# daijifeng001/MNC

Measured on AMD Instinct MI355X. Metric: images/sec (600x1000, 300 RoIs) VGG16 MNC-5stage, higher is better.
Workload: dtype f32; 1 GPU; VGG16 MNC 5-stage inference + gpu_mask_voting; one 600x1000 uint8 image per GPU per step (8 seeded images rotating), 300 RoIs per stage, H2D + device prep + forward + tail + gpu_mask_voting + D2H of the voted instances all inside the timed region; synthetic weights; math=fp32, images_in_flight_per_gpu=12, engine=native, parallelism=single GPU

## Files before the change

include/mnc_hip.h:

```cpp
#ifndef MNC_HIP_H_
#define MNC_HIP_H_

#include <stddef.h>

#ifdef __cplusplus
extern "C" {
#endif

#define MNC_API __attribute__((visibility("default")))

enum {
  MNC_OK = 0,
  MNC_ERR_INVALID = 1,
  MNC_ERR_HIP = 2,
  MNC_ERR_NOMEM = 3,
  MNC_ERR_STATE = 4,
  MNC_ERR_UNSUPPORTED = 5
};

MNC_API const char* mnc_last_error(void);
MNC_API int mnc_device_count(int* count);
MNC_API int mnc_device_mem_info(int device_id, size_t* free_bytes, size_t* total_bytes);
MNC_API const char* mnc_version(void);

// ... 61 lines not shown
  long long work;
  long long reserved1;
} mnc_mask_info;
typedef struct mnc_mask_head {
  int kept;
  int reserved0;
  long long bits_bytes;
  long long items;
  long long reserved1[29];
} mnc_mask_head;
MNC_API int mnc_instance_masks(const double* boxes, const float* masks, int n, int mask_size, double binarize_thresh,
                               int image_height, int image_width, int clip, int* bounds, long long* offsets, long long* areas,
                               void* bits, size_t bits_cap, size_t* bits_bytes, int device_id);

MNC_API int mnc_mask_overlaps(const int* a_bounds, const long long* a_offsets, const long long* a_areas, const void* a_bits,
                              size_t a_bytes, int na, const int* b_bounds, const long long* b_offsets, const long long* b_areas,
                              const void* b_bits, size_t b_bytes, int nb, long long* inter, double* iou, int device_id);
MNC_API int mnc_mask_nms(const int* bounds, const long long* offsets, const long long* areas, const void* bits, size_t bytes,
                         int n, const int* classes, const float* scores, double thresh, int class_aware, int* keep_out,
                         int* num_out, int device_id);

MNC_API int mnc_mask_rle(const int* bounds, const long long* offsets, const void* bits, size_t bytes, int n, int H, int W,
                         long long* run_ptr, unsigned* runs, size_t runs_cap, size_t* runs_total, int device_id);
MNC_API int mnc_mask_from_rle(const long long* run_ptr, const unsigned* runs, int n, int H, int W, int* bounds, long long* offsets,
                              long long* areas, void* bits, size_t bits_cap, size_t* bits_bytes, int device_id);

MNC_API int mnc_mask_match(const int* dt_bounds, const long long* dt_offsets, const long long* dt_areas, const void* dt_bits,
                           size_t dt_bytes, int nd, const int* dt_classes, const float* dt_scores, const int* gt_bounds,
                           const long long* gt_offsets, const long long* gt_areas, const void* gt_bits, size_t gt_bytes, int ng,
                           const int* gt_classes, const unsigned char* gt_crowd, const unsigned char* gt_ignore_in,
                           const double* gt_eval_area, const double* iou_thrs, int T, const double* area_rngs, int A, int max_det,
                           int* rank, int* dt_match, unsigned char* dt_ignore, int* gt_match, unsigned char* gt_ignore,
                           double* iou, int device_id);

MNC_API int mnc_mask_from_polygons(const double* xy, const long long* vert_ptr, const long long* poly_ptr, int n, int H, int W,
                                   int* bounds, long long* offsets, long long* areas, void* bits, size_t bits_cap,
                                   size_t* bits_bytes, int device_id);
MNC_API int mnc_mask_poly_timing(int on, double* last_ms);

MNC_API int mnc_coco_accumulate(const int* dt_class_idx, const float* dt_score, const int* dt_rank, const unsigned char* dt_flags,
                                int N, const int* gt_class_idx, const unsigned char* gt_ignore, int Gn, int K, int T, int A,
                                const int* max_dets, int M, const double* rec_thrs, int R, double* precision, double* recall,
                                long long* npig, int device_id);
MNC_API int mnc_coco_accum_timing(int on, double* last_ms);

MNC_API int mnc_mask_boundary(const int* bounds, const long long* offsets, const void* bits, size_t bytes, int n, int H, int W,
                              int d, int* out_bounds, long long* out_offsets, long long* out_areas, void* out_bits,
                              size_t bits_cap, size_t* bits_bytes, int device_id);
MNC_API int mnc_mask_match_boundary(const int* dt_bounds, const long long* dt_offsets, const long long* dt_areas, const void* dt_bits,
                                    size_t dt_bytes, int nd, const int* dt_classes, const float* dt_scores, const int* gt_bounds,
                                    const long long* gt_offsets, const long long* gt_areas, const void* gt_bits, size_t gt_bytes,
                                    int ng, const int* gt_classes, const unsigned char* gt_crowd, const unsigned char* gt_ignore_in,
                                    const double* gt_eval_area, const double* iou_thrs, int T, const double* area_rngs, int A,
                                    int max_det, int H, int W, int d, int* rank, int* dt_match, unsigned char* dt_ignore,
                                    int* gt_match, unsigned char* gt_ignore, double* iou, double* biou, int device_id);
MNC_API int mnc_mask_boundary_timing(int on, double* last_ms);

MNC_API int mnc_mask_components(const int* bounds, const long long* offsets, const void* bits, size_t bytes, int n, int connectivity,
                                long long* comp_ptr, long long* area, int* bbox, int* anchor, size_t comp_cap, size_t* n_comp,
                                int device_id);
MNC_API int mnc_mask_select(const int* bounds, const long long* offsets, const void* bits, size_t bytes, int n, int connectivity,
                            int min_area, int keep, long long* out_areas, void* out_bits, size_t bits_cap, int device_id);
MNC_API int mnc_mask_fill_holes(const int* bounds, const long long* offsets, const void* bits, size_t bytes, int n, int connectivity,
                                long long* out_areas, void* out_bits, size_t bits_cap, int device_id);
MNC_API int mnc_mask_split(const int* bounds, const long long* offsets, const void* bits, size_t bytes, int n, int connectivity,
                           int* out_bounds, long long* out_offsets, long long* out_areas, int* out_source, size_t comp_cap,
                           size_t* n_comp, void* out_bits, size_t bits_cap, size_t* bits_bytes, int device_id);
MNC_API int mnc_mask_components_timing(int on, double* last_ms);

MNC_API int mnc_mask_contours(const int* bounds, const long long* offsets, const void* bits, size_t bytes, int n, int connectivity,
                              long long* loop_ptr, long long* vert_ptr, long long* area, int* xy, size_t loop_cap, size_t vert_cap,
                              size_t* n_loops, size_t* n_verts, int device_id);
MNC_API int mnc_mask_contours_timing(int on, double* last_ms);

MNC_API int mnc_contours_simplify(const long long* vert_ptr, const int* xy, size_t n_loops, size_t n_verts, int q,
                                  long long* out_vert_ptr, int* out_xy, long long* out_index, size_t* out_verts, int device_id);
MNC_API int mnc_contours_simplify_timing(int on, double* last_ms);

MNC_API int mnc_mcg_maskdb(const int* superpixels, int H, int W, const int* label_ptr, const int* label_ids, int n,
                           int mask_size, double* boxes, unsigned char* masks, int device_id);

MNC_API int mnc_bbox_overlaps(const double* boxes, int n, const double* query_boxes, int k, double* overlaps);

typedef struct mnc_ctx mnc_ctx;

MNC_API int mnc_ctx_create(mnc_ctx** out, int device_id);
MNC_API int mnc_ctx_destroy(mnc_ctx* ctx);
MNC_API int mnc_ctx_sync(mnc_ctx* ctx);
MNC_API int mnc_ctx_device(const mnc_ctx* ctx, int* device_id);
MNC_API int mnc_ctx_arena_generation(const mnc_ctx* ctx, unsigned long* generation);

typedef struct mnc_layer_conventions {
  int warp_sample;
  int warp_round_edges;
  int warp_no_plus_one;
  int warp_oob;
  int resize_mode;
  int maskpool_binary;
  float maskpool_thresh;
  int inherit;
} mnc_layer_conventions;
MNC_API int mnc_ctx_set_layer_conventions(mnc_ctx* ctx, const mnc_layer_conventions* conv);
MNC_API int mnc_ctx_set_tuning(mnc_ctx* ctx, const char* name, const char* value);
MNC_API int mnc_ctx_get_layer_conventions(const mnc_ctx* ctx, mnc_layer_conventions* conv);

typedef struct mnc_graph mnc_graph;
MNC_API int mnc_ctx_capture_begin(mnc_ctx* ctx);
MNC_API int mnc_ctx_capture_end(mnc_ctx* ctx, mnc_graph** out);
MNC_API int mnc_graph_launch(mnc_ctx* ctx, mnc_graph* graph);
MNC_API int mnc_graph_destroy(mnc_graph* graph);
MNC_API int mnc_proposal_count_ptr(mnc_ctx* ctx, void** d_count);

MNC_API int mnc_dev_alloc(mnc_ctx* ctx, size_t bytes, void** d_ptr);
MNC_API int mnc_dev_free(mnc_ctx* ctx, void* d_ptr);
MNC_API int mnc_h2d(mnc_ctx* ctx, void* d_dst, const void* src_host, size_t bytes);
MNC_API int mnc_d2h(mnc_ctx* ctx, void* dst_host, const void* d_src, size_t bytes);
MNC_API int mnc_d2d(mnc_ctx* ctx, void* d_dst, const void* d_src, size_t bytes);
MNC_API int mnc_dev_zero(mnc_ctx* ctx, void* d_ptr, size_t bytes);
MNC_API int mnc_host_alloc(mnc_ctx* ctx, size_t bytes, void** host_ptr);
MNC_API int mnc_host_free(mnc_ctx* ctx, void* host_ptr);
MNC_API int mnc_h2d_async(mnc_ctx* ctx, void* d_dst, const void* src_host, size_t bytes);
MNC_API int mnc_d2h_async(mnc_ctx* ctx, void* dst_host, const void* d_src, size_t bytes);

MNC_API int mnc_prof_enable(mnc_ctx* ctx, int enable);
MNC_API int mnc_prof_reset(mnc_ctx* ctx);
MNC_API int mnc_prof_count(mnc_ctx* ctx, int* n_records);
MNC_API int mnc_prof_get(mnc_ctx* ctx, int index, char* name_buf, int name_cap, float* ms, double* flops,
                         double* bytes);

MNC_API int mnc_nchw_to_c8(mnc_ctx* ctx, const float* d_nchw, float* d_c8, int C, int H, int W);
MNC_API int mnc_c8_to_nchw(mnc_ctx* ctx, const float* d_c8, float* d_nchw, int C, int H, int W);
MNC_API int mnc_rchw_to_rhwc(mnc_ctx* ctx, const float* d_in, float* d_out, int R, int C, int PH, int PW);
MNC_API int mnc_rhwc_to_rchw(mnc_ctx* ctx, const float* d_in, float* d_out, int R, int C, int PH, int PW);
MNC_API int mnc_pack_conv3x3_weights(mnc_ctx* ctx, const float* d_oihw, float* d_packed, int Cout, int Cin);
MNC_API int mnc_pack_fc_weights(mnc_ctx* ctx, const float* d_nchw_cols, float* d_hwc_cols, int N, int C, int PH, int PW);

MNC_API int mnc_conv3x3_c3(mnc_ctx* ctx, const float* d_in_nchw, const float* d_w_oihw, const float* d_bias,
                           float* d_out_c8, int H, int W, int Cout, int relu);
MNC_API int mnc_conv3x3(mnc_ctx* ctx, const float* d_in_c8, const float* d_w_packed, const float* d_bias,
                        float* d_out_c8, int H, int W, int Cin, int Cout, int relu);
MNC_API int mnc_pack_conv3x3_bf16x3(mnc_ctx* ctx, const float* d_oihw, void* d_packed, int Cout, int Cin);
MNC_API int mnc_conv3x3_bf16x3(mnc_ctx* ctx, const float* d_in_c8, const void* d_w_packed, const float* d_bias,
                               float* d_out_c8, int H, int W, int Cin, int Cout, int relu);
MNC_API int mnc_pack_conv3x3_wino(mnc_ctx* ctx, const float* d_oihw, float* d_packed, int Cout, int Cin);
MNC_API int mnc_conv3x3_wino(mnc_ctx* ctx, const float* d_in_c8, const float* d_w_packed, const float* d_bias, float* d_out_c8,
                             int H, int W, int Cin, int Cout, int relu);
MNC_API int mnc_conv3x3_wino_pool(mnc_ctx* ctx, const float* d_in_c8, const float* d_w_packed, const float* d_bias,
                                  float* d_out_pooled_c8, int H, int W, int Cin, int Cout, int relu);
MNC_API int mnc_pack_conv3x3_wino4(mnc_ctx* ctx, const float* d_oihw, float* d_packed, int Cout, int Cin);
MNC_API int mnc_conv3x3_wino4(mnc_ctx* ctx, const float* d_in_c8, const float* d_w_packed, const float* d_bias, float* d_out_c8,
                              int H, int W, int Cin, int Cout, int relu);
MNC_API int mnc_conv3x3_wino4_pool(mnc_ctx* ctx, const float* d_in_c8, const float* d_w_packed, const float* d_bias,
                                   float* d_out_pooled_c8, int H, int W, int Cin, int Cout, int relu);
MNC_API int mnc_maxpool2_c8(mnc_ctx* ctx, const float* d_in, float* d_out, int C, int H, int W);
MNC_API int mnc_conv1x1_to_nchw(mnc_ctx* ctx, const float* d_in_c8, const float* d_w, const float* d_bias,
                                float* d_out_nchw, int H, int W, int Cin, int Cout);
MNC_API int mnc_rpn_softmax(mnc_ctx* ctx, const float* d_score_nchw, float* d_prob_nchw, int A, int H, int W);
MNC_API int mnc_rpn_heads(mnc_ctx* ctx, const float* d_in_c8, const float* d_w, const float* d_bias, float* d_score_nchw,
                          float* d_prob_nchw, int H, int W, int Cin, int A);
MNC_API int mnc_roi_warp(mnc_ctx* ctx, const float* d_feat_c8, int C, int H, int W, const float* d_rois, int R,
                         int PH, int PW, float spatial_scale, int pool2, float* d_out_rhwc);
MNC_API int mnc_pack_conv_weights(mnc_ctx* ctx, const float* d_oihw, float* d_packed, int Cout, int Cin, int KH, int KW);
MNC_API int mnc_conv2d(mnc_ctx* ctx, const float* d_in_c8, const float* d_w_packed, const float* d_bias,
                       const float* d_residual_c8, float* d_out_c8, int H, int W, int Cin, int Cout, int KH, int KW, int stride,
                       int pad, int relu);
MNC_API int mnc_pack_conv_weights_f16(mnc_ctx* ctx, const float* d_oihw, void* d_packed, int Cout, int Cin, int KH, int KW);
MNC_API int mnc_conv2d_f16(mnc_ctx* ctx, const float* d_in_c8, const void* d_w_packed, const float* d_bias,
                           const float* d_residual_c8, float* d_out_c8, int H, int W, int Cin, int Cout, int KH, int KW,
                           int stride, int pad, int relu);
MNC_API int mnc_pack_conv1x1(mnc_ctx* ctx, const float* d_w, void* d_packed, int Cout, int Cin, int f16);
MNC_API int mnc_conv1x1(mnc_ctx* ctx, const float* d_in_c8, const void* d_w_packed, const float* d_bias,
                        const float* d_residual_c8, float* d_out_c8, int H, int W, int Cin, int Cout, int stride, int relu);
MNC_API int mnc_conv1x1_f16_pk(mnc_ctx* ctx, const void* d_in_pk, const void* d_w_packed, const float* d_bias,
                               const void* d_residual, void* d_out, int H, int W, int Cin, int Cout, int stride, int relu,
                               int res_packed, int out_packed);
MNC_API int mnc_conv_stem_c3(mnc_ctx* ctx, const float* d_in_nchw, const float* d_w_oihw, const float* d_bias, float* d_out_c8,
                             int H, int W, int Cout, int K, int stride, int pad, int relu);
MNC_API int mnc_conv_stem_c3_fmt(mnc_ctx* ctx, const float* d_in_nchw, const float* d_w_oihw, const float* d_bias, void* d_out,
                                 int H, int W, int Cout, int K, int stride, int pad, int relu, int out_packed);
MNC_API int mnc_pack_conv_stem_f16(mnc_ctx* ctx, const float* d_w_oihw, void* d_packed, int Cout, int K);
MNC_API int mnc_conv_stem_f16(mnc_ctx* ctx, const float* d_in_nchw, const void* d_w_packed, const float* d_bias, void* d_out, int H,
                              int W, int Cout, int K, int stride, int pad, int relu, int out_packed);
MNC_API int mnc_maxpool_c8(mnc_ctx* ctx, const float* d_in, float* d_out, int C, int H, int W, int K, int stride, int pad);
MNC_API int mnc_maxpool_c8_f16(mnc_ctx* ctx, const void* d_in, void* d_out, int C, int H, int W, int K, int stride, int pad);
MNC_API int mnc_add(mnc_ctx* ctx, const float* d_a, const float* d_b, float* d_out, size_t n, int relu);
MNC_API int mnc_prep_image(mnc_ctx* ctx, const unsigned char* d_bgr_hwc, int H, int W, const double* means_host,
                           const int* d_x0, const float* d_ax, int OW, const int* d_y0, const float* d_ay, int OH,
                           float* d_out_chw, int PH, int PW);
MNC_API int mnc_roi_pool(mnc_ctx* ctx, const float* d_feat_c8, int N, int C, int H, int W, const float* d_rois, int R,
                         int PH, int PW, float spatial_scale, float* d_out_rhwc);
MNC_API int mnc_maxpool2_rhwc(mnc_ctx* ctx, const float* d_in, float* d_out, int R, int PH, int PW, int C);
MNC_API int mnc_mask_resize(mnc_ctx* ctx, const float* d_in, float* d_out, int R, int IH, int IW, int OH, int OW);
MNC_API int mnc_mask_pool(mnc_ctx* ctx, const float* d_feat, const float* d_mask, float* d_out, int R, int PH,
                          int PW, int C, int pool2);
MNC_API int mnc_fc(mnc_ctx* ctx, const float* d_a, const float* d_w, const float* d_bias, float* d_out, int M,
                   int N, int K, int ldc, int act);
MNC_API int mnc_fc_pair(mnc_ctx* ctx, const float* d_a0, const float* d_w0, const float* d_bias0, float* d_out0, const float* d_a1,
                        const float* d_w1, const float* d_bias1, float* d_out1, int M, int N, int K, int ldc, int act);
MNC_API int mnc_pack_fc_bf16x3(mnc_ctx* ctx, const float* d_w, void* d_packed, int N, int K);
MNC_API int mnc_fc_bf16x3(mnc_ctx* ctx, const float* d_a, const void* d_w_packed, const float* d_bias, float* d_out, int M,
                          int N, int K, int ldc, int act);
MNC_API size_t mnc_conv3x3_lowp_weight_bytes(int mode, int Cout, int Cin);
MNC_API int mnc_pack_conv3x3_lowp(mnc_ctx* ctx, int mode, const float* d_oihw, void* d_packed, int Cout, int Cin);
MNC_API int mnc_conv3x3_lowp(mnc_ctx* ctx, int mode, const void* d_in_packed, const void* d_w_packed, const float* d_bias,
                             void* d_out_packed, float* d_out_c8, int H, int W, int Cin, int Cout, int relu);
MNC_API int mnc_conv3x3_lowp_pool(mnc_ctx* ctx, int mode, const void* d_in_packed, const void* d_w_packed, const float* d_bias,
                                  void* d_out_pooled_packed, int H, int W, int Cin, int Cout, int relu);
MNC_API int mnc_pack_conv3x3_f16(mnc_ctx* ctx, const float* d_oihw, void* d_packed, int Cout, int Cin);
MNC_API int mnc_pack_conv3x3_bf16(mnc_ctx* ctx, const float* d_oihw, void* d_packed, int Cout, int Cin);
MNC_API int mnc_conv3x3_bf16(mnc_ctx* ctx, const float* d_in_c8, const void* d_w_packed, const float* d_bias, float* d_out_c8,
                             int H, int W, int Cin, int Cout, int relu);
MNC_API int mnc_conv3x3_f16(mnc_ctx* ctx, const float* d_in_c8, const void* d_w_packed, const float* d_bias, float* d_out_c8,
                            int H, int W, int Cin, int Cout, int relu);
MNC_API int mnc_conv3x3_bf16x3_pk(mnc_ctx* ctx, const void* d_in, const void* d_w_packed, const float* d_bias, void* d_out,
                                  int H, int W, int Cin, int Cout, int relu, int in_packed, int out_packed);
MNC_API int mnc_conv3x3_f16_pk(mnc_ctx* ctx, const void* d_in, const void* d_w_packed, const float* d_bias, void* d_out,
                               int H, int W, int Cin, int Cout, int relu, int in_packed, int out_packed);
MNC_API int mnc_conv3x3_bf16_pk(mnc_ctx* ctx, const void* d_in, const void* d_w_packed, const float* d_bias, void* d_out,
                                int H, int W, int Cin, int Cout, int relu, int in_packed, int out_packed);
MNC_API int mnc_conv3x3_c3_fmt(mnc_ctx* ctx, const float* d_in_nchw, const float* d_w_oihw, const float* d_bias, void* d_out,
                               int H, int W, int Cout, int relu, int out_fmt);
MNC_API int mnc_maxpool2_c8_bf16x3(mnc_ctx* ctx, const void* d_in, void* d_out, int C, int H, int W);
MNC_API int mnc_maxpool2_c8_f16(mnc_ctx* ctx, const void* d_in, void* d_out, int C, int H, int W);
MNC_API int mnc_maxpool2_c8_bf16(mnc_ctx* ctx, const void* d_in, void* d_out, int C, int H, int W);
MNC_API int mnc_act_pack(mnc_ctx* ctx, const float* d_c8, void* d_packed, size_t n, int f16);
MNC_API int mnc_act_unpack(mnc_ctx* ctx, const void* d_packed, float* d_c8, size_t n, int f16);
MNC_API int mnc_pack_fc_f16(mnc_ctx* ctx, const float* d_w, void* d_packed, int N, int K);
MNC_API int mnc_pack_fc_bf16(mnc_ctx* ctx, const float* d_w, void* d_packed, int N, int K);
MNC_API int mnc_fc_bf16(mnc_ctx* ctx, const float* d_a, const void* d_w_packed, const float* d_bias, float* d_out, int M, int N,
                        int K, int ldc, int act);
MNC_API int mnc_fc_f16(mnc_ctx* ctx, const float* d_a, const void* d_w_packed, const float* d_bias, float* d_out, int M, int N,
                       int K, int ldc, int act);
MNC_API int mnc_fc_lowp_pair(mnc_ctx* ctx, int mode, const float* d_a0, const void* d_a_sm0, const float* d_a1, const void* d_a_sm1,
                             int m_stride, const void* d_w0, const void* d_w1, const float* d_bias0, const float* d_bias1,
                             float* d_out0, float* d_out1, int M, int N, int K, int ldc, int act, void* d_out_sm0, void* d_out_sm1,
                             int out_sm_fmt);
MNC_API int mnc_fc_pack_act(mnc_ctx* ctx, const float* d_a, void* d_a_sm, int M, int K, int f16);
MNC_API int mnc_fc_unpack_act(mnc_ctx* ctx, const void* d_a_sm, float* d_a, int M, int K, int fmt);
MNC_API int mnc_roi_warp_sm_only_ok(mnc_ctx* ctx, int C, int pool2, int* ok);
MNC_API int mnc_fc_f16_pre(mnc_ctx* ctx, const void* d_a_sm, int m_stride, const void* d_w_packed, const float* d_bias,
                           float* d_out, int M, int N, int K, int ldc, int act);
MNC_API int mnc_fc_bf16x3_pre(mnc_ctx* ctx, const void* d_a_sm, int m_stride, const void* d_w_packed, const float* d_bias,
                              float* d_out, int M, int N, int K, int ldc, int act);
MNC_API int mnc_fc_f16_ex(mnc_ctx* ctx, const float* d_a, const void* d_a_sm, int m_stride, const void* d_w_packed,
                          const float* d_bias, float* d_out, int M, int N, int K, int ldc, int act, void* d_out_sm, int out_sm_fmt);
MNC_API int mnc_fc_bf16x3_ex(mnc_ctx* ctx, const float* d_a, const void* d_a_sm, int m_stride, const void* d_w_packed,
                             const float* d_bias, float* d_out, int M, int N, int K, int ldc, int act, void* d_out_sm,
                             int out_sm_fmt);
MNC_API int mnc_fc_bf16_ex(mnc_ctx* ctx, const float* d_a, const void* d_a_sm, int m_stride, const void* d_w_packed,
                           const float* d_bias, float* d_out, int M, int N, int K, int ldc, int act, void* d_out_sm, int out_sm_fmt);
MNC_API int mnc_roi_warp_sm(mnc_ctx* ctx, const float* d_feat_c8, int C, int H, int W, const float* d_rois, int R, int PH, int PW,
                            float spatial_scale, int pool2, float* d_out_rhwc, void* d_sm, int sm_fmt);
MNC_API int mnc_maxpool2_rhwc_sm(mnc_ctx* ctx, const float* d_in, float* d_out, int R, int PH, int PW, int C, void* d_sm,
                                 int sm_fmt);
MNC_API int mnc_mask_pool_sm(mnc_ctx* ctx, const float* d_feat, const float* d_mask, float* d_out, int R, int PH, int PW, int C,
                             int pool2, void* d_sm, int sm_fmt);
MNC_API int mnc_box_mask_pool(mnc_ctx* ctx, const float* d_feat, const float* d_mask, float* d_box_out, float* d_mask_out, int R,
                              int PH, int PW, int C, void* d_box_sm, void* d_mask_sm, int sm_fmt);
MNC_API int mnc_box_mask_pool_ex(mnc_ctx* ctx, const float* d_feat, const void* d_feat_sm, int feat_sm_fmt, const float* d_mask,
                                 float* d_box_out, float* d_mask_out, int R, int PH, int PW, int C, void* d_box_sm, void* d_mask_sm,
                                 int sm_fmt);
MNC_API int mnc_softmax_rows(mnc_ctx* ctx, const float* d_in, float* d_out, int M, int N);
MNC_API int mnc_softmax_rows_ld(mnc_ctx* ctx, const float* d_in, int ld_in, float* d_out, int M, int N);
MNC_API int mnc_eltwise(mnc_ctx* ctx, const float* d_in, float* d_out, size_t count, int op);
MNC_API int mnc_copy2d(mnc_ctx* ctx, float* d_dst, int dst_ld, const float* d_src, int src_ld, int rows, int cols);

MNC_API int mnc_proposal(mnc_ctx* ctx, const float* d_cls_prob, const float* d_bbox_pred, int A, int H, int W,
                         const float* anchors_host, int feat_stride, float im_h, float im_w, float im_scale,
                         int pre_nms_topn, int post_nms_topn, float nms_thresh, float min_size, float* d_rois,
                         int* num_rois_host);
MNC_API int mnc_mask_voting_dev(mnc_ctx* ctx, const float* d_boxes, const float* d_masks, const float* d_scores, int n,
                                int num_classes, int mask_size, int max_per_image, float nms_thresh, float iou_thresh,
                                int image_height, int image_width, float* out_mask, int* out_box, float* out_score,
                                int* class_count, int* result_num);
MNC_API int mnc_vote_instances(mnc_ctx* ctx, const float* d_boxes, const float* d_masks, const float* d_scores, int n,
                               int num_classes, int mask_size, int max_per_image, float nms_thresh, float iou_thresh,
                               int image_height, int image_width, float* d_records, int record_cap, int* d_counts);
#define MNC_VOTE_MV 0
#define MNC_VOTE_IMAGE 1
MNC_API int mnc_vote_instances_ex(mnc_ctx* ctx, int mode, const float* d_boxes, const float* d_masks, const float* d_scores,
                                  int n, int num_classes, int mask_size, int max_per_image, float nms_thresh, float iou_thresh,
                                  double binarize_thresh, int image_height, int image_width, float* d_records, int record_cap,
                                  int* d_counts);
MNC_API int mnc_render_records(mnc_ctx* ctx, const float* d_records, const int* d_counts, int record_cap, int num_classes,
                               int mask_size, double vis_thresh, double binarize_thresh, int H, int W,
                               const unsigned char* d_bgr_hwc, float alpha, int* d_inst, int* d_cls, unsigned char* d_inst_rgb,
                               unsigned char* d_cls_rgb, unsigned char* d_overlay_rgb, int* d_kept);
MNC_API int mnc_mask_records(mnc_ctx* ctx, const float* d_records, const int* d_counts, int record_cap, int num_classes,
                             int mask_size, double score_thresh, double binarize_thresh, int H, int W, void** d_info,
                             void** d_bits);
MNC_API int mnc_mask_overlaps_dev(mnc_ctx* ctx, const void* d_info, const void* d_bits, int rows_cap, const int* b_bounds,
                                  const long long* b_offsets, const long long* b_areas, const void* b_bits, size_t b_bytes, int nb,
                                  void** d_inter, void** d_iou);
MNC_API int mnc_mask_nms_dev(mnc_ctx* ctx, const void* d_info, const void* d_bits, int rows_cap, double thresh, int class_aware,
                             void** d_keep);
MNC_API int mnc_mask_rle_dev(mnc_ctx* ctx, const void* d_info, const void* d_bits, int rows_cap, int H, int W, size_t runs_cap,
                             void** d_rle);
MNC_API int mnc_mask_match_dev(mnc_ctx* ctx, const void* d_info, const void* d_bits, int rows_cap, const int* gt_bounds,
                               const long long* gt_offsets, const long long* gt_areas, const void* gt_bits, size_t gt_bytes, int ng,
                               const int* gt_classes, const unsigned char* gt_crowd, const unsigned char* gt_ignore_in,
                               const double* gt_eval_area, const double* iou_thrs, int T, const double* area_rngs, int A,
                               int max_det, int want_iou, void** d_rank, void** d_dt_match, void** d_dt_ignore, void** d_gt_match,
                               void** d_gt_ignore, void** d_iou);
MNC_API int mnc_detect_tail(mnc_ctx* ctx, const float* d_rois1, int R1, const float* d_rois2, int R2, float scale,
                            int image_height, int image_width, float* d_boxes);

MNC_API int mnc_proposal_count(mnc_ctx* ctx, int* num_rois_host);
MNC_API int mnc_proposal_candidates(mnc_ctx* ctx, float* boxes_host, float* scores_host, int capacity, int* n_host);
MNC_API int mnc_stage_bridge(mnc_ctx* ctx, const float* d_rois, const float* d_bbox_pred, int ld_bbox, const float* d_probs,
                             int ld_probs, int R, int K, float im_h, float im_w, float* d_rois_ext);

typedef struct mnc_net mnc_net;
typedef struct mnc_net_config {
  int trunk_channels[5];
  int rpn_channels;
  int num_anchors;
  float anchors[64];
  int feat_stride;
  int pre_nms_topn, post_nms_topn;
  float rpn_nms_thresh, rpn_min_size;
  int mask_fc, mask_size;
  int fc_dim;
  int num_classes;
  int roi_size;
  float spatial_scale;
  int target_size, max_size;
  double pixel_means[3];
  int max_per_image;
  float vote_nms_thresh, vote_iou_thresh;
  int math;
  int use_graph;
  int winograd;
  mnc_layer_conventions conventions;
} mnc_net_config;

MNC_API int mnc_net_default_config(mnc_net_config* cfg);
MNC_API int mnc_net_create(mnc_ctx* ctx, const mnc_net_config* cfg, mnc_net** out);
MNC_API int mnc_net_create_shared(mnc_ctx* ctx, mnc_net* parent, mnc_net** out);
MNC_API int mnc_net_set_param(mnc_net* net, const char* layer, int index, const float* data_host, size_t count);
MNC_API int mnc_net_load_file(mnc_net* net, const char* path);
MNC_API int mnc_net_set_voting(mnc_net* net, int mode, double binarize_thresh);
MNC_API int mnc_forward_image(mnc_net* net, const unsigned char* bgr_host, int H, int W, float* records_host, int record_cap,
                              int* counts_host);
MNC_API int mnc_forward_image_async(mnc_net* net, const unsigned char* bgr_host, int H, int W, float** d_records, int** d_counts);
MNC_API int mnc_net_fetch(mnc_net* net, float* records_host, int record_cap, int* counts_host);
MNC_API int mnc_net_render(mnc_net* net, double vis_thresh, double binarize_thresh, float alpha, int* inst_host, int* cls_host,
                           unsigned char* inst_rgb_host, unsigned char* cls_rgb_host, unsigned char* overlay_rgb_host,
                           int* kept_host);
MNC_API int mnc_net_masks(mnc_net* net, double score_thresh, double binarize_thresh, void* info_host, int info_cap,
                          void* bits_host, size_t bits_cap, size_t* bits_bytes);
MNC_API int mnc_net_blob(mnc_net* net, const char* name, void** d_ptr, int* dims, int* ndim);
// ... 13 lines not shown
```

mnc_amd/_lib.py:

```python
import ctypes
import os
import re

import numpy as np

HERE = os.path.dirname(os.path.abspath(__file__))
HEADER = os.path.join(HERE, "..", "include", "mnc_hip.h")
LIB_PATH = os.environ.get("MNC_LIB_PATH") or os.path.join(HERE, "libmnc_hip.so")

MNC_OK = 0


class MncError(RuntimeError):
    def __init__(self, code, func, msg):
        RuntimeError.__init__(self, "%s failed (status %d): %s" % (func, code, msg))
        self.code = code


_CTYPES = {
    "int": ctypes.c_int, "float": ctypes.c_float, "size_t": ctypes.c_size_t, "double": ctypes.c_double,
    "void": None,
}


def _map_type(t):
    t = t.replace("const ", "").strip()
    if t.endswith("*"):
        return ctypes.c_void_p
    return _CTYPES[t]


def parse_header(path=HEADER):
    with open(path) as f:
        src = f.read()
    src = re.sub(r"/\*.*?\*/", "", src, flags=re.S)
    decls = {}
    for m in re.finditer(r"MNC_API\s+([\w\s\*]+?)\s*\b(\w+)\s*\(([^)]*)\)\s*;", src):
        ret, name, args = m.group(1).strip(), m.group(2), m.group(3).strip()
        argtypes, argnames = [], []
        if args and args != "void":
            for a in args.split(","):
                a = " ".join(a.split())
                mm = re.match(r"(.+?)(\w+)$", a)
                argtypes.append(_map_type(mm.group(1)))
                argnames.append(mm.group(2))
        restype = ctypes.c_char_p if "char" in ret else _map_type(ret)
        decls[name] = (restype, argtypes, argnames)
    return decls


_lib = None
_decls = None


def load():
    global _lib, _decls
    if _lib is not None:
        return _lib
    if not os.path.isfile(LIB_PATH):
        from . import _build
        _build.build()
    lib = ctypes.CDLL(LIB_PATH)
    _decls = parse_header()
    for name, (restype, argtypes, _) in _decls.items():
        fn = getattr(lib, name)
        fn.restype = restype
        fn.argtypes = argtypes
    _lib = lib
    return lib


def call(name, *args):
    lib = load()
    rc = getattr(lib, name)(*args)
    if rc != MNC_OK:
        raise MncError(rc, name, lib.mnc_last_error().decode("utf-8", "replace"))
    return rc


def ptr(a):
    if a is None:
        return None
    if isinstance(a, np.ndarray):
        assert a.flags["C_CONTIGUOUS"], "array must be C-contiguous"
        return a.ctypes.data
    return a


def device_count():
    n = ctypes.c_int(0)
    call("mnc_device_count", ctypes.addressof(n))
    return n.value


def device_mem_info(device_id=0):
    fr, tot = ctypes.c_size_t(0), ctypes.c_size_t(0)
    call("mnc_device_mem_info", int(device_id), ctypes.addressof(fr), ctypes.addressof(tot))
    return fr.value, tot.value


def timing(entry_name, on):
    last = ctypes.c_double(-1.0)
    call(entry_name, int(bool(on)), ctypes.addressof(last))
    return float(last.value)
```

mnc_amd/csrc/gemm.hip:

```cpp
#include <atomic>
#include <type_traits>
#include <cstdlib>

#include "fc_plan.h"
#include "mnc_internal.h"
#include "x3_split.h"

namespace mnc {

typedef float f32x16 __attribute__((ext_vector_type(16)));

constexpr int kBN = 128, kBK = 32;

__device__ __forceinline__ float apply_act(float v, int act) {
  if (act == 1) return fmaxf(v, 0.f);
  if (act == 2) return 1.0f / (1.0f + expf(-v));
  return v;
}

template <int kMT, int kSK = 32, int ABL = 0>
__global__ __launch_bounds__(256) void fc_mfma_kernel(const float* __restrict__ A, const float* __restrict__ Wt,
                                                      const float* __restrict__ bias, float* __restrict__ out,
                                                      float* __restrict__ part, int M, int N, int K, int ldc, int kper,
                                                      int act, int fused, int tn_, int splits_, int tm_) {
// ... 231 lines not shown
  typedef float f32x4v __attribute__((ext_vector_type(4)));
  f32x4v hacc[2] = {{0.f, 0.f, 0.f, 0.f}, {0.f, 0.f, 0.f, 0.f}};
  const int r16 = lane & 15, g4 = lane >> 4;
  int h_off[8];
#pragma unroll
  for (int c = 0; c < 8; ++c)
    h_off[c] = ((2 * (c >> 1) + (g4 & 1)) ^ ((r16 >> 1) & 7)) * 16 + (2 * (c & 1) + (g4 >> 1)) * 4;
  const int ha_base = ((kMT - 1) * 32 + r16) * 128, hb_base = (kBM + wn * 32 + r16) * 128;
  int hflip = 0;

  int a_off[4], b_off[4];
#pragma unroll
  for (int kc = 0; kc < 4; ++kc) {
    const int c = (2 * kc + kk) ^ ((j >> 1) & 7);
    a_off[kc] = ((wm * TR * 32 + j) * 32 + c * 4) * 4;
    b_off[kc] = ((kBM + wn * 32 + j) * 32 + c * 4) * 4;
  }
  struct Frags { float4 a[TR]; float4 b; float ha[2]; float hb[2][2]; };
  auto read_frags = [&](int kc, int flip, Frags& f, auto last_tag) {
    constexpr bool LAST = decltype(last_tag)::value;
    f.b = *reinterpret_cast<const float4*>(s_fc_dma + (b_off[kc] ^ flip));
#pragma unroll
    for (int t = 0; t < (LAST ? TR - 1 : TR); ++t) f.a[t] = *reinterpret_cast<const float4*>(s_fc_dma + (a_off[kc] ^ flip) + t * 4096);
    if (LAST) {
      const int hf = hflip ^ flip;
#pragma unroll
      for (int h = 0; h < 2; ++h) {
        f.ha[h] = *reinterpret_cast<const float*>(s_fc_dma + ((ha_base + h_off[2 * kc + h]) ^ hf));
        f.hb[h][0] = *reinterpret_cast<const float*>(s_fc_dma + ((hb_base + h_off[2 * kc + h]) ^ hf));
        f.hb[h][1] = *reinterpret_cast<const float*>(s_fc_dma + ((hb_base + 2048 + h_off[2 * kc + h]) ^ hf));
      }
    }
  };
  auto half_mfmas = [&](const Frags& f) {
    hacc[0] = __builtin_amdgcn_mfma_f32_16x16x4f32(f.ha[0], f.hb[0][0], hacc[0], 0, 0, 0);
    hacc[1] = __builtin_amdgcn_mfma_f32_16x16x4f32(f.ha[0], f.hb[0][1], hacc[1], 0, 0, 0);
    hacc[0] = __builtin_amdgcn_mfma_f32_16x16x4f32(f.ha[1], f.hb[1][0], hacc[0], 0, 0, 0);
    hacc[1] = __builtin_amdgcn_mfma_f32_16x16x4f32(f.ha[1], f.hb[1][1], hacc[1], 0, 0, 0);
  };
  auto mfmas = [&](const Frags& f, auto last_tag) {
    constexpr bool LAST = decltype(last_tag)::value;
    constexpr int NT = LAST ? TR - 1 : TR;
#pragma unroll
    for (int t = 0; t < NT; ++t) acc[t] = __builtin_amdgcn_mfma_f32_32x32x2f32(f.a[t].x, f.b.x, acc[t], 0, 0, 0);
#pragma unroll
    for (int t = 0; t < NT; ++t) acc[t] = __builtin_amdgcn_mfma_f32_32x32x2f32(f.a[t].y, f.b.y, acc[t], 0, 0, 0);
    if (LAST) half_mfmas(f);
#pragma unroll
    for (int t = 0; t < NT; ++t) acc[t] = __builtin_amdgcn_mfma_f32_32x32x2f32(f.a[t].z, f.b.z, acc[t], 0, 0, 0);
#pragma unroll
    for (int t = 0; t < NT; ++t) acc[t] = __builtin_amdgcn_mfma_f32_32x32x2f32(f.a[t].w, f.b.w, acc[t], 0, 0, 0);
  };
  auto pin_acc = [&]() {
#pragma unroll
    for (int t = 0; t < TR; ++t) asm volatile("" : "+a"(acc[t]));
  };

  auto run = [&](auto last_tag) {
    constexpr bool LAST = decltype(last_tag)::value;
    constexpr int NT = LAST ? TR - 1 : TR;
    constexpr int kNM = 4 * NT + (LAST ? 4 : 0), kNR = NT + 1 + (LAST ? 6 : 0);
    Frags f0, f1;
    dma_stage(0, 0);
    dma_stage(1, kBufXor);
    dma_wait();
    __syncthreads();
    read_frags(0, 0, f0, last_tag);
    int cur = 0;
    for (int s = 0; s < nstages; ++s) {
      read_frags(1, 0, f1, last_tag);
      mfmas(f0, last_tag);
      read_frags(2, 0, f0, last_tag);
      mfmas(f1, last_tag);
      read_frags(3, 0, f1, last_tag);
      mfmas(f0, last_tag);
#pragma unroll
      for (int i = 0; i < 3 * kNM; ++i) {
        __builtin_amdgcn_sched_group_barrier(0x008, 1, 0);
        if ((i + 1) * 3 * kNR / (3 * kNM) > i * 3 * kNR / (3 * kNM)) __builtin_amdgcn_sched_group_barrier(0x100, 1, 0);
      }
      pin_acc();
      dma_wait();
      __syncthreads();
      read_frags(0, kBufXor, f0, last_tag);
      {
        const long off = ABL == 1 ? 0 : (long)min(s + 2, nstages - 1) * 32;
#pragma unroll
        for (int q = 0; q < 4; ++q) {
#pragma unroll
          for (int t = 0; t < NT; ++t) {
            const int i = q * NT + t;
            const float av = q == 0 ? f1.a[t].x : q == 1 ? f1.a[t].y : q == 2 ? f1.a[t].z : f1.a[t].w;
            const float bv = q == 0 ? f1.b.x : q == 1 ? f1.b.y : q == 2 ? f1.b.z : f1.b.w;
            acc[t] = __builtin_amdgcn_mfma_f32_32x32x2f32(av, bv, acc[t], 0, 0, 0);
            if (i >= 4 * NT - kPer - 2 && i < 4 * NT - 2) {
              __builtin_amdgcn_sched_barrier(0);
              dma_piece(i - (4 * NT - kPer - 2), off, cur);
              __builtin_amdgcn_sched_barrier(0);
            }
          }
          if (LAST && q == 0) half_mfmas(f1);
        }
      }
      pin_acc();
#pragma unroll
      for (int kc = 0; kc < 4; ++kc) { a_off[kc] ^= kBufXor; b_off[kc] ^= kBufXor; }
      hflip ^= kBufXor;
      cur ^= kBufXor;
    }
    dma_wait();
    __syncthreads();
  };
  if (nstages > 0) {
    if (last_wave) run(std::true_type{});
    else run(std::false_type{});
  }

  const int n = n0 + wn * 32 + j;
  if (n < N) {
    const float bv = fused ? bias[n] : 0.f;
#pragma unroll
    for (int t = 0; t < TR; ++t) {
      if (last_wave && t == TR - 1) continue;
      if (wm * TR + t < mtiles) {
#pragma unroll
        for (int e = 0; e < 16; ++e) {
          const int m = m0 + (wm * TR + t) * 32 + (e & 3) + 8 * (e >> 2) + 4 * kk;
          if (m < M) {
            if (fused) out[(long)m * ldc + n] = apply_act(acc[t][e] + bv, act);
            else part[((long)split * M + m) * N + n] = acc[t][e];
          }
        }
      }
    }
  }
  if (last_wave) {
#pragma unroll
    for (int ch = 0; ch < 2; ++ch) {
      const int nh = n0 + wn * 32 + ch * 16 + r16;
      if (nh >= N) continue;
      const float bh = fused ? bias[nh] : 0.f;
#pragma unroll
      for (int e = 0; e < 4; ++e) {
        const int m = m0 + (kMT - 1) * 32 + 4 * g4 + e;
        if (m < M) {
          if (fused) out[(long)m * ldc + nh] = apply_act(hacc[ch][e] + bh, act);
          else part[((long)split * M + m) * N + nh] = hacc[ch][e];
        }
      }
    }
  }
}

template <int kMT, int ABL = 0, int BUF = 0>
__global__ __launch_bounds__(512) void fc_mfma_dma16_kernel(const float* __restrict__ A_0, const float* __restrict__ Wt_0,
                                                            const float* __restrict__ bias_0, float* __restrict__ out_0,
                                                            float* __restrict__ part_0, int M, int N, int K, int ldc, int kper,
                                                            int act, int fused, int tn_, int splits_, int tm_, int drop_last,
                                                            const float* __restrict__ A_1,
                                                            const float* __restrict__ Wt_1, const float* __restrict__ bias_1,
                                                            float* __restrict__ out_1, int pair_tn) {
  constexpr int kBM = 32 * kMT;
  constexpr int kRows = kBM + kBN;
  constexpr int kNW = 8;
  constexpr int TS = kMT;
  constexpr int kPer = kRows * 128 / 1024 / kNW;
  static_assert(kRows % (8 * kNW) == 0 && kMT % 2 == 0, "whole pieces and row tiles per wave");
  extern __shared__ __attribute__((aligned(1024))) char s_fc_dma[];
  constexpr int kBufXor = 65536;
  const int tid = threadIdx.x, lane = tid & 63;
  const int wave = __builtin_amdgcn_readfirstlane(tid >> 6);
  const int wn = wave & 3, wm = wave >> 2;
  const int r16 = lane & 15, g4 = lane >> 4;
  int bn, split, bmz;
  xcd_decode(blockIdx.x, tn_, splits_, tm_, bn, split, bmz);
  const int which = (pair_tn && bn >= pair_tn) ? 1 : 0;
  bn -= which * pair_tn;
  const float* __restrict__ A = which ? A_1 : A_0;
  const float* __restrict__ Wt = which ? Wt_1 : Wt_0;
  const float* __restrict__ bias = which ? bias_1 : bias_0;
  float* __restrict__ out = which ? out_1 : out_0;
  float* __restrict__ part = part_0;
  const int n0 = bn * kBN, m0 = bmz * kBM;
  const int kbeg = split * kper, kend = min(K, kbeg + kper);
  const int nstages = (kend - kbeg) / 32;
  const int mrows = min(M - m0, kBM);

  const float* src[kPer];
#pragma unroll
  for (int i = 0; i < kPer; ++i) {
    const int slot = (wave + kNW * i) * 64 + lane, r = slot >> 3, c = (slot & 7) ^ ((r >> 1) & 7);
    src[i] = (r < kBM ? A + (long)(m0 + min(r, mrows - 1)) * K
                      : Wt + (long)min(n0 + r - kBM, N - 1) * K) + kbeg + c * 4;
  }
  const unsigned lds0 = (unsigned)(unsigned long)(__attribute__((address_space(3))) char*)s_fc_dma;
  typedef int i32x4d __attribute__((ext_vector_type(4)));
  auto make_rsrc = [](const float* base) {
    const unsigned long a = (unsigned long)base;
    i32x4d r;
    r.x = __builtin_amdgcn_readfirstlane((int)(unsigned)a);
    r.y = __builtin_amdgcn_readfirstlane((int)((unsigned)(a >> 32) & 0xFFFFu));
    r.z = 0x70000000;
    r.w = 0x00020000;
    return r;
  };
  const i32x4d rs_a = make_rsrc(A + (long)m0 * K + kbeg), rs_w = make_rsrc(Wt + (long)min(n0, N - 1) * K + kbeg);
  int voff[kPer];
#pragma unroll
  for (int i = 0; i < kPer; ++i) {
    const int slot = (wave + kNW * i) * 64 + lane, r = slot >> 3, c = (slot & 7) ^ ((r >> 1) & 7);
    voff[i] = (r < kBM ? min(r, mrows - 1) * K : (min(n0 + r - kBM, N - 1) - min(n0, N - 1)) * K) * 4 + c * 16;
  }
  auto dma_piece = [&](int i, long off, int buf_byte, bool in_loop = false) {
    const unsigned l = __builtin_amdgcn_readfirstlane(lds0 + (unsigned)buf_byte + (unsigned)(wave + kNW * i) * 1024u);
    if (BUF) {
      const bool is_a = (wave + kNW * i) * 8 < kBM;
      const i32x4d rs = is_a ? rs_a : rs_w;
      const int so = __builtin_amdgcn_readfirstlane((int)off * 4);
      const int vo = ((ABL & 4) && in_loop) ? 0x7FFFFFF0 : voff[i];
      asm volatile("s_mov_b32 m0, %3\n\ts_nop 0\n\tbuffer_load_dwordx4 %0, %1, %2 offen lds" ::"v"(vo), "s"(rs), "s"(so), "s"(l) : "memory");
    } else {
      const float* g = src[i] + off;
      asm volatile("s_mov_b32 m0, %1\n\ts_nop 0\n\tglobal_load_lds_dwordx4 %0, off" ::"v"(g), "s"(l));
    }
  };
  auto dma_stage = [&](int s, int buf_byte) {
    const long off = (long)min(s, nstages - 1) * 32;
#pragma unroll
    for (int i = 0; i < kPer; ++i) dma_piece(i, off, buf_byte);
  };
  auto dma_wait = [&]() { asm volatile("s_waitcnt vmcnt(0)" ::: "memory"); };

  typedef float f32x4v __attribute__((ext_vector_type(4)));
  f32x4v acc[TS][2];
#pragma unroll
  for (int i = 0; i < TS; ++i)
#pragma unroll
    for (int c = 0; c < 2; ++c) acc[i][c] = f32x4v{0.f, 0.f, 0.f, 0.f};

  int a_off[2], b_off[2];
#pragma unroll
  for (int G = 0; G < 2; ++G) {
    const int sl = ((4 * G + g4) ^ ((r16 >> 1) & 7)) * 16;
    a_off[G] = (wm * TS * 16 + r16) * 128 + sl;
    b_off[G] = (kBM + wn * 32 + r16) * 128 + sl;
  }
  const bool last_wave = drop_last && wm == 1;

  auto run = [&](auto last_tag) {
    constexpr int NS = decltype(last_tag)::value ? TS - 1 : TS;
    constexpr int kNM = 8 * NS, kNR = NS + 2;
    struct Frags { f32x4v a[NS]; f32x4v b[2]; };
    auto read_frags = [&](int G, int flip, Frags& f) {
      f.b[0] = *reinterpret_cast<const f32x4v*>(s_fc_dma + (b_off[G] ^ flip));
      f.b[1] = *reinterpret_cast<const f32x4v*>(s_fc_dma + (b_off[G] ^ flip) + 2048);
#pragma unroll
      for (int i = 0; i < NS; ++i) f.a[i] = *reinterpret_cast<const f32x4v*>(s_fc_dma + (a_off[G] ^ flip) + i * 2048);
    };
    Frags f0, f1;
    dma_stage(0, 0);
    dma_stage(1, kBufXor);
    static_assert(kPer == 7, "the literal in the wait below");
    asm volatile("s_waitcnt vmcnt(7)" ::: "memory");
    __syncthreads();
    read_frags(0, 0, f0);
    int cur = 0;
    for (int s = 0; s < nstages; ++s) {
      read_frags(1, 0, f1);
#pragma unroll
      for (int q = 0; q < 4; ++q)
#pragma unroll
        for (int i = 0; i < NS; ++i) {
          acc[i][0] = __builtin_amdgcn_mfma_f32_16x16x4f32(f0.a[i][q], f0.b[0][q], acc[i][0], 0, 0, 0);
          acc[i][1] = __builtin_amdgcn_mfma_f32_16x16x4f32(f0.a[i][q], f0.b[1][q], acc[i][1], 0, 0, 0);
        }
#pragma unroll
      for (int i = 0; i < kNM; ++i) {
        __builtin_amdgcn_sched_group_barrier(0x008, 1, 0);
        if ((i + 1) * 2 * kNR / kNM > i * 2 * kNR / kNM && i * 2 < kNM) __builtin_amdgcn_sched_group_barrier(0x100, 1, 0);
      }
      dma_wait();
      if (!(ABL & 2)) __syncthreads();
      read_frags(0, kBufXor, f0);
      {
        const long off = (long)min(s + 2, nstages - 1) * 32;
#pragma unroll
        for (int q = 0; q < 4; ++q)
#pragma unroll
          for (int i = 0; i < NS; ++i) {
            acc[i][0] = __builtin_amdgcn_mfma_f32_16x16x4f32(f1.a[i][q], f1.b[0][q], acc[i][0], 0, 0, 0);
            acc[i][1] = __builtin_amdgcn_mfma_f32_16x16x4f32(f1.a[i][q], f1.b[1][q], acc[i][1], 0, 0, 0);
            const int m = 2 * (q * NS + i);
            if (m >= kNM - 4 * kPer - 8 && m < kNM - 8 && (m - (kNM - 4 * kPer - 8)) % 4 == 0) {
              __builtin_amdgcn_sched_barrier(0);
              if (!(ABL & 1)) dma_piece((m - (kNM - 4 * kPer - 8)) / 4, off, cur, true);
              __builtin_amdgcn_sched_barrier(0);
            }
          }
      }
#pragma unroll
      for (int G = 0; G < 2; ++G) { a_off[G] ^= kBufXor; b_off[G] ^= kBufXor; }
      cur ^= kBufXor;
    }
    dma_wait();
    __syncthreads();
  };
  if (nstages > 0) {
    if (last_wave) run(std::true_type{});
    else run(std::false_type{});
  }

  const bool final_out = fused == 1;
  if (fused == 0) {
    constexpr int kSlabF4 = kNW * TS * 2 * 64;
    const int tile = bmz * tn_ + which * pair_tn + bn;
    f32x4v* slab = reinterpret_cast<f32x4v*>(part) + ((size_t)tile * splits_ + split) * kSlabF4 + wave * TS * 2 * 64 + lane;
#pragma unroll
    for (int i = 0; i < TS; ++i)
#pragma unroll
      for (int c = 0; c < 2; ++c) slab[(i * 2 + c) * 64] = acc[i][c];
    return;
  }
#pragma unroll
  for (int c = 0; c < 2; ++c) {
    const int n = n0 + wn * 32 + c * 16 + r16;
    if (n >= N) continue;
    const float bv = final_out ? bias[n] : 0.f;
#pragma unroll
    for (int i = 0; i < TS; ++i)
#pragma unroll
      for (int e = 0; e < 4; ++e) {
        const int m = m0 + wm * TS * 16 + i * 16 + 4 * g4 + e;
        if (m < M) {
          out[(long)m * ldc + n] = apply_act(acc[i][c][e] + bv, act);
        }
      }
  }
}

__global__ __launch_bounds__(256) void fc_reduce_slab_kernel(const float* __restrict__ part, const float* __restrict__ bias0,
                                                             const float* __restrict__ bias1, float* __restrict__ out0,
                                                             float* __restrict__ out1, int M, int N, int ldc, int splits, int act,
                                                             int tn_all, int pair_tn, int ntiles) {
  constexpr int kSlabF4 = 8 * 10 * 2 * 64;
  typedef float f32x4v __attribute__((ext_vector_type(4)));
  const f32x4v* p4 = reinterpret_cast<const f32x4v*>(part);
  const long total = (long)ntiles * kSlabF4;
  for (long idx = (long)blockIdx.x * blockDim.x + threadIdx.x; idx < total; idx += (long)gridDim.x * blockDim.x) {
    const int tile = (int)(idx / kSlabF4), piece = (int)(idx - (long)tile * kSlabF4);
    const int lane = piece & 63, ic = (piece >> 6) % 20, wave = piece / (64 * 20);
    const int i = ic >> 1, c = ic & 1, wn = wave & 3, wm = wave >> 2, r16 = lane & 15, g4 = lane >> 4;
    const int bmz = tile / tn_all;
    int bn = tile - bmz * tn_all;
    const int which = (pair_tn && bn >= pair_tn) ? 1 : 0;
    bn -= which * pair_tn;
    const int n = bn * kBN + wn * 32 + c * 16 + r16;
    const int m0 = bmz * 320 + wm * 160 + i * 16 + 4 * g4;
    if (n >= N || m0 >= M) continue;
    const f32x4v* src = p4 + (long)tile * splits * kSlabF4 + piece;
    f32x4v v = {0.f, 0.f, 0.f, 0.f};
    int sp = 0;
    for (; sp + 4 <= splits; sp += 4) {
      const f32x4v a = src[(long)sp * kSlabF4], b = src[(long)(sp + 1) * kSlabF4], cc = src[(long)(sp + 2) * kSlabF4],
                   d = src[(long)(sp + 3) * kSlabF4];
      v = (((v + a) + b) + cc) + d;
    }
    for (; sp < splits; ++sp) v += src[(long)sp * kSlabF4];
    const float bv = (which ? bias1 : bias0)[n];
    float* o = (which ? out1 : out0) + (long)m0 * ldc + n;
#pragma unroll
    for (int e = 0; e < 4; ++e)
      if (m0 + e < M) o[(long)e * ldc] = apply_act(v[e] + bv, act);
  }
}

template <int VEC, int SM = 0>
__global__ __launch_bounds__(256) void fc_reduce_kernel(const float* __restrict__ part, const float* __restrict__ bias,
                                                        float* __restrict__ out, int M, int N, int ldc, int splits,
                                                        int act, void* __restrict__ sm = nullptr, long sm_rows = 0,
                                                        long sm_row0 = 0, const float* __restrict__ part1 = nullptr,
                                                        const float* __restrict__ bias1 = nullptr, float* __restrict__ out1 = nullptr,
                                                        void* __restrict__ sm1 = nullptr) {
  if (blockIdx.y) { part = part1; bias = bias1; out = out1; sm = sm1; }
  const long total = (long)M * N;
  if (VEC == 4) {
    const int n4 = N >> 2;
    const long total4 = total >> 2;
    const float4* p4 = reinterpret_cast<const float4*>(part);
    for (long i = (long)blockIdx.x * blockDim.x + threadIdx.x; i < total4; i += (long)gridDim.x * blockDim.x) {
      const int n = (int)(i % n4) * 4;
      const long m = i / n4;
      float4 v = make_float4(0.f, 0.f, 0.f, 0.f);
      int s = 0;
      for (; s + 4 <= splits; s += 4) {
        const float4 a = p4[(long)s * total4 + i], b = p4[(long)(s + 1) * total4 + i], c = p4[(long)(s + 2) * total4 + i],
                     d = p4[(long)(s + 3) * total4 + i];
        v.x = (((v.x + a.x) + b.x) + c.x) + d.x;
        v.y = (((v.y + a.y) + b.y) + c.y) + d.y;
        v.z = (((v.z + a.z) + b.z) + c.z) + d.z;
        v.w = (((v.w + a.w) + b.w) + c.w) + d.w;
      }
      for (; s < splits; ++s) {
        const float4 a = p4[(long)s * total4 + i];
        v.x += a.x; v.y += a.y; v.z += a.z; v.w += a.w;
      }
      const float4 b = *reinterpret_cast<const float4*>(bias + n);
      const float4 y =
          make_float4(apply_act(v.x + b.x, act), apply_act(v.y + b.y, act), apply_act(v.z + b.z, act), apply_act(v.w + b.w, act));
      *reinterpret_cast<float4*>(out + m * ldc + n) = y;
      if (SM) sm_store4<SM>(sm, sm_rows, sm_row0 + m, n, y);
    }
    return;
  }
  for (long idx = (long)blockIdx.x * blockDim.x + threadIdx.x; idx < total; idx += (long)gridDim.x * blockDim.x) {
    const int n = (int)(idx % N);
    const long m = idx / N;
    float v = 0.f;
    for (int s = 0; s < splits; ++s) v += part[(long)s * total + idx];
    out[m * ldc + n] = apply_act(v + bias[n], act);
  }
}

void fc_reduce_launch(hipStream_t stream, const float* part, const float* bias, float* out, int M, int N, int ldc, int splits,
                      int act) {
  fc_reduce_launch_sm(stream, part, bias, out, M, N, ldc, splits, act, nullptr, 0, 0, 0);
}

bool fc_reduce_launch_sm(hipStream_t stream, const float* part, const float* bias, float* out, int M, int N, int ldc, int splits,
                         int act, void* sm, int sm_fmt, long sm_rows, long sm_row0) {
  const bool vec = N % 4 == 0 && ldc % 4 == 0 && (reinterpret_cast<uintptr_t>(out) & 15) == 0 &&
                   (reinterpret_cast<uintptr_t>(bias) & 15) == 0;
  const long items = vec ? (long)M * N / 4 : (long)M * N;
  int g = (int)((items + 255) / 256);
  if (g > 4096) g = 4096;
  const bool sm_ok = sm && vec && (((sm_fmt == 1 || sm_fmt == 3) && N % 64 == 0) || (sm_fmt == 2 && N % 32 == 0));
  if (sm_ok && sm_fmt == 1)
    hipLaunchKernelGGL((fc_reduce_kernel<4, 1>), dim3(g), dim3(256), 0, stream, part, bias, out, M, N, ldc, splits, act, sm, sm_rows, sm_row0);
  else if (sm_ok && sm_fmt == 3)
    hipLaunchKernelGGL((fc_reduce_kernel<4, 3>), dim3(g), dim3(256), 0, stream, part, bias, out, M, N, ldc, splits, act, sm, sm_rows, sm_row0);
  else if (sm_ok)
    hipLaunchKernelGGL((fc_reduce_kernel<4, 2>), dim3(g), dim3(256), 0, stream, part, bias, out, M, N, ldc, splits, act, sm, sm_rows, sm_row0);
  else if (vec) hipLaunchKernelGGL((fc_reduce_kernel<4, 0>), dim3(g), dim3(256), 0, stream, part, bias, out, M, N, ldc, splits, act, nullptr, 0L, 0L);
  else hipLaunchKernelGGL((fc_reduce_kernel<1, 0>), dim3(g), dim3(256), 0, stream, part, bias, out, M, N, ldc, splits, act, nullptr, 0L, 0L);
  return sm_ok;
}

bool fc_reduce_pair_launch_sm(hipStream_t stream, const float* part0, const float* part1, const float* bias0, const float* bias1,
                              float* out0, float* out1, int M, int N, int ldc, int splits, int act, void* sm0, void* sm1, int sm_fmt,
                              long sm_rows, bool* sm_done) {
  const bool vec = N % 4 == 0 && ldc % 4 == 0 && ((reinterpret_cast<uintptr_t>(out0) | reinterpret_cast<uintptr_t>(out1) |
                                                   reinterpret_cast<uintptr_t>(bias0) | reinterpret_cast<uintptr_t>(bias1)) & 15) == 0;
  if (!vec || (sm0 != nullptr) != (sm1 != nullptr)) return false;
  const long items = (long)M * N / 4;
  int g = (int)((items + 255) / 256);
  if (g > 4096) g = 4096;
  const bool sm_ok = sm0 && (((sm_fmt == 1 || sm_fmt == 3) && N % 64 == 0) || (sm_fmt == 2 && N % 32 == 0));
  if (sm_ok && sm_fmt == 1)
    hipLaunchKernelGGL((fc_reduce_kernel<4, 1>), dim3(g, 2), dim3(256), 0, stream, part0, bias0, out0, M, N, ldc, splits, act, sm0, sm_rows, 0L,
                       part1, bias1, out1, sm1);
  else if (sm_ok && sm_fmt == 3)
    hipLaunchKernelGGL((fc_reduce_kernel<4, 3>), dim3(g, 2), dim3(256), 0, stream, part0, bias0, out0, M, N, ldc, splits, act, sm0, sm_rows, 0L,
                       part1, bias1, out1, sm1);
  else if (sm_ok)
    hipLaunchKernelGGL((fc_reduce_kernel<4, 2>), dim3(g, 2), dim3(256), 0, stream, part0, bias0, out0, M, N, ldc, splits, act, sm0, sm_rows, 0L,
                       part1, bias1, out1, sm1);
  else
    hipLaunchKernelGGL((fc_reduce_kernel<4, 0>), dim3(g, 2), dim3(256), 0, stream, part0, bias0, out0, M, N, ldc, splits, act, (void*)nullptr, 0L,
                       0L, part1, bias1, out1, (void*)nullptr);
  *sm_done = sm_ok;
  return true;
}

__global__ void softmax_rows_kernel(const float* __restrict__ in, int ld_in, float* __restrict__ out, int M, int N) {
  const int m = blockIdx.x * blockDim.x + threadIdx.x;
  if (m >= M) return;
  const float* r = in + (long)m * ld_in;
  float mx = r[0];
  for (int i = 1; i < N; ++i) mx = fmaxf(mx, r[i]);
  float sum = 0.f;
  for (int i = 0; i < N; ++i) sum += expf(r[i] - mx);
  for (int i = 0; i < N; ++i) out[(long)m * N + i] = expf(r[i] - mx) / sum;
}

__global__ __launch_bounds__(256) void softmax_rows_wave_kernel(const float* __restrict__ in, int ld_in,
                                                                float* __restrict__ out, int M, int N) {
  const int lane = threadIdx.x & 63;
  const int m = blockIdx.x * (blockDim.x >> 6) + (threadIdx.x >> 6);
  if (m >= M) return;
  const bool live = lane < N;
  const float v = live ? in[(long)m * ld_in + lane] : -INFINITY;
  float mx = v;
  for (int o = 32; o > 0; o >>= 1) mx = fmaxf(mx, __shfl_xor(mx, o));
  const float e = live ? expf(v - mx) : 0.f;
  float sum = 0.f;
  for (int i = 0; i < N; ++i) sum += __shfl(e, i);
  if (live) out[(long)m * N + lane] = e / sum;
}

__global__ void eltwise_kernel(const float* __restrict__ in, float* __restrict__ out, size_t n, int op) {
  for (size_t i = (size_t)blockIdx.x * blockDim.x + threadIdx.x; i < n; i += (size_t)gridDim.x * blockDim.x)
    out[i] = apply_act(in[i], op);
}

__global__ void pack_fc_kernel(const float* __restrict__ in, float* __restrict__ out, long N, int C, int P) {
  const long total = N * C * P;
  for (long idx = (long)blockIdx.x * blockDim.x + threadIdx.x; idx < total; idx += (long)gridDim.x * blockDim.x) {
    const int c = (int)(idx % C);
    const long r = idx / C;
    const int p = (int)(r % P);
    const long n = r / P;
    out[idx] = in[(n * C + c) * P + p];
  }
}

}

using namespace mnc;

extern "C" {

int mnc_fc(mnc_ctx* ctx, const float* d_a, const float* d_w, const float* d_bias, float* d_out, int M, int N, int K,
           int ldc, int act) {
  MNC_REQUIRE(ctx && d_a && d_w && d_bias && d_out, "mnc_fc: null pointer");
  MNC_REQUIRE(M >= 0 && N > 0 && K > 0 && K % kBK == 0 && ldc >= N && act >= 0 && act <= 2,
              "mnc_fc: unsupported shape M=%d N=%d K=%d ldc=%d act=%d (need K%%32==0)", M, N, K, ldc, act);
  if (M == 0) return MNC_OK;
  const FcPlan p = fc_plan(FcCall(M, N, K, ldc), ctx->tune, kTuningBuild);
  if (p.head) {
    const int head = p.head;
    const bool defer = ctx->defer_reduce;
    ctx->defer_reduce = false;
    int rc = mnc_fc(ctx, d_a, d_w, d_bias, d_out, head, N, K, ldc, act);
    if (!rc) rc = mnc_fc(ctx, d_a + (size_t)head * K, d_w, d_bias, d_out + (size_t)head * ldc, M - head, N, K, ldc, act);
    ctx->defer_reduce = defer;
    ctx->deferred_part = nullptr;
    ctx->deferred_splits = 1;
    return rc;
  }
  const int mt = p.mt, tn = p.tn, tm = p.tm, splits = p.splits, kper = p.kper;
  const bool small = p.small, dma = p.kernel == kFcDma16, slab = p.slab;
  float* part = nullptr;
  if (splits > 1) {
    int rc = ensure_scratch(ctx, p.part_bytes);
    if (rc) return rc;
    part = (float*)ctx->scratch.p;
  }
  const double flops = 2.0 * M * (double)N * K, bytes = 4.0 * ((double)N * K + (double)M * K + (double)M * N);
  {
    LaunchScope ls(ctx, small ? "fc_mfma_small" : "fc_mfma", flops, bytes);
#define MNC_FC_LAUNCH(MT, SK, A) hipLaunchKernelGGL((fc_mfma_kernel<MT, SK, A>), dim3(tn * splits * tm), dim3(256), 0, ctx->stream, \
                         d_a, d_w, d_bias, d_out, part, M, N, K, ldc, kper, act, splits == 1 ? 1 : 0, tn, splits, tm)
#define MNC_FC_DMA_LAUNCH(A, WM) MNC_FC_DMA_LAUNCH_H(A, WM, 0)
#define MNC_FC_DMA_LAUNCH_H(A, WM, H)                                                                                               \
  do {                                                                                                                              \
    MNC_HIP_TRY((lds_limit_once<fc_mfma_dma_kernel<10, A, WM, H>>(ctx->device, lds)));                                              \
    hipLaunchKernelGGL((fc_mfma_dma_kernel<10, A, WM, H>), dim3(tn * splits * tm), dim3(256 * WM), lds, ctx->stream, d_a, d_w, d_bias, \
                       d_out, part, M, N, K, ldc, kper, act, splits == 1 ? 1 : 0, tn, splits, tm);                                  \
  } while (0)
    if (dma) {
      constexpr int lds = 65536 + (320 + kBN) * 32 * 4;
      bool launched = false;
#ifdef MNC_TUNING
      const int waves = tune(ctx, T_FC_DMA_WAVES, 8), dabl = tune(ctx, T_FC_DMA_ABL, 0);
      if (dabl >= 16) {
        launched = true;
        auto kern = dabl == 17 ? fc_mfma_dma16_kernel<10, 1> : dabl == 18 ? fc_mfma_dma16_kernel<10, 2> : dabl == 19 ? fc_mfma_dma16_kernel<10, 3>
                    : dabl == 20 ? fc_mfma_dma16_kernel<10, 0, 1> : dabl == 21 ? fc_mfma_dma16_kernel<10, 4, 1> : fc_mfma_dma16_kernel<10, 0>;
        MNC_HIP_TRY(hipFuncSetAttribute(reinterpret_cast<const void*>(kern), hipFuncAttributeMaxDynamicSharedMemorySize, lds));
        hipLaunchKernelGGL(kern, dim3(tn * splits * tm), dim3(512), lds, ctx->stream, d_a, d_w, d_bias, d_out, part, M, N, K, ldc, kper,
                           act, splits == 1 ? 1 : 0, tn, splits, tm, p.drop, (const float*)nullptr, (const float*)nullptr,
                           (const float*)nullptr, (float*)nullptr, 0);
      } else if (tune(ctx, T_FC_MFMA16, 1) == 0 || waves == 4 || dabl) {
        launched = true;
        if (dabl == 1) MNC_FC_DMA_LAUNCH(1, 1);
        else if (dabl == 3) MNC_FC_DMA_LAUNCH(3, 1);
        else if (waves == 4) MNC_FC_DMA_LAUNCH(0, 1);
        else if (tm == 1 && M > 288 && M <= 304 && tune(ctx, T_FC_HALF, 1) != 0) MNC_FC_DMA_LAUNCH_H(0, 2, 1);
        else MNC_FC_DMA_LAUNCH(0, 2);
      }
#endif
      if (!launched) {
        if (p.buf) MNC_HIP_TRY((lds_limit_once<fc_mfma_dma16_kernel<10, 0, 1>>(ctx->device, lds)));
        else MNC_HIP_TRY((lds_limit_once<fc_mfma_dma16_kernel<10, 0, 0>>(ctx->device, lds)));
        hipLaunchKernelGGL((p.buf ? fc_mfma_dma16_kernel<10, 0, 1> : fc_mfma_dma16_kernel<10, 0, 0>), dim3(tn * splits * tm), dim3(512), lds,
                           ctx->stream, d_a, d_w, d_bias, d_out, part, M, N, K, ldc, kper, act, splits == 1 ? 1 : 0, tn, splits,
                           tm, p.drop, (const float*)nullptr, (const float*)nullptr, (const float*)nullptr, (float*)nullptr, 0);
      }
    }
    else if (mt == 2) MNC_FC_LAUNCH(2, 32, 0);
    else if (mt == 5) {
#ifdef MNC_TUNING
      const int abl = tune(ctx, T_FC_ABL, 0);
      if (abl == 1) MNC_FC_LAUNCH(5, 16, 1);
      else if (abl == 3) MNC_FC_LAUNCH(5, 16, 3);
      else
#endif
      MNC_FC_LAUNCH(5, 16, 0);
    } else {
#ifdef MNC_TUNING
      const int abl = tune(ctx, T_FC_ABL, 0);
      if (abl == 1) MNC_FC_LAUNCH(10, 32, 1);
      else if (abl == 2) MNC_FC_LAUNCH(10, 32, 2);
      else if (abl == 3) MNC_FC_LAUNCH(10, 32, 3);
      else if (abl == 4) MNC_FC_LAUNCH(10, 32, 4);
      else
#endif
      MNC_FC_LAUNCH(10, 32, 0);
    }
#undef MNC_FC_LAUNCH
#undef MNC_FC_DMA_LAUNCH
#undef MNC_FC_DMA_LAUNCH_H
    int rc = ls.finish("fc_mfma_kernel");
    if (rc) return rc;
  }
  if (ctx->defer_reduce && !slab) {
    ctx->deferred_part = splits > 1 ? part : nullptr;
    ctx->deferred_splits = splits > 1 ? splits : 1;
    return MNC_OK;
  }
  ctx->deferred_part = nullptr;
  ctx->deferred_splits = 1;
  if (splits > 1 && slab) {
    LaunchScope ls(ctx, "fc_reduce", 0.0, 4.0 * ((double)splits + 1.0) * M * N);
    long g = ((long)tn * tm * 10240 + 255) / 256;
    if (g > 8192) g = 8192;
    hipLaunchKernelGGL(fc_reduce_slab_kernel, dim3((int)g), dim3(256), 0, ctx->stream, part, d_bias, (const float*)nullptr, d_out,
                       (float*)nullptr, M, N, ldc, splits, act, tn, 0, tn * tm);
    return ls.finish("fc_reduce_slab_kernel");
  }
  if (splits > 1) {
    LaunchScope ls(ctx, "fc_reduce", 0.0, 4.0 * ((double)splits + 1.0) * M * N);
    fc_reduce_launch(ctx->stream, part, d_bias, d_out, M, N, ldc, splits, act);
    return ls.finish("fc_reduce_kernel");
  }
  return MNC_OK;
}

int mnc_fc_pair(mnc_ctx* ctx, const float* d_a0, const float* d_w0, const float* d_bias0, float* d_out0, const float* d_a1,
                const float* d_w1, const float* d_bias1, float* d_out1, int M, int N, int K, int ldc, int act) {
  MNC_REQUIRE(ctx && d_a0 && d_w0 && d_bias0 && d_out0 && d_a1 && d_w1 && d_bias1 && d_out1, "mnc_fc_pair: null pointer");
  MNC_REQUIRE(M >= 0 && N > 0 && K > 0 && K % kBK == 0 && ldc >= N && act >= 0 && act <= 2,
              "mnc_fc_pair: unsupported shape M=%d N=%d K=%d ldc=%d act=%d (need K%%32==0)", M, N, K, ldc, act);
  if (M == 0) return MNC_OK;
  FcCall call(M, N, K, ldc);
  call.defer_reduce = ctx->defer_reduce;
  call.aligned16 = ((reinterpret_cast<uintptr_t>(d_out0) | reinterpret_cast<uintptr_t>(d_out1) | reinterpret_cast<uintptr_t>(d_bias0) |
                     reinterpret_cast<uintptr_t>(d_bias1)) & 15) == 0;
  const FcPlan p = fc_pair_plan(call, ctx->tune, kTuningBuild);
  if (p.two_singles) {
    int rc = mnc_fc(ctx, d_a0, d_w0, d_bias0, d_out0, M, N, K, ldc, act);
    if (rc) return rc;
    return mnc_fc(ctx, d_a1, d_w1, d_bias1, d_out1, M, N, K, ldc, act);
  }
  const int tn = p.tn / 2, tm = p.tm, splits = p.splits, kper = p.kper;
  float* part = nullptr;
  if (splits > 1) {
    int rc = ensure_scratch(ctx, p.part_bytes);
    if (rc) return rc;
    part = (float*)ctx->scratch.p;
  }
  constexpr int lds = 65536 + (320 + kBN) * 32 * 4;
  {
    const double flops = 4.0 * M * (double)N * K, bytes = 8.0 * ((double)N * K + (double)M * K + (double)M * N);
    LaunchScope ls(ctx, "fc_mfma", flops, bytes);
    MNC_HIP_TRY((lds_limit_once<fc_mfma_dma16_kernel<10, 0, 1>>(ctx->device, lds)));
    hipLaunchKernelGGL((fc_mfma_dma16_kernel<10, 0, 1>), dim3(2 * tn * splits * tm), dim3(512), lds, ctx->stream, d_a0, d_w0, d_bias0,
                       d_out0, part, M, N, K, ldc, kper, act, splits == 1 ? 1 : 0, 2 * tn, splits, tm, p.drop, d_a1, d_w1,
                       d_bias1, d_out1, tn);
    int rc = ls.finish("fc_mfma_dma16_kernel");
    if (rc) return rc;
  }
  if (splits > 1) {
    LaunchScope ls(ctx, "fc_reduce", 0.0, 8.0 * ((double)splits + 1.0) * M * N);
    long g = ((long)2 * tn * tm * 10240 + 255) / 256;
    if (g > 8192) g = 8192;
    hipLaunchKernelGGL(fc_reduce_slab_kernel, dim3((int)g), dim3(256), 0, ctx->stream, part, d_bias0, d_bias1, d_out0, d_out1, M, N,
                       ldc, splits, act, 2 * tn, tn, 2 * tn * tm);
    return ls.finish("fc_reduce_slab_kernel");
  }
  return MNC_OK;
}

int mnc_softmax_rows_ld(mnc_ctx* ctx, const float* d_in, int ld_in, float* d_out, int M, int N) {
  MNC_REQUIRE(ctx && d_in && d_out && M >= 0 && N > 0 && ld_in >= N, "mnc_softmax_rows: bad argument");
  if (M == 0) return MNC_OK;
  LaunchScope ls(ctx, "softmax_rows");
  if (N <= 64)
    hipLaunchKernelGGL(softmax_rows_wave_kernel, dim3(cdiv(M, 4)), dim3(256), 0, ctx->stream, d_in, ld_in, d_out, M, N);
  else
    hipLaunchKernelGGL(softmax_rows_kernel, dim3(cdiv(M, 64)), dim3(64), 0, ctx->stream, d_in, ld_in, d_out, M, N);
  return ls.finish("softmax_rows_kernel");
}

int mnc_softmax_rows(mnc_ctx* ctx, const float* d_in, float* d_out, int M, int N) {
  return mnc_softmax_rows_ld(ctx, d_in, N, d_out, M, N);
}

int mnc_eltwise(mnc_ctx* ctx, const float* d_in, float* d_out, size_t count, int op) {
  MNC_REQUIRE(ctx && (count == 0 || (d_in && d_out)) && (op == 1 || op == 2), "mnc_eltwise: bad argument");
  if (count == 0) return MNC_OK;
  LaunchScope ls(ctx, "eltwise");
  size_t g = (count + 255) / 256;
  if (g > 8192) g = 8192;
  hipLaunchKernelGGL(eltwise_kernel, dim3((int)g), dim3(256), 0, ctx->stream, d_in, d_out, count, op);
  return ls.finish("eltwise_kernel");
}

int mnc_copy2d(mnc_ctx* ctx, float* d_dst, int dst_ld, const float* d_src, int src_ld, int rows, int cols) {
  MNC_REQUIRE(ctx && rows >= 0 && cols >= 0 && dst_ld >= cols && src_ld >= cols, "mnc_copy2d: bad argument");
  if (rows == 0 || cols == 0) return MNC_OK;
  MNC_REQUIRE(d_dst && d_src, "mnc_copy2d: null pointer");
  MNC_HIP_TRY(hipMemcpy2DAsync(d_dst, (size_t)dst_ld * 4, d_src, (size_t)src_ld * 4, (size_t)cols * 4, rows,
                               hipMemcpyDeviceToDevice, ctx->stream));
  return MNC_OK;
}

int mnc_pack_fc_weights(mnc_ctx* ctx, const float* d_in, float* d_out, int N, int C, int PH, int PW) {
  MNC_REQUIRE(ctx && d_in && d_out && N > 0 && C > 0 && PH > 0 && PW > 0, "mnc_pack_fc_weights: bad argument");
  LaunchScope ls(ctx, "pack_fc");
  long total = (long)N * C * PH * PW;
  long g = (total + 255) / 256;
  if (g > 65536) g = 65536;
  hipLaunchKernelGGL(pack_fc_kernel, dim3((int)g), dim3(256), 0, ctx->stream, d_in, d_out, (long)N, C, PH * PW);
  return ls.finish("pack_fc_kernel");
}

}
```

mnc_amd/csrc/mnc_internal.h:

```cpp
#pragma once
#include <hip/hip_runtime.h>

#include <atomic>
#include <cstdarg>
#include <cstdio>
#include <cstring>
#include <mutex>
#include <string>
#include <vector>

#include "../../include/mnc_hip.h"
#include "tune.h"
#include "ws_layout.h"

namespace mnc {

struct DevArena {
  void* p = nullptr;
  size_t cap = 0;
};

void set_error(const char* fmt, ...);
void clear_error();

// ... 74 lines not shown
  do {                                                                                                   \
    if ((ctx)->capturing) {                                                                              \
      mnc::set_error("%s: synchronises or re-allocates; not allowed while a launch sequence is captured", what); \
      return MNC_ERR_STATE;                                                                              \
    }                                                                                                    \
  } while (0)

#define MNC_REQUIRE(cond, ...)       \
  do {                               \
    if (!(cond)) {                   \
      mnc::set_error(__VA_ARGS__);   \
      return MNC_ERR_INVALID;        \
    }                                \
  } while (0)

template <auto kKernel>
inline hipError_t lds_limit_once(int device, int bytes) {
  static std::atomic<unsigned long long> done{0};
  const unsigned long long bit = 1ull << (device & 63);
  if (done.load(std::memory_order_relaxed) & bit) return hipSuccess;
  const hipError_t e = hipFuncSetAttribute(reinterpret_cast<const void*>(kKernel), hipFuncAttributeMaxDynamicSharedMemorySize, bytes);
  if (e == hipSuccess) done.fetch_or(bit, std::memory_order_relaxed);
  return e;
}

struct LaunchScope {
  mnc_ctx* ctx;
  bool on;
  LaunchScope(mnc_ctx* c, const char* name, double flops = 0.0, double bytes = 0.0) : ctx(c) {
    (void)hipSetDevice(ctx->device);
    on = ctx->profiling == 1 || (ctx->profiling == 2 && flops >= 1.0e9);
    if (on) prof_begin(ctx, name, flops, bytes);
  }
  int finish(const char* name) {
    if (on) prof_end(ctx);
    hipError_t e = hipGetLastError();
    if (e != hipSuccess) {
      set_error("kernel launch %s failed: %s", name, hipGetErrorString(e));
      return MNC_ERR_HIP;
    }
    return MNC_OK;
  }
};

__device__ __forceinline__ void xcd_decode(int bid, int tn, int splits, int tm, int& bn, int& split, int& bm) {
  const int total = tn * splits * tm;
  const int q = total >> 3, r = total & 7;
  const int xcd = bid & 7, idx = bid >> 3;
  const int logical = (xcd < r ? xcd * (q + 1) : r * (q + 1) + (xcd - r) * q) + idx;
  bn = logical % tn;
  const int rest = logical / tn;
  split = rest % splits;
  bm = rest / splits;
}

typedef unsigned mnc_u32x4 __attribute__((ext_vector_type(4)));
typedef float mnc_f32x4 __attribute__((ext_vector_type(4)));
__device__ __forceinline__ __amdgpu_buffer_rsrc_t slab_rsrc(float* base) {
  return __builtin_amdgcn_make_buffer_rsrc(base, 0, 0x7FFFFFF0, 0x00020000);
}
__device__ __forceinline__ void slab_store(__amdgpu_buffer_rsrc_t rs, int voff, int soff, mnc_f32x4 v) {
  __builtin_amdgcn_raw_buffer_store_b128(__builtin_bit_cast(mnc_u32x4, v), rs, voff, soff,  16);
}
__device__ __forceinline__ mnc_f32x4 slab_load(__amdgpu_buffer_rsrc_t rs, int voff, int soff) {
  return __builtin_bit_cast(mnc_f32x4, __builtin_amdgcn_raw_buffer_load_b128(rs, voff, soff,  16));
}
__device__ __forceinline__ bool slab_last_arriver(unsigned* ticket, int arrivals, volatile unsigned* flag) {
  asm volatile("s_waitcnt vmcnt(0)" ::: "memory");
  __syncthreads();
  if (threadIdx.x == 0) *flag = __hip_atomic_fetch_add(ticket, 1u, __ATOMIC_RELAXED, __HIP_MEMORY_SCOPE_AGENT);
  __syncthreads();
  const bool last = __builtin_amdgcn_readfirstlane(*flag) == (unsigned)(arrivals - 1);
  if (last) {
    if (threadIdx.x == 0) {
      __hip_atomic_store(ticket, 0u, __ATOMIC_RELAXED, __HIP_MEMORY_SCOPE_AGENT);
      __builtin_amdgcn_fence(__ATOMIC_ACQUIRE, "agent");
    }
    __syncthreads();
  }
  return last;
}

struct CallBuf {
  void* p = nullptr;
  ~CallBuf() { if (p) (void)hipFree(p); }
  int alloc(const char* who, size_t bytes);
};

struct HostScope {
  std::unique_lock<std::mutex> lock;
  hipStream_t stream = nullptr;
  void* buf = nullptr;
  int open(int device_id, size_t bytes);
  hipError_t up(void* d_dst, const void* src, size_t bytes) const {
    return bytes ? hipMemcpyAsync(d_dst, src, bytes, hipMemcpyHostToDevice, stream) : hipSuccess;
  }
  hipError_t down(void* dst, const void* d_src, size_t bytes) const {
    return bytes ? hipMemcpyAsync(dst, d_src, bytes, hipMemcpyDeviceToHost, stream) : hipSuccess;
  }
  hipError_t sync() const { return hipStreamSynchronize(stream); }
};

struct CallTimer {
  std::atomic<int> on{0};
  std::atomic<double> last_ms{-1.0};
  int set(int enable, double* out_last_ms);
};

struct TimedSpan {
  CallTimer& timer;
  hipEvent_t a = nullptr, b = nullptr;
  bool on = false;
  explicit TimedSpan(CallTimer& t) : timer(t) {}
  TimedSpan(const TimedSpan&) = delete;
  ~TimedSpan() {
    if (a) (void)hipEventDestroy(a);
    if (b) (void)hipEventDestroy(b);
  }
  void begin(hipStream_t s) {
    if (!timer.on.load(std::memory_order_relaxed)) return;
    on = hipEventCreate(&a) == hipSuccess && hipEventCreate(&b) == hipSuccess && hipEventRecord(a, s) == hipSuccess;
  }
  void end(hipStream_t s) { if (on) on = hipEventRecord(b, s) == hipSuccess; }
  double ms() {
    float t = 0.f;
    if (on) on = hipEventElapsedTime(&t, a, b) == hipSuccess;
    return on ? (double)t : 0.0;
  }
  void keep() {
    const double t = ms();
    if (on) timer.last_ms.store(t);
  }
  void keep_sum(TimedSpan& earlier) {
    const double t = earlier.ms() + ms();
    if (on && earlier.on) timer.last_ms.store(t);
  }
};

int nms_mask_launch(hipStream_t stream, const float* d_boxes, const int* d_order, int n, int dim, float thr,
                    unsigned long long* d_mask, int batch);
int nms_scan_launch(hipStream_t stream, const unsigned long long* d_mask, int n, int max_keep, int* d_keep, int* d_num,
                    int batch);
int nms_mask_launch_indirect(hipStream_t stream, const float* d_boxes, const int* d_order, const int* d_n, int n_cap,
                             int dim, float thr, unsigned long long* d_mask);
int nms_scan_launch_indirect(hipStream_t stream, const unsigned long long* d_mask, const int* d_n, int n_cap, int max_keep,
                             int* d_keep, int* d_num, const float* d_gather_boxes = nullptr, const int* d_gather_order = nullptr,
                             float* d_rois = nullptr, int rois_cap = 0);
void proposal_state_free(void* state);
void comm_free(mnc_ctx* ctx);
void fc_reduce_launch(hipStream_t stream, const float* part, const float* bias, float* out, int M, int N, int ldc, int splits,
                      int act);
bool fc_reduce_launch_sm(hipStream_t stream, const float* part, const float* bias, float* out, int M, int N, int ldc, int splits,
                         int act, void* sm, int sm_fmt, long sm_rows, long sm_row0);
bool fc_reduce_pair_launch_sm(hipStream_t stream, const float* part0, const float* part1, const float* bias0, const float* bias1,
                              float* out0, float* out1, int M, int N, int ldc, int splits, int act, void* sm0, void* sm1, int sm_fmt,
                              long sm_rows, bool* sm_done);
void conv_splitk_reduce_launch(hipStream_t stream, const float* d_part, const float* d_bias, float* d_out, int H, int W,
                               int Cout, int ksplit, int relu);
int heads_finish_launch(mnc_ctx* ctx, const float* part, int splits, const float* bias, float* heads, int ld, int M, int K,
                        float* scores, const float* rois, float im_h, float im_w, float* rois_ext, const float* rois1,
                        const float* rois2, float scale, int image_height, int image_width, float* boxes, const int* copy_src,
                        int* copy_dst);
int c8_to_hwc_launch(mnc_ctx* ctx, const float* d_feat, float* d_hwc, int C, int H, int W);
int roi_warp_from_hwc(mnc_ctx* ctx, const float* d_hwc, int C, int H, int W, const float* d_rois, int R, int PH, int PW, float scale,
                      int pool2, float* d_out, void* d_sm, int sm_fmt);
bool roi_warp_sm_only_ok(const mnc_ctx* ctx, int C, int pool2);
int detect_tail_launch(mnc_ctx* ctx, const float* d_rois1, int R1, const float* d_rois2, int R2, float scale, int image_height,
                       int image_width, float* d_boxes, const int* d_copy_src, int* d_copy_dst);
int mv_launch(hipStream_t stream, const float* d_boxes, int box_dim, const float* d_masks, int S, const int* d_inds,
              const int* d_begins, const int* d_ends, const float* d_wts, int H, int W, int R, int* d_bounds,
              float* d_out_mask, int* d_out_box);
int mv_image_launch(hipStream_t stream, const float* d_boxes, const float* d_masks, int S, const int* d_inds, const int* d_begins,
                    const int* d_ends, const float* d_wts, int H, int W, double thresh, int R, const int* d_rcount, int grid_rows,
                    int* d_bounds, float* d_records, const float* d_rscore, const int* d_rows, int record_cap);

}
```

mnc_amd/csrc/pipeline.hip:

```cpp
#include <atomic>
#include <cmath>
#include <map>
#include <string>

#include "mnc_internal.h"

namespace mnc {
int* proposal_count_ptr(mnc_ctx* ctx);
}

using namespace mnc;

namespace {

struct HostBlob {
  std::vector<float> v;
};

struct DevBuf {
  void* p = nullptr;
  size_t cap = 0;
};

const char* kTrunk[13] = {"conv1_1", "conv1_2", "conv2_1", "conv2_2", "conv3_1", "conv3_2", "conv3_3",
                          "conv4_1", "conv4_2", "conv4_3", "conv5_1", "conv5_2", "conv5_3"};
const int kTrunkStage[13] = {0, 0, 1, 1, 2, 2, 2, 3, 3, 3, 4, 4, 4};
const bool kPoolAfter[13] = {false, true, false, true, false, false, true, false, false, true, false, false, false};

inline int pool_out(int n) { return (n - 2 + 1) / 2 + 1; }

void linear_taps(int n_dst, int n_src, double scale, int* lo, float* frac) {
  const double inv = 1.0 / scale;
  for (int i = 0; i < n_dst; ++i) {
    const float src = (float)(((double)i + 0.5) * inv - 0.5);
    long l = (long)std::floor((double)src);
    float f = (float)((double)src - (double)l);
    if (l < 0) { l = 0; f = 0.0f; }
    if (l >= n_src - 1) { l = n_src - 1; f = 0.0f; }
    lo[i] = (int)l;
    frac[i] = f;
  }
}

}

struct mnc_net {
  mnc_ctx* ctx = nullptr;
  mnc_ctx* ctx_b = nullptr;
  hipEvent_t ev_fork[2] = {nullptr, nullptr}, ev_join[2] = {nullptr, nullptr};
  mnc_net_config cfg;
  std::map<std::string, HostBlob> params;
  bool finalized = false;
  mnc_net* owner = nullptr;
  std::atomic<int> sharers{0};
  float* w_c3 = nullptr;
  void* w_conv[14] = {nullptr};
  bool packed_trunk = false;
  bool conv_fast[14] = {false};
  float* b_conv[14] = {nullptr};
  float *w_rpn = nullptr, *b_rpn = nullptr;
  struct Fc { void* w = nullptr; float* b = nullptr; int N = 0, K = 0, kind = 0; };
  Fc fc_maskest, fc_maskpred, fc6, fc7, fc6m, fc7m, fc_heads;
  int cap_ph = 0, cap_pw = 0, cap_src = 0;
  DevBuf img, taps, data, act[13], pooled[4], act12_pk, rpn_out, rpn_score, rpn_prob;
  float* rpn_bbox_p = nullptr;
  DevBuf rois, rois_ext, feat14, h_mask, m14, box7, mask7, f6, f6m, join, heads, boxes, masks, scores;
  DevBuf outblk;
  DevBuf hwc5;
  float* records() const { return (float*)((char*)outblk.p + 512); }
  int* counts() const { return (int*)outblk.p; }
  int* prop_count() const { return (int*)((char*)outblk.p + 256); }
  DevBuf feat14_sm, box7_sm, mask7_sm, f6_sm, f6m_sm;
  unsigned char* pin_img = nullptr; size_t pin_img_cap = 0;
  float* pin_out = nullptr; size_t pin_out_cap = 0;
  int H = 0, W = 0, OH = 0, OW = 0, fh = 0, fw = 0;
  float im_scale = 1.0f;
  int tap_key_h = -1, tap_key_w = -1;
  int last_r1 = 0, last_r2 = 0;
  bool fc_sm = true, fuse_pools = true;
  bool fuse_small = true;
  bool tail_done = false;
  bool in_flight = false;
  hipGraphExec_t gexec = nullptr;
  int graph_h = -1, graph_w = -1, seen_h = -1, seen_w = -1;
  unsigned long graph_gen = 0;
  void* render_dev = nullptr; void* render_pin = nullptr; size_t render_cap = 0;
  int vote_mode = MNC_VOTE_MV;
  double vote_binarize = 0.4;
};

namespace {

int dev_ensure(mnc_net* n, DevBuf* b, size_t bytes) {
  if (bytes <= b->cap) return MNC_OK;
  if (b->p) {
    int rc = mnc_dev_free(n->ctx, b->p);
    if (rc) return rc;
    b->p = nullptr; b->cap = 0;
  }
  const size_t want = bytes + (bytes >> 3) + 256;
  int rc = mnc_dev_alloc(n->ctx, want, &b->p);
  if (rc) return rc;
  b->cap = want;
  if (n->gexec) { (void)hipGraphExecDestroy(n->gexec); n->gexec = nullptr; n->graph_h = n->graph_w = -1; }
  return MNC_OK;
}

const HostBlob* find(mnc_net* n, const std::string& layer, int index) {
  auto it = n->params.find(layer + "/" + std::to_string(index));
  return it == n->params.end() ? nullptr : &it->second;
}

int upload(mnc_net* n, const std::vector<float>& v, float** out) {
  void* p = nullptr;
  int rc = mnc_dev_alloc(n->ctx, v.size() * 4, &p);
  if (rc) return rc;
  rc = mnc_h2d(n->ctx, p, v.data(), v.size() * 4);
  if (rc) return rc;
  *out = (float*)p;
  return MNC_OK;
}

#define NET_TRY(expr)        \
  do {                       \
    int rc__ = (expr);       \
    if (rc__) return rc__;   \
  } while (0)

int need(mnc_net* n, const char* layer, int index, size_t count, const HostBlob** out) {
  const HostBlob* b = find(n, layer, index);
  if (!b) {
    set_error("mnc_net: parameter %s/%d has not been set", layer, index);
    return MNC_ERR_STATE;
  }
  if (b->v.size() != count) {
    set_error("mnc_net: parameter %s/%d holds %zu values, the configured graph needs %zu", layer, index, b->v.size(), count);
    return MNC_ERR_INVALID;
  }
  *out = b;
  return MNC_OK;
}

static inline int conv_math(const mnc_net_config& c) { return c.math == 3 ? 1 : c.math; }
static inline int lowp_mode(int cm) { return cm == 1 ? 0 : cm == 2 ? 1 : 2; }
static inline int fc_math(const mnc_net_config& c) { return c.math == 3 ? 2 : c.math; }

int prepare_fc(mnc_net* n, const char* layer, int N, int K, int C, int PH, int PW, mnc_net::Fc* fc) {
  const HostBlob *w, *b;
  NET_TRY(need(n, layer, 0, (size_t)N * K, &w));
  NET_TRY(need(n, layer, 1, (size_t)N, &b));
  fc->N = N; fc->K = K;
  NET_TRY(upload(n, b->v, &fc->b));
  float* raw = nullptr;
  NET_TRY(upload(n, w->v, &raw));
  if (PH * PW > 1) {
    void* perm = nullptr;
    NET_TRY(mnc_dev_alloc(n->ctx, (size_t)N * K * 4, &perm));
    NET_TRY(mnc_pack_fc_weights(n->ctx, raw, (float*)perm, N, C, PH, PW));
    NET_TRY(mnc_dev_free(n->ctx, raw));
    raw = (float*)perm;
  }
  const bool big = 2.0 * n->cfg.post_nms_topn * (double)N * (double)K >= 2.0e9;
  const int fm = (n->cfg.math == 3 && K > 50000) ? 1 : fc_math(n->cfg);
  const bool bf = fm == 4 && K % 64 == 0 && big;
  const bool f16 = (fm == 2 && K % 64 == 0 && big) || bf;
  const bool x3 = !f16 && (fm == 1 || fm == 2) && K % 32 == 0 && big;
  fc->kind = bf ? 3 : f16 ? 2 : x3 ? 1 : 0;
  if (fc->kind == 0) { fc->w = raw; return MNC_OK; }
  void* packed = nullptr;
  NET_TRY(mnc_dev_alloc(n->ctx, (size_t)((N + 127) / 128) * 128 * K * (f16 ? 2 : 4), &packed));
  NET_TRY(bf ? mnc_pack_fc_bf16(n->ctx, raw, packed, N, K)
             : f16 ? mnc_pack_fc_f16(n->ctx, raw, packed, N, K) : mnc_pack_fc_bf16x3(n->ctx, raw, packed, N, K));
  NET_TRY(mnc_dev_free(n->ctx, raw));
  fc->w = packed;
  return MNC_OK;
}

int run_fc(mnc_ctx* ctx, const mnc_net::Fc& fc, const float* a, float* out, int M, int ldc, int act) {
  if (M == 0) return MNC_OK;
  if (fc.kind == 3) return mnc_fc_bf16(ctx, a, fc.w, fc.b, out, M, fc.N, fc.K, ldc, act);
  if (fc.kind == 2) return mnc_fc_f16(ctx, a, fc.w, fc.b, out, M, fc.N, fc.K, ldc, act);
  if (fc.kind == 1) return mnc_fc_bf16x3(ctx, a, fc.w, fc.b, out, M, fc.N, fc.K, ldc, act);
  return mnc_fc(ctx, a, (const float*)fc.w, fc.b, out, M, fc.N, fc.K, ldc, act);
}
int run_fc(mnc_net* n, const mnc_net::Fc& fc, const float* a, float* out, int M, int ldc, int act) {
  return run_fc(n->ctx, fc, a, out, M, ldc, act);
}
int sm_format(const mnc_net* n, const mnc_net::Fc& fc, int C) {
  if (!n->fc_sm) return 0;
  if (fc.kind == 2) return C % 64 == 0 ? 1 : 0;
  if (fc.kind == 1) return C % 32 == 0 ? 2 : 0;
  if (fc.kind == 3) return C % 64 == 0 ? 3 : 0;
  return 0;
}
int run_fc_sm(mnc_ctx* ctx, const mnc_net::Fc& fc, const float* a, const void* a_sm, int fmt, float* out, int M, int ldc, int act,
              void* out_sm = nullptr, int out_fmt = 0) {
  if (M == 0) return MNC_OK;
  if (!out_sm) out_fmt = 0;
  if (fc.kind == 2) return mnc_fc_f16_ex(ctx, fmt == 1 ? nullptr : a, fmt == 1 ? a_sm : nullptr, M, fc.w, fc.b, out, M, fc.N, fc.K, ldc,
                                         act, out_fmt ? out_sm : nullptr, out_fmt);
  if (fc.kind == 1) return mnc_fc_bf16x3_ex(ctx, fmt == 2 ? nullptr : a, fmt == 2 ? a_sm : nullptr, M, fc.w, fc.b, out, M, fc.N, fc.K,
                                            ldc, act, out_fmt ? out_sm : nullptr, out_fmt);
  if (fc.kind == 3) return mnc_fc_bf16_ex(ctx, fmt == 3 ? nullptr : a, fmt == 3 ? a_sm : nullptr, M, fc.w, fc.b, out, M, fc.N, fc.K, ldc,
                                          act, out_fmt ? out_sm : nullptr, out_fmt);
  return run_fc(ctx, fc, a, out, M, ldc, act);
}

int finalize(mnc_net* n) {
  if (n->finalized) return MNC_OK;
  const mnc_net_config& c = n->cfg;
  const HostBlob *w, *b;
  int cin = 3;
  for (int i = 0; i < 14; ++i) {
    const char* name = i < 13 ? kTrunk[i] : "rpn_conv_3x3";
    const int cout = i < 13 ? c.trunk_channels[kTrunkStage[i]] : c.rpn_channels;
    NET_TRY(need(n, name, 0, (size_t)cout * cin * 9, &w));
    NET_TRY(need(n, name, 1, (size_t)cout, &b));
    NET_TRY(upload(n, b->v, &n->b_conv[i]));
    if (i == 0) {
      NET_TRY(upload(n, w->v, &n->w_c3));
    } else {
      float* raw = nullptr;
      NET_TRY(upload(n, w->v, &raw));
      n->conv_fast[i] = cout % 32 == 0;
      if (n->conv_fast[i]) {
        const int cm = conv_math(c);
        const int pitch = c.winograd == 4 ? 288 : c.winograd ? 136 : 76;
        const size_t wbytes = cm == 0 ? (size_t)(cin / 8) * cout * pitch * 4 : mnc_conv3x3_lowp_weight_bytes(lowp_mode(cm), cout, cin);
        NET_TRY(mnc_dev_alloc(n->ctx, wbytes, &n->w_conv[i]));
        NET_TRY(cm == 0 ? (c.winograd == 4 ? mnc_pack_conv3x3_wino4(n->ctx, raw, (float*)n->w_conv[i], cout, cin)
                               : c.winograd ? mnc_pack_conv3x3_wino(n->ctx, raw, (float*)n->w_conv[i], cout, cin)
                                            : mnc_pack_conv3x3_weights(n->ctx, raw, (float*)n->w_conv[i], cout, cin))
                : cm == 1 ? mnc_pack_conv3x3_bf16x3(n->ctx, raw, n->w_conv[i], cout, cin)
                : cm == 4 ? mnc_pack_conv3x3_bf16(n->ctx, raw, n->w_conv[i], cout, cin)
                              : mnc_pack_conv3x3_f16(n->ctx, raw, n->w_conv[i], cout, cin));
      } else if (conv_math(c) == 2) {
        NET_TRY(mnc_dev_alloc(n->ctx, (size_t)9 * ((cin + 31) / 32) * 32 * cout * 2, &n->w_conv[i]));
        NET_TRY(mnc_pack_conv_weights_f16(n->ctx, raw, n->w_conv[i], cout, cin, 3, 3));
      } else {
        NET_TRY(mnc_dev_alloc(n->ctx, (size_t)cout * cin * 9 * 4, &n->w_conv[i]));
        NET_TRY(mnc_pack_conv_weights(n->ctx, raw, (float*)n->w_conv[i], cout, cin, 3, 3));
      }
      NET_TRY(mnc_dev_free(n->ctx, raw));
    }
    cin = cout;
  }
  n->packed_trunk = conv_math(c) != 0 && tune(n->ctx, T_PACKED_ACT, 1) != 0;
  for (int i = 1; i < 13; ++i) n->packed_trunk = n->packed_trunk && n->conv_fast[i];
  const int A = c.num_anchors, RC = c.rpn_channels;
  {
    const HostBlob *wc, *bc, *wb, *bb;
    NET_TRY(need(n, "rpn_cls_score", 0, (size_t)2 * A * RC, &wc));
    NET_TRY(need(n, "rpn_cls_score", 1, (size_t)2 * A, &bc));
    NET_TRY(need(n, "rpn_bbox_pred", 0, (size_t)4 * A * RC, &wb));
    NET_TRY(need(n, "rpn_bbox_pred", 1, (size_t)4 * A, &bb));
    std::vector<float> wcat(wc->v), bcat(bc->v);
    wcat.insert(wcat.end(), wb->v.begin(), wb->v.end());
    bcat.insert(bcat.end(), bb->v.begin(), bb->v.end());
    NET_TRY(upload(n, wcat, &n->w_rpn));
    NET_TRY(upload(n, bcat, &n->b_rpn));
  }
  const int C5 = c.trunk_channels[4], P = c.roi_size, S = c.mask_size, F = c.fc_dim, K = c.num_classes;
  NET_TRY(prepare_fc(n, "fc6_maskest", c.mask_fc, C5 * P * P, C5, P, P, &n->fc_maskest));
  NET_TRY(prepare_fc(n, "mask_pred", S * S, c.mask_fc, c.mask_fc, 1, 1, &n->fc_maskpred));
  NET_TRY(prepare_fc(n, "fc6", F, C5 * (P / 2) * (P / 2), C5, P / 2, P / 2, &n->fc6));
  NET_TRY(prepare_fc(n, "fc7", F, F, F, 1, 1, &n->fc7));
  NET_TRY(prepare_fc(n, "fc6_mask", F, C5 * (P / 2) * (P / 2), C5, P / 2, P / 2, &n->fc6m));
  NET_TRY(prepare_fc(n, "fc7_mask", F, F, F, 1, 1, &n->fc7m));
  {
    const char* names[3] = {"cls_score", "seg_cls_score", "bbox_pred"};
    const int widths[3] = {K, K, 4 * K};
    std::vector<float> W, B;
    for (int i = 0; i < 3; ++i) {
      NET_TRY(need(n, names[i], 0, (size_t)widths[i] * 2 * F, &w));
      NET_TRY(need(n, names[i], 1, (size_t)widths[i], &b));
      W.insert(W.end(), w->v.begin(), w->v.end());
      B.insert(B.end(), b->v.begin(), b->v.end());
    }
    n->fc_heads.N = 6 * K; n->fc_heads.K = 2 * F; n->fc_heads.kind = 0;
    float* dw = nullptr;
    NET_TRY(upload(n, W, &dw));
    n->fc_heads.w = dw;
    NET_TRY(upload(n, B, &n->fc_heads.b));
  }
  NET_TRY(mnc_ctx_sync(n->ctx));
  n->params.clear();
  n->finalized = true;
  return MNC_OK;
}

int ensure_buffers(mnc_net* n, int H, int W, int OH, int OW) {
  const mnc_net_config& c = n->cfg;
  NET_TRY(dev_ensure(n, &n->img, (size_t)H * W * 3));
  NET_TRY(dev_ensure(n, &n->taps, (size_t)(2 * OW + 2 * OH) * 4));
  NET_TRY(dev_ensure(n, &n->data, (size_t)3 * OH * OW * 4));
  int h = OH, w = OW, pi = 0;
  for (int i = 0; i < 13; ++i) {
    const int ch = c.trunk_channels[kTrunkStage[i]];
    NET_TRY(dev_ensure(n, &n->act[i], (size_t)ch * h * w * 4));
    if (kPoolAfter[i]) {
      h = pool_out(h); w = pool_out(w);
      NET_TRY(dev_ensure(n, &n->pooled[pi++], (size_t)ch * h * w * 4));
    }
  }
  const int A = c.num_anchors;
  if (n->packed_trunk) NET_TRY(dev_ensure(n, &n->act12_pk, (size_t)c.trunk_channels[4] * h * w * 4));
  NET_TRY(dev_ensure(n, &n->hwc5, (size_t)c.trunk_channels[4] * h * w * 4));
  NET_TRY(dev_ensure(n, &n->rpn_out, (size_t)c.rpn_channels * h * w * 4));
  NET_TRY(dev_ensure(n, &n->rpn_score, (size_t)6 * A * h * w * 4));
  NET_TRY(dev_ensure(n, &n->rpn_prob, (size_t)2 * A * h * w * 4));
  n->rpn_bbox_p = (float*)n->rpn_score.p + (size_t)2 * A * h * w;
  const int R = c.post_nms_topn, C5 = c.trunk_channels[4], P = c.roi_size, S = c.mask_size, F = c.fc_dim, K = c.num_classes;
  NET_TRY(dev_ensure(n, &n->rois, (size_t)R * 5 * 4));
  NET_TRY(dev_ensure(n, &n->rois_ext, (size_t)R * 5 * 4));
  NET_TRY(dev_ensure(n, &n->feat14, (size_t)R * P * P * C5 * 4));
  NET_TRY(dev_ensure(n, &n->h_mask, (size_t)R * c.mask_fc * 4));
  NET_TRY(dev_ensure(n, &n->m14, (size_t)R * P * P * 4));
  NET_TRY(dev_ensure(n, &n->box7, (size_t)R * (P / 2) * (P / 2) * C5 * 4));
  NET_TRY(dev_ensure(n, &n->mask7, (size_t)R * (P / 2) * (P / 2) * C5 * 4));
  if (sm_format(n, n->fc_maskest, C5)) NET_TRY(dev_ensure(n, &n->feat14_sm, (size_t)R * P * P * C5 * (n->fc_maskest.kind == 1 ? 4 : 2)));
  if (sm_format(n, n->fc6, C5)) NET_TRY(dev_ensure(n, &n->box7_sm, (size_t)R * (P / 2) * (P / 2) * C5 * (n->fc6.kind == 1 ? 4 : 2)));
  if (sm_format(n, n->fc6m, C5)) NET_TRY(dev_ensure(n, &n->mask7_sm, (size_t)R * (P / 2) * (P / 2) * C5 * (n->fc6m.kind == 1 ? 4 : 2)));
  NET_TRY(dev_ensure(n, &n->f6, (size_t)R * F * 4));
  NET_TRY(dev_ensure(n, &n->f6m, (size_t)R * F * 4));
  if (sm_format(n, n->fc7, F)) NET_TRY(dev_ensure(n, &n->f6_sm, (size_t)R * F * (n->fc7.kind == 1 ? 4 : 2)));
  if (sm_format(n, n->fc7m, F)) NET_TRY(dev_ensure(n, &n->f6m_sm, (size_t)R * F * (n->fc7m.kind == 1 ? 4 : 2)));
  NET_TRY(dev_ensure(n, &n->join, (size_t)R * 2 * F * 4));
  NET_TRY(dev_ensure(n, &n->heads, (size_t)2 * R * 6 * K * 4));
  NET_TRY(dev_ensure(n, &n->boxes, (size_t)2 * R * 4 * 4));
  NET_TRY(dev_ensure(n, &n->masks, (size_t)2 * R * S * S * 4));
  NET_TRY(dev_ensure(n, &n->scores, (size_t)2 * R * K * 4));
  const size_t rows = (size_t)(K - 1) * c.max_per_image;
  NET_TRY(dev_ensure(n, &n->outblk, 512 + rows * (6 + S * S) * 4));
  if ((size_t)H * W * 3 > n->pin_img_cap) {
    if (n->pin_img) NET_TRY(mnc_host_free(n->ctx, n->pin_img));
    n->pin_img = nullptr;
    NET_TRY(mnc_host_alloc(n->ctx, (size_t)H * W * 3 + 4096, (void**)&n->pin_img));
    n->pin_img_cap = (size_t)H * W * 3 + 4096;
    if (n->gexec) { (void)hipGraphExecDestroy(n->gexec); n->gexec = nullptr; n->graph_h = n->graph_w = -1; }
  }
  const size_t out_bytes = 512 + rows * (6 + S * S) * 4;
  if (out_bytes > n->pin_out_cap) {
    if (n->pin_out) NET_TRY(mnc_host_free(n->ctx, n->pin_out));
    n->pin_out = nullptr;
    NET_TRY(mnc_host_alloc(n->ctx, out_bytes, (void**)&n->pin_out));
    n->pin_out_cap = out_bytes;
    if (n->gexec) { (void)hipGraphExecDestroy(n->gexec); n->gexec = nullptr; n->graph_h = n->graph_w = -1; }
  }
  return MNC_OK;
}

int set_geometry(mnc_net* n, int H, int W) {
  const mnc_net_config& c = n->cfg;
  const int shortside = H < W ? H : W, longside = H < W ? W : H;
  double scale = (double)c.target_size / (double)shortside;
  if (std::nearbyint(scale * longside) > c.max_size) scale = (double)c.max_size / (double)longside;
  const int OH = (int)std::nearbyint(H * scale), OW = (int)std::nearbyint(W * scale);
  NET_TRY(ensure_buffers(n, H, W, OH, OW));
  n->H = H; n->W = W; n->OH = OH; n->OW = OW;
  n->im_scale = (float)scale;
  if (n->tap_key_h != H || n->tap_key_w != W) {
    std::vector<int> lo(OW > OH ? OW : OH);
    std::vector<float> fr(lo.size());
    std::vector<float> table((size_t)2 * OW + 2 * OH);
    linear_taps(OW, W, scale, lo.data(), fr.data());
    memcpy(table.data(), lo.data(), (size_t)OW * 4);
    memcpy(table.data() + OW, fr.data(), (size_t)OW * 4);
    linear_taps(OH, H, scale, lo.data(), fr.data());
    memcpy(table.data() + 2 * OW, lo.data(), (size_t)OH * 4);
    memcpy(table.data() + 2 * OW + OH, fr.data(), (size_t)OH * 4);
    NET_TRY(mnc_h2d(n->ctx, n->taps.p, table.data(), table.size() * 4));
    n->tap_key_h = H; n->tap_key_w = W;
  }
  return MNC_OK;
}

int conv3(mnc_net* n, int i, const float* in, float* out, int h, int w, int cin, int cout) {
  const mnc_net_config& c = n->cfg;
  const int cm = conv_math(c);
  if (!n->conv_fast[i]) {
    if (cm == 2) return mnc_conv2d_f16(n->ctx, in, n->w_conv[i], n->b_conv[i], nullptr, out, h, w, cin, cout, 3, 3, 1, 1, 1);
    return mnc_conv2d(n->ctx, in, (const float*)n->w_conv[i], n->b_conv[i], nullptr, out, h, w, cin, cout, 3, 3, 1, 1, 1);
  }
  if (cm == 0 && c.winograd == 4)
    return mnc_conv3x3_wino4(n->ctx, in, (const float*)n->w_conv[i], n->b_conv[i], out, h, w, cin, cout, 1);
  if (cm == 0 && c.winograd)
    return mnc_conv3x3_wino(n->ctx, in, (const float*)n->w_conv[i], n->b_conv[i], out, h, w, cin, cout, 1);
  if (cm == 0) return mnc_conv3x3(n->ctx, in, (const float*)n->w_conv[i], n->b_conv[i], out, h, w, cin, cout, 1);
  if (cm == 1) return mnc_conv3x3_bf16x3(n->ctx, in, n->w_conv[i], n->b_conv[i], out, h, w, cin, cout, 1);
  if (cm == 4) return mnc_conv3x3_bf16(n->ctx, in, n->w_conv[i], n->b_conv[i], out, h, w, cin, cout, 1);
  return mnc_conv3x3_f16(n->ctx, in, n->w_conv[i], n->b_conv[i], out, h, w, cin, cout, 1);
}

int run_trunk(mnc_net* n) {
  const mnc_net_config& c = n->cfg;
  mnc_ctx* ctx = n->ctx;
  const float* t = (const float*)n->taps.p;
  NET_TRY(mnc_prep_image(ctx, (const unsigned char*)n->img.p, n->H, n->W, c.pixel_means, (const int*)t, t + n->OW, n->OW,
                         (const int*)(t + 2 * n->OW), t + 2 * n->OW + n->OH, n->OH, (float*)n->data.p, n->OH, n->OW));
  int h = n->OH, w = n->OW, pi = 0, cin = 3;
  const float* cur = (const float*)n->data.p;
  if (n->packed_trunk) {
    const int mode = lowp_mode(conv_math(c));
    const void* pc = cur;
    for (int i = 0; i < 13; ++i) {
      const int cout = c.trunk_channels[kTrunkStage[i]];
      void* out = n->act[i].p;
      if (kPoolAfter[i] && i > 0 && n->fuse_small) {
        void* p = n->pooled[pi++].p;
        NET_TRY(mnc_conv3x3_lowp_pool(ctx, mode, pc, n->w_conv[i], n->b_conv[i], p, h, w, cin, cout, 1));
        h = pool_out(h); w = pool_out(w);
        pc = p; cin = cout;
        continue;
      }
      if (i == 0) NET_TRY(mnc_conv3x3_c3_fmt(ctx, cur, n->w_c3, n->b_conv[0], out, h, w, cout, 1, mode + 1));
      else if (i < 12) NET_TRY(mnc_conv3x3_lowp(ctx, mode, pc, n->w_conv[i], n->b_conv[i], out, nullptr, h, w, cin, cout, 1));
      else NET_TRY(mnc_conv3x3_lowp(ctx, mode, pc, n->w_conv[i], n->b_conv[i], n->act12_pk.p, (float*)out, h, w, cin, cout, 1));
      pc = out; cin = cout;
      if (kPoolAfter[i]) {
        void* p = n->pooled[pi++].p;
        NET_TRY(mode == 1 ? mnc_maxpool2_c8_f16(ctx, pc, p, cout, h, w)
                          : mode == 2 ? mnc_maxpool2_c8_bf16(ctx, pc, p, cout, h, w) : mnc_maxpool2_c8_bf16x3(ctx, pc, p, cout, h, w));
        h = pool_out(h); w = pool_out(w);
        pc = p;
      }
    }
    cur = (const float*)pc;
  } else
  for (int i = 0; i < 13; ++i) {
    const int cout = c.trunk_channels[kTrunkStage[i]];
    float* out = (float*)n->act[i].p;
    if (kPoolAfter[i] && i > 0 && conv_math(c) == 0 && c.winograd && n->conv_fast[i]) {
      float* p = (float*)n->pooled[pi++].p;
      NET_TRY(c.winograd == 4 ? mnc_conv3x3_wino4_pool(ctx, cur, (const float*)n->w_conv[i], n->b_conv[i], p, h, w, cin, cout, 1)
                              : mnc_conv3x3_wino_pool(ctx, cur, (const float*)n->w_conv[i], n->b_conv[i], p, h, w, cin, cout, 1));
      h = pool_out(h); w = pool_out(w);
      cur = p; cin = cout;
      continue;
    }
    if (i == 0) NET_TRY(mnc_conv3x3_c3(ctx, cur, n->w_c3, n->b_conv[0], out, h, w, cout, 1));
    else NET_TRY(conv3(n, i, cur, out, h, w, cin, cout));
    cur = out; cin = cout;
    if (kPoolAfter[i]) {
      float* p = (float*)n->pooled[pi++].p;
      NET_TRY(mnc_maxpool2_c8(ctx, cur, p, cout, h, w));
      h = pool_out(h); w = pool_out(w);
      cur = p;
    }
  }
  n->fh = h; n->fw = w;
  if (n->fuse_small)
    NET_TRY(c8_to_hwc_launch(ctx, (const float*)n->act[12].p, (float*)n->hwc5.p, c.trunk_channels[4], h, w));
  const int A = c.num_anchors;
  if (n->packed_trunk && n->conv_fast[13])
    NET_TRY(mnc_conv3x3_lowp(ctx, lowp_mode(conv_math(c)), n->act12_pk.p, n->w_conv[13], n->b_conv[13], nullptr, (float*)n->rpn_out.p, h, w,
                             cin, c.rpn_channels, 1));
  else NET_TRY(conv3(n, 13, cur, (float*)n->rpn_out.p, h, w, cin, c.rpn_channels));
  if (n->fuse_small) {
    NET_TRY(mnc_rpn_heads(ctx, (const float*)n->rpn_out.p, n->w_rpn, n->b_rpn, (float*)n->rpn_score.p, (float*)n->rpn_prob.p, h, w,
                          c.rpn_channels, A));
  } else {
    NET_TRY(mnc_conv1x1_to_nchw(ctx, (const float*)n->rpn_out.p, n->w_rpn, n->b_rpn, (float*)n->rpn_score.p, h, w, c.rpn_channels,
                                6 * A));
    NET_TRY(mnc_rpn_softmax(ctx, (const float*)n->rpn_score.p, (float*)n->rpn_prob.p, A, h, w));
  }
  NET_TRY(mnc_proposal(ctx, (const float*)n->rpn_prob.p, (const float*)n->rpn_bbox_p, A, h, w, c.anchors, c.feat_stride,
                       (float)n->OH, (float)n->OW, n->im_scale, c.pre_nms_topn, c.post_nms_topn, c.rpn_nms_thresh,
                       c.rpn_min_size, (float*)n->rois.p, nullptr));
  return MNC_OK;
}

int run_stage(mnc_net* n, const float* rois, int R, bool second, int row0) {
  const mnc_net_config& c = n->cfg;
  mnc_ctx* ctx = n->ctx;
  const int C5 = c.trunk_channels[4], P = c.roi_size, S = c.mask_size, F = c.fc_dim, K = c.num_classes;
  const float* conv5 = (const float*)n->act[12].p;
  float* feat14 = (float*)n->feat14.p;
  const int sm_feat = sm_format(n, n->fc_maskest, C5), sm_box = sm_format(n, n->fc6, C5), sm_mask = sm_format(n, n->fc6m, C5);
  const bool fork0 = n->ctx_b && ctx->profiling == 0 && R > 0;
  const bool lowp_pairs = n->fuse_small && n->fuse_pools && sm_box == sm_mask && !fork0 && n->fc6.kind != 0 && n->fc6m.kind == n->fc6.kind &&
                          n->fc7.kind == n->fc6.kind && n->fc7m.kind == n->fc6.kind && n->fc6.K == n->fc6m.K &&
                          sm_format(n, n->fc7, F) == sm_format(n, n->fc7m, F) && R > 0;
  const bool sm_only = lowp_pairs && sm_box != 0;
  const bool feat_sm_only = sm_only && sm_feat != 0 && (P * P * C5) % 64 == 0 && roi_warp_sm_only_ok(ctx, C5, second ? 0 : 1);
  if (feat_sm_only) feat14 = nullptr;
  if (n->fuse_small)
    NET_TRY(roi_warp_from_hwc(ctx, (const float*)n->hwc5.p, C5, n->fh, n->fw, rois, R, P, P, c.spatial_scale, second ? 0 : 1, feat14,
                              n->feat14_sm.p, sm_feat));
  else
    NET_TRY(mnc_roi_warp_sm(ctx, conv5, C5, n->fh, n->fw, rois, R, P, P, c.spatial_scale, second ? 0 : 1, feat14, n->feat14_sm.p,
                            sm_feat));
  float* masks = (float*)n->masks.p + (size_t)row0 * S * S;
  NET_TRY(run_fc_sm(ctx, n->fc_maskest, feat14, n->feat14_sm.p, sm_feat, (float*)n->h_mask.p, R, c.mask_fc, 1));
  NET_TRY(run_fc(n, n->fc_maskpred, (const float*)n->h_mask.p, masks, R, S * S, 2));
  NET_TRY(mnc_mask_resize(ctx, masks, (float*)n->m14.p, R, S, S, P, P));
  float* join = (float*)n->join.p;
  const bool one_pass = n->fuse_pools && sm_box == sm_mask;
  if (one_pass)
    NET_TRY(mnc_box_mask_pool_ex(ctx, feat14, sm_feat ? n->feat14_sm.p : nullptr, sm_feat, (const float*)n->m14.p,
                                 sm_only ? nullptr : (float*)n->box7.p, sm_only ? nullptr : (float*)n->mask7.p, R, P, P, C5, n->box7_sm.p,
                                 n->mask7_sm.p, sm_box));
  const bool fork = n->ctx_b && ctx->profiling == 0 && R > 0;
  mnc_ctx* cb = fork ? n->ctx_b : ctx;
  const int si = second ? 1 : 0;
  if (fork) {
    MNC_HIP_TRY(hipEventRecord(n->ev_fork[si], ctx->stream));
    MNC_HIP_TRY(hipStreamWaitEvent(cb->stream, n->ev_fork[si], 0));
  }
  if (!one_pass) NET_TRY(mnc_maxpool2_rhwc_sm(cb, feat14, (float*)n->box7.p, R, P, P, C5, n->box7_sm.p, sm_box));
  const int sm_f6 = sm_format(n, n->fc7, F), sm_f6m = sm_format(n, n->fc7m, F);
  if (n->fuse_small && one_pass && !fork && n->fc6.kind == 0 && n->fc6m.kind == 0 && n->fc7.kind == 0 && n->fc7m.kind == 0 &&
      n->fc6.K == n->fc6m.K) {
    NET_TRY(mnc_fc_pair(ctx, (const float*)n->box7.p, (const float*)n->fc6.w, n->fc6.b, (float*)n->f6.p, (const float*)n->mask7.p,
                        (const float*)n->fc6m.w, n->fc6m.b, (float*)n->f6m.p, R, F, n->fc6.K, F, 1));
    NET_TRY(mnc_fc_pair(ctx, (const float*)n->f6.p, (const float*)n->fc7.w, n->fc7.b, join + F, (const float*)n->f6m.p,
                        (const float*)n->fc7m.w, n->fc7m.b, join, R, F, F, 2 * F, 1));
  } else if (lowp_pairs) {
    const int mode = n->fc6.kind == 1 ? 0 : n->fc6.kind == 2 ? 1 : 2;
    const bool pre6 = sm_box != 0, pre7 = sm_f6 != 0;
    NET_TRY(mnc_fc_lowp_pair(ctx, mode, pre6 ? nullptr : (const float*)n->box7.p, pre6 ? n->box7_sm.p : nullptr,
                             pre6 ? nullptr : (const float*)n->mask7.p, pre6 ? n->mask7_sm.p : nullptr, R, n->fc6.w, n->fc6m.w, n->fc6.b,
                             n->fc6m.b, (float*)n->f6.p, (float*)n->f6m.p, R, F, n->fc6.K, F, 1, pre7 ? n->f6_sm.p : nullptr,
                             pre7 ? n->f6m_sm.p : nullptr, sm_f6));
    NET_TRY(mnc_fc_lowp_pair(ctx, mode, pre7 ? nullptr : (const float*)n->f6.p, pre7 ? n->f6_sm.p : nullptr,
                             pre7 ? nullptr : (const float*)n->f6m.p, pre7 ? n->f6m_sm.p : nullptr, R, n->fc7.w, n->fc7m.w, n->fc7.b,
                             n->fc7m.b, join + F, join, R, F, F, 2 * F, 1, nullptr, nullptr, 0));
  } else {
  NET_TRY(run_fc_sm(cb, n->fc6, (const float*)n->box7.p, n->box7_sm.p, sm_box, (float*)n->f6.p, R, F, 1, n->f6_sm.p, sm_f6));
  NET_TRY(run_fc_sm(cb, n->fc7, (const float*)n->f6.p, n->f6_sm.p, n->fc6.kind ? sm_f6 : 0, join + F, R, 2 * F, 1));
  if (fork) MNC_HIP_TRY(hipEventRecord(n->ev_join[si], cb->stream));
  if (!one_pass)
    NET_TRY(mnc_mask_pool_sm(ctx, feat14, (const float*)n->m14.p, (float*)n->mask7.p, R, P, P, C5, 1, n->mask7_sm.p, sm_mask));
  NET_TRY(run_fc_sm(ctx, n->fc6m, (const float*)n->mask7.p, n->mask7_sm.p, sm_mask, (float*)n->f6m.p, R, F, 1, n->f6m_sm.p, sm_f6m));
  NET_TRY(run_fc_sm(ctx, n->fc7m, (const float*)n->f6m.p, n->f6m_sm.p, n->fc6m.kind ? sm_f6m : 0, join, R, 2 * F, 1));
  if (fork) MNC_HIP_TRY(hipStreamWaitEvent(ctx->stream, n->ev_join[si], 0));
  }
  float* heads = (float*)n->heads.p + (size_t)row0 * 6 * K;
  float* scores = (float*)n->scores.p + (size_t)row0 * K;
  n->tail_done = false;
  if (n->fuse_small && R > 0 && K <= 64 && n->fc_heads.kind == 0 && 2.0 * R * 6.0 * K * n->fc_heads.K < 2.0e9) {
    ctx->defer_reduce = true;
    int rc = run_fc(n, n->fc_heads, join, heads, R, 6 * K, 0);
    ctx->defer_reduce = false;
    if (rc) return rc;
    NET_TRY(heads_finish_launch(ctx, ctx->deferred_part, ctx->deferred_splits, n->fc_heads.b, heads, 6 * K, R, K, scores, rois,
                                (float)n->OH, (float)n->OW, second ? nullptr : (float*)n->rois_ext.p, (const float*)n->rois.p,
                                (const float*)n->rois_ext.p, n->im_scale, n->H, n->W, second ? (float*)n->boxes.p : nullptr,
                                second ? proposal_count_ptr(ctx) : nullptr, second ? n->prop_count() : nullptr));
    n->tail_done = second;
    return MNC_OK;
  }
  NET_TRY(run_fc(n, n->fc_heads, join, heads, R, 6 * K, 0));
  if (R) NET_TRY(mnc_softmax_rows_ld(ctx, heads + K, 6 * K, scores, R, K));
  if (!second)
    NET_TRY(mnc_stage_bridge(ctx, rois, heads + 2 * K, 6 * K, scores, K, R, K, (float)n->OH, (float)n->OW,
                             (float*)n->rois_ext.p));
  return MNC_OK;
}

int run_heads_and_vote(mnc_net* n, int r1) {
  const mnc_net_config& c = n->cfg;
  mnc_ctx* ctx = n->ctx;
  const int S = c.mask_size, K = c.num_classes;
  NET_TRY(run_stage(n, (const float*)n->rois.p, r1, false, 0));
  NET_TRY(run_stage(n, (const float*)n->rois_ext.p, r1, true, r1));
  if (!n->tail_done)
    NET_TRY(detect_tail_launch(ctx, (const float*)n->rois.p, r1, (const float*)n->rois_ext.p, r1, n->im_scale, n->H, n->W,
                               (float*)n->boxes.p, proposal_count_ptr(ctx), n->prop_count()));
  const int rows = (K - 1) * c.max_per_image;
  NET_TRY(mnc_vote_instances_ex(ctx, n->vote_mode, (const float*)n->boxes.p, (const float*)n->masks.p, (const float*)n->scores.p,
                                2 * r1, K, S, c.max_per_image, c.vote_nms_thresh, c.vote_iou_thresh, n->vote_binarize, n->H, n->W,
                                n->records(), rows, n->counts()));
  n->last_r1 = r1; n->last_r2 = r1;
  return MNC_OK;
}

int enqueue_outputs(mnc_net* n) {
  const mnc_net_config& c = n->cfg;
  const size_t rec_bytes = (size_t)c.max_per_image * (6 + c.mask_size * c.mask_size) * 4;
  NET_TRY(mnc_d2h_async(n->ctx, n->pin_out, n->outblk.p, 512 + rec_bytes));
  return MNC_OK;
}

int enqueue_image(mnc_net* n) {
  NET_TRY(mnc_h2d_async(n->ctx, n->img.p, n->pin_img, (size_t)n->H * n->W * 3));
  NET_TRY(run_trunk(n));
// ... 8 lines not shown
  NET_TRY(finalize(n));
  MNC_HIP_TRY(hipSetDevice(n->ctx->device));
  if (n->in_flight) MNC_HIP_TRY(hipStreamSynchronize(n->ctx->stream));
  NET_TRY(set_geometry(n, H, W));
  memcpy(n->pin_img, bgr_host, (size_t)H * W * 3);
  n->in_flight = true;
  hipStream_t s = n->ctx->stream;
  const bool want_graph = n->cfg.use_graph && n->ctx->profiling == 0;
  if (n->gexec && n->graph_gen != arena_gen(n)) {
    (void)hipGraphExecDestroy(n->gexec);
    n->gexec = nullptr; n->graph_h = n->graph_w = -1; n->seen_h = n->seen_w = -1;
  }
  if (want_graph && n->gexec && n->graph_h == H && n->graph_w == W) {
    MNC_HIP_TRY(hipGraphLaunch(n->gexec, s));
    return MNC_OK;
  }
  if (want_graph && n->seen_h == H && n->seen_w == W) {
    if (n->gexec) { (void)hipGraphExecDestroy(n->gexec); n->gexec = nullptr; }
    hipGraph_t g = nullptr;
    MNC_HIP_TRY(hipStreamBeginCapture(s, hipStreamCaptureModeRelaxed));
    const unsigned long gen0 = arena_gen(n);
    n->ctx->capturing = true;
    if (n->ctx_b) n->ctx_b->capturing = true;
    int rc = enqueue_image(n);
    n->ctx->capturing = false;
    if (n->ctx_b) n->ctx_b->capturing = false;
    hipError_t e = hipStreamEndCapture(s, &g);
    if (rc == MNC_OK && e == hipSuccess && g && gen0 == arena_gen(n)) {
      e = hipGraphInstantiate(&n->gexec, g, nullptr, nullptr, 0);
      (void)hipGraphDestroy(g);
      if (e == hipSuccess) {
        n->graph_h = H; n->graph_w = W;
        n->graph_gen = gen0;
        MNC_HIP_TRY(hipGraphLaunch(n->gexec, s));
        return MNC_OK;
      }
      n->gexec = nullptr;
      (void)hipGetLastError();
      n->cfg.use_graph = 0;
    } else {
      if (g) (void)hipGraphDestroy(g);
      (void)hipGetLastError();
      if (e != hipSuccess) n->cfg.use_graph = 0;
    }
  }
  n->seen_h = H; n->seen_w = W;
  return enqueue_image(n);
}

}

extern "C" {

int mnc_net_default_config(mnc_net_config* cfg) {
  MNC_REQUIRE(cfg, "mnc_net_default_config: null pointer");
  memset(cfg, 0, sizeof(*cfg));
  const int tc[5] = {64, 128, 256, 512, 512};
  memcpy(cfg->trunk_channels, tc, sizeof(tc));
  cfg->rpn_channels = 512;
  cfg->num_anchors = 9;
  const float a[36] = {-84, -40, 99, 55,  -176, -88, 191, 103,  -360, -184, 375, 199,  -56, -56, 71, 71,  -120, -120, 135, 135,
                       -248, -248, 263, 263,  -36, -80, 51, 95,  -80, -168, 95, 183,  -168, -344, 183, 359};
  memcpy(cfg->anchors, a, sizeof(a));
  cfg->feat_stride = 16;
  cfg->pre_nms_topn = 6000; cfg->post_nms_topn = 300;
  cfg->rpn_nms_thresh = 0.7f; cfg->rpn_min_size = 16.0f;
  cfg->mask_fc = 256; cfg->mask_size = 21;
  cfg->fc_dim = 4096;
  cfg->num_classes = 21;
  cfg->roi_size = 14;
  cfg->spatial_scale = 0.0625f;
  cfg->target_size = 600; cfg->max_size = 1000;
  cfg->pixel_means[0] = 102.9801; cfg->pixel_means[1] = 115.9465; cfg->pixel_means[2] = 122.7717;
  cfg->max_per_image = 100;
  cfg->vote_nms_thresh = 0.3f; cfg->vote_iou_thresh = 0.5f;
  cfg->math = 0;
  cfg->use_graph = 1;
  cfg->winograd = 4;
  cfg->conventions.maskpool_thresh = 0.4f;
  cfg->conventions.inherit = 1;
  clear_error();
  return MNC_OK;
}

int mnc_net_create(mnc_ctx* ctx, const mnc_net_config* cfg, mnc_net** out) {
  MNC_REQUIRE(ctx && cfg && out, "mnc_net_create: null pointer");
  *out = nullptr;
  for (int i = 0; i < 5; ++i)
    MNC_REQUIRE(cfg->trunk_channels[i] > 0 && cfg->trunk_channels[i] % 8 == 0 && cfg->trunk_channels[i] <= 4096,
                "mnc_net_create: trunk width %d must be a positive multiple of 8", cfg->trunk_channels[i]);
  MNC_REQUIRE(cfg->trunk_channels[0] <= 512, "mnc_net_create: conv1 width %d > 512", cfg->trunk_channels[0]);
  MNC_REQUIRE(cfg->rpn_channels > 0 && cfg->rpn_channels % 8 == 0 && cfg->num_anchors > 0 && cfg->num_anchors <= 16,
              "mnc_net_create: RPN shape");
  MNC_REQUIRE(cfg->roi_size > 0 && cfg->roi_size % 2 == 0 && cfg->mask_size >= 2 && cfg->num_classes >= 2 &&
              cfg->post_nms_topn > 0 && cfg->max_per_image > 0 && cfg->fc_dim > 0 && cfg->mask_fc > 0,
              "mnc_net_create: head shape");
  MNC_REQUIRE(cfg->num_classes <= 64, "mnc_net_create: num_classes %d > 64 (the result header holds 64 counts)", cfg->num_classes);
  MNC_REQUIRE(cfg->math >= 0 && cfg->math <= 4, "mnc_net_create: math must be 0 (fp32), 1 (bf16x3), 2 (f16), 3 (mixed) or 4 (bf16)");
  MNC_REQUIRE(cfg->target_size > 0 && cfg->max_size >= cfg->target_size, "mnc_net_create: target_size / max_size");
  if (!cfg->conventions.inherit) {
    int rc = mnc_ctx_set_layer_conventions(ctx, &cfg->conventions);
    if (rc) return rc;
  }
  MNC_REQUIRE(cfg->math != 0 || cfg->winograd != 4 ||
                  (double)cfg->trunk_channels[0] * cfg->max_size * (double)cfg->max_size * 4.0 < 2147483648.0,
              "mnc_net_create: winograd = 4 with max_size %d: a %d-channel %dx%d map exceeds the F(4x4) kernel's 2 GB operand range; "
              "use winograd = 2", cfg->max_size, cfg->trunk_channels[0], cfg->max_size, cfg->max_size);
  mnc_net* n = new (std::nothrow) mnc_net();
  if (!n) { set_error("mnc_net_create: out of host memory"); return MNC_ERR_NOMEM; }
  n->ctx = ctx;
  n->cfg = *cfg;
  n->cfg.conventions = ctx->conv;
  n->fc_sm = tune(ctx, T_FC_SM, 1) != 0;
  n->fuse_pools = tune(ctx, T_FUSE_POOLS, 1) != 0;
  n->fuse_small = tune(ctx, T_FUSE_SMALL, 1) != 0;
  if (tune(ctx, T_BRANCH_STREAMS, 0) == 1) {
    if (mnc_ctx_create(&n->ctx_b, ctx->device) != MNC_OK) n->ctx_b = nullptr;
    if (n->ctx_b) (void)mnc_ctx_set_layer_conventions(n->ctx_b, &ctx->conv);
    for (int i = 0; i < 2 && n->ctx_b; ++i) {
      if (hipEventCreateWithFlags(&n->ev_fork[i], hipEventDisableTiming) != hipSuccess ||
          hipEventCreateWithFlags(&n->ev_join[i], hipEventDisableTiming) != hipSuccess) {
        (void)mnc_ctx_destroy(n->ctx_b);
        n->ctx_b = nullptr;
      }
    }
  }
  *out = n;
  clear_error();
  return MNC_OK;
}

int mnc_net_create_shared(mnc_ctx* ctx, mnc_net* parent, mnc_net** out) {
  MNC_REQUIRE(ctx && parent && out, "mnc_net_create_shared: null pointer");
  *out = nullptr;
  MNC_REQUIRE(!parent->owner, "mnc_net_create_shared: `parent` borrows its weights itself; share with the net that owns them");
  MNC_REQUIRE(ctx->device == parent->ctx->device, "mnc_net_create_shared: context on device %d, the weights live on device %d",
              ctx->device, parent->ctx->device);
  MNC_REQUIRE(ctx != parent->ctx, "mnc_net_create_shared: give the sharing net its own context (stream and scratch arenas)");
  NET_TRY(finalize(parent));
  mnc_net* n = nullptr;
  {
    mnc_net_config cfg = parent->cfg;
    int rc = mnc_net_create(ctx, &cfg, &n);
    if (rc) return rc;
    rc = mnc_ctx_set_layer_conventions(ctx, &parent->cfg.conventions);
    if (rc) { (void)mnc_net_destroy(n); return rc; }
    n->cfg.conventions = ctx->conv;
  }
  n->owner = parent;
  ++parent->sharers;
  n->w_c3 = parent->w_c3;
  for (int i = 0; i < 14; ++i) {
    n->w_conv[i] = parent->w_conv[i];
    n->b_conv[i] = parent->b_conv[i];
    n->conv_fast[i] = parent->conv_fast[i];
  }
  n->packed_trunk = parent->packed_trunk;
  n->w_rpn = parent->w_rpn; n->b_rpn = parent->b_rpn;
  n->fc_maskest = parent->fc_maskest; n->fc_maskpred = parent->fc_maskpred;
  n->fc6 = parent->fc6; n->fc7 = parent->fc7; n->fc6m = parent->fc6m; n->fc7m = parent->fc7m; n->fc_heads = parent->fc_heads;
  n->finalized = true;
  *out = n;
  clear_error();
  return MNC_OK;
}

int mnc_net_set_param(mnc_net* net, const char* layer, int index, const float* data_host, size_t count) {
  MNC_REQUIRE(net && layer && data_host && index >= 0 && index <= 1 && count > 0, "mnc_net_set_param: bad argument");
  MNC_REQUIRE(!net->owner, "mnc_net_set_param: this net shares another net's weights (mnc_net_create_shared)");
  MNC_REQUIRE(!net->finalized, "mnc_net_set_param: the weights of this net are already packed (set them before the first image)");
  try {
    HostBlob& b = net->params[std::string(layer) + "/" + std::to_string(index)];
    b.v.assign(data_host, data_host + count);
  } catch (const std::exception&) {
    set_error("mnc_net_set_param: out of host memory for %s/%d (%zu values)", layer, index, count);
    return MNC_ERR_NOMEM;
  }
  clear_error();
  return MNC_OK;
}

int mnc_net_load_file(mnc_net* net, const char* path) {
  MNC_REQUIRE(net && path, "mnc_net_load_file: null pointer");
  FILE* f = fopen(path, "rb");
  MNC_REQUIRE(f, "mnc_net_load_file: cannot open %s", path);
  long file_bytes = 0;
  if (fseek(f, 0, SEEK_END) == 0) file_bytes = ftell(f);
  rewind(f);
  char magic[8];
  unsigned n = 0;
  bool ok = file_bytes >= 12 && fread(magic, 1, 8, f) == 8 && memcmp(magic, "MNCW0001", 8) == 0 && fread(&n, 4, 1, f) == 1;
  int rc = MNC_OK;
  const char* why = "is not a complete MNCW0001 file";
  try {
    std::vector<float> v;
    for (unsigned i = 0; ok && i < n; ++i) {
      unsigned short len = 0;
      unsigned char idx = 0, nd = 0;
      char name[256];
      unsigned dims[8];
      ok = fread(&len, 2, 1, f) == 1 && len < sizeof(name) && fread(name, 1, len, f) == len && fread(&idx, 1, 1, f) == 1 &&
           fread(&nd, 1, 1, f) == 1 && nd <= 8 && fread(dims, 4, nd, f) == nd;
      if (!ok) break;
      name[len] = 0;
      const bool skip = idx > 1;
      const size_t left = (size_t)(file_bytes - ftell(f)) / 4;
      size_t count = 1;
      for (int d = 0; d < nd && ok; ++d) {
        if (dims[d] == 0 || count > left / dims[d]) ok = false;
        else count *= dims[d];
      }
      if (!ok) { why = "declares a blob larger than the file"; break; }
      v.resize(count);
      ok = fread(v.data(), 4, count, f) == count;
      if (!ok) break;
      if (!skip) rc = mnc_net_set_param(net, name, idx, v.data(), count);
      if (rc) break;
    }
  } catch (const std::exception&) {
    fclose(f);
    set_error("mnc_net_load_file: out of host memory while reading %s", path);
    return MNC_ERR_NOMEM;
  }
  fclose(f);
  if (rc) return rc;
  MNC_REQUIRE(ok, "mnc_net_load_file: %s %s", path, why);
  clear_error();
  return MNC_OK;
}

int mnc_forward_image_async(mnc_net* net, const unsigned char* bgr_host, int H, int W, float** d_records, int** d_counts) {
  int rc = launch_image(net, bgr_host, H, W);
  if (rc) return rc;
  if (d_records) *d_records = net->records();
  if (d_counts) *d_counts = net->counts();
  clear_error();
  return MNC_OK;
}

int mnc_net_set_voting(mnc_net* net, int mode, double binarize_thresh) {
  MNC_REQUIRE(net, "mnc_net_set_voting: null pointer");
  MNC_REQUIRE(mode == MNC_VOTE_MV || mode == MNC_VOTE_IMAGE, "mnc_net_set_voting: mode %d is not MNC_VOTE_MV / MNC_VOTE_IMAGE", mode);
  if (mode != net->vote_mode || binarize_thresh != net->vote_binarize) {
    if (net->gexec) {
      MNC_HIP_TRY(hipSetDevice(net->ctx->device));
      if (net->in_flight) MNC_HIP_TRY(hipStreamSynchronize(net->ctx->stream));
      (void)hipGraphExecDestroy(net->gexec);
      net->gexec = nullptr; net->graph_h = net->graph_w = -1;
    }
    net->vote_mode = mode;
    net->vote_binarize = binarize_thresh;
  }
  clear_error();
  return MNC_OK;
}

int mnc_net_fetch(mnc_net* net, float* records_host, int record_cap, int* counts_host) {
  MNC_REQUIRE(net && records_host && counts_host && record_cap >= 0, "mnc_net_fetch: null pointer");
  MNC_REQUIRE(net->H > 0, "mnc_net_fetch: no image has been launched on this net");
  const mnc_net_config& c = net->cfg;
  const int D = 6 + c.mask_size * c.mask_size;
  MNC_REQUIRE(record_cap <= (c.num_classes - 1) * c.max_per_image, "mnc_net_fetch: record_cap %d > %d", record_cap,
              (c.num_classes - 1) * c.max_per_image);
  MNC_HIP_TRY(hipSetDevice(net->ctx->device));
  MNC_HIP_TRY(hipStreamSynchronize(net->ctx->stream));
  net->in_flight = false;
  const int* head = (const int*)net->pin_out;
  const int n_prop = *(const int*)((const char*)net->pin_out + 256);
  if (n_prop < c.post_nms_topn) {
    NET_TRY(run_heads_and_vote(net, n_prop));
    NET_TRY(enqueue_outputs(net));
    MNC_HIP_TRY(hipStreamSynchronize(net->ctx->stream));
  }
  const int R = head[0];
  for (int k = 0; k < c.num_classes; ++k) counts_host[k] = head[k];
  const int first = c.max_per_image < record_cap ? c.max_per_image : record_cap;
  const int have = R < first ? R : first;
  memcpy(records_host, (const char*)net->pin_out + 512, (size_t)have * D * 4);
  if (have < record_cap) memset(records_host + (size_t)have * D, 0, (size_t)(record_cap - have) * D * 4);
  if (R > first && record_cap > first) {
    const int more = (R < record_cap ? R : record_cap) - first;
    NET_TRY(mnc_d2h(net->ctx, records_host + (size_t)first * D, (const float*)net->records() + (size_t)first * D,
                    (size_t)more * D * 4));
  }
  clear_error();
  return MNC_OK;
}

int mnc_net_render(mnc_net* net, double vis_thresh, double binarize_thresh, float alpha, int* inst_host, int* cls_host,
                   unsigned char* inst_rgb_host, unsigned char* cls_rgb_host, unsigned char* overlay_rgb_host, int* kept_host) {
  MNC_REQUIRE(net, "mnc_net_render: null pointer");
  if (net->H <= 0) {
    set_error("mnc_net_render: no image has been forwarded on this net");
    return MNC_ERR_STATE;
  }
  const mnc_net_config& c = net->cfg;
  mnc_ctx* ctx = net->ctx;
  MNC_HIP_TRY(hipSetDevice(ctx->device));
  MNC_HIP_TRY(hipStreamSynchronize(ctx->stream));
  net->in_flight = false;
  if (*(const int*)((const char*)net->pin_out + 256) < c.post_nms_topn) {
    NET_TRY(run_heads_and_vote(net, *(const int*)((const char*)net->pin_out + 256)));
    NET_TRY(enqueue_outputs(net));
  }
  const size_t px = (size_t)net->H * net->W;
  const size_t o_cls = px * 4, o_irgb = o_cls + px * 4, o_crgb = o_irgb + px * 3, o_ovl = o_crgb + px * 3,
               o_kept = (o_ovl + px * 3 + 255) & ~(size_t)255, total = o_kept + 256;
  if (total > net->render_cap) {
    if (net->render_dev) MNC_HIP_TRY(hipFree(net->render_dev));
    if (net->render_pin) MNC_HIP_TRY(hipHostFree(net->render_pin));
    net->render_dev = net->render_pin = nullptr;
    net->render_cap = 0;
    if (hipMalloc(&net->render_dev, total) != hipSuccess || hipHostMalloc(&net->render_pin, total, hipHostMallocDefault) != hipSuccess) {
      (void)hipGetLastError();
      if (net->render_dev) (void)hipFree(net->render_dev);
      net->render_dev = net->render_pin = nullptr;
      set_error("mnc_net_render: allocating %zu bytes failed", total);
      return MNC_ERR_NOMEM;
    }
    net->render_cap = total;
  }
  char* d = (char*)net->render_dev;
  char* h = (char*)net->render_pin;
  const int rows = (c.num_classes - 1) * c.max_per_image;
  NET_TRY(mnc_render_records(ctx, net->records(), net->counts(), rows, c.num_classes, c.mask_size, vis_thresh, binarize_thresh,
                             net->H, net->W, (const unsigned char*)net->img.p, alpha, inst_host ? (int*)d : nullptr,
                             cls_host ? (int*)(d + o_cls) : nullptr, inst_rgb_host ? (unsigned char*)(d + o_irgb) : nullptr,
                             cls_rgb_host ? (unsigned char*)(d + o_crgb) : nullptr,
                             overlay_rgb_host ? (unsigned char*)(d + o_ovl) : nullptr, (int*)(d + o_kept)));
  struct Out { void* host; size_t off, bytes; };
  const Out outs[] = {{inst_host, 0, px * 4}, {cls_host, o_cls, px * 4}, {inst_rgb_host, o_irgb, px * 3},
                      {cls_rgb_host, o_crgb, px * 3}, {overlay_rgb_host, o_ovl, px * 3}, {kept_host, o_kept, sizeof(int)}};
  for (const Out& o : outs)
    if (o.host) NET_TRY(mnc_d2h_async(ctx, h + o.off, d + o.off, o.bytes));
  MNC_HIP_TRY(hipStreamSynchronize(ctx->stream));
  for (const Out& o : outs)
    if (o.host) memcpy(o.host, h + o.off, o.bytes);
  clear_error();
  return MNC_OK;
}

int mnc_net_masks(mnc_net* net, double score_thresh, double binarize_thresh, void* info_host, int info_cap, void* bits_host,
                  size_t bits_cap, size_t* bits_bytes) {
  MNC_REQUIRE(net && info_host && info_cap >= 0, "mnc_net_masks: null pointer");
  if (net->H <= 0) {
    set_error("mnc_net_masks: no image has been forwarded on this net");
    return MNC_ERR_STATE;
  }
  const mnc_net_config& c = net->cfg;
  mnc_ctx* ctx = net->ctx;
  MNC_HIP_TRY(hipSetDevice(ctx->device));
  MNC_HIP_TRY(hipStreamSynchronize(ctx->stream));
  net->in_flight = false;
  if (*(const int*)((const char*)net->pin_out + 256) < c.post_nms_topn) {
    NET_TRY(run_heads_and_vote(net, *(const int*)((const char*)net->pin_out + 256)));
    NET_TRY(enqueue_outputs(net));
    MNC_HIP_TRY(hipStreamSynchronize(ctx->stream));
  }
  const int cap = (c.num_classes - 1) * c.max_per_image, R = *(const int*)net->pin_out;
  const int rows = R < 0 ? 0 : R < cap ? R : cap;
  MNC_REQUIRE(info_cap >= rows, "mnc_net_masks: info_cap %d is below the image's %d instances", info_cap, rows);
  void* d_info = nullptr; void* d_bits = nullptr;
  NET_TRY(mnc_mask_records(ctx, net->records(), net->counts(), rows, c.num_classes, c.mask_size, score_thresh, binarize_thresh,
                           net->H, net->W, &d_info, bits_host ? &d_bits : nullptr));
  NET_TRY(mnc_d2h(ctx, info_host, d_info, sizeof(mnc_mask_head) + (size_t)rows * sizeof(mnc_mask_info)));
  const size_t need = (size_t)((const mnc_mask_head*)info_host)->bits_bytes;
  if (bits_bytes) *bits_bytes = need;
  if (bits_host) {
    MNC_REQUIRE(bits_cap >= need, "mnc_net_masks: bits_cap %zu is below the %zu bytes of the masks", bits_cap, need);
    if (need) NET_TRY(mnc_d2h(ctx, bits_host, d_bits, need));
  }
  clear_error();
  return MNC_OK;
}

int mnc_forward_image(mnc_net* net, const unsigned char* bgr_host, int H, int W, float* records_host, int record_cap,
                      int* counts_host) {
  MNC_REQUIRE(net && records_host && counts_host && record_cap >= 0, "mnc_forward_image: null pointer");
  int rc = launch_image(net, bgr_host, H, W);
  if (rc) return rc;
  return mnc_net_fetch(net, records_host, record_cap, counts_host);
}

int mnc_net_blob(mnc_net* net, const char* name, void** d_ptr, int* dims, int* ndim) {
  MNC_REQUIRE(net && name && d_ptr && dims && ndim, "mnc_net_blob: null pointer");
  const mnc_net_config& c = net->cfg;
  const std::string s(name);
  const int A = c.num_anchors, R1 = net->last_r1, R2 = net->last_r2;
  auto set = [&](void* p, int n, int a, int b, int cc, int d) {
    *d_ptr = p; *ndim = n; dims[0] = a; dims[1] = b; dims[2] = cc; dims[3] = d;
    return MNC_OK;
  };
  if (s == "data") return set(net->data.p, 4, 1, 3, net->OH, net->OW);
  if (s == "conv5_3") return set(net->act[12].p, 4, 1, c.trunk_channels[4], net->fh, net->fw);
  if (s == "rpn_cls_prob_reshape") return set(net->rpn_prob.p, 4, 1, 2 * A, net->fh, net->fw);
  if (s == "rpn_bbox_pred") return set(net->rpn_bbox_p, 4, 1, 4 * A, net->fh, net->fw);
  if (s == "rois") return set(net->rois.p, 2, R1, 5, 0, 0);
  if (s == "rois_ext") return set(net->rois_ext.p, 2, R2, 5, 0, 0);
  if (s == "mask_proposal") return set(net->masks.p, 4, R1 + R2, 1, c.mask_size, c.mask_size);
  if (s == "seg_cls_prob") return set(net->scores.p, 2, R1 + R2, c.num_classes, 0, 0);
  if (s == "boxes") return set(net->boxes.p, 2, R1 + R2, 4, 0, 0);
  if (s == "head_scores") return set(net->heads.p, 2, R1 + R2, 6 * c.num_classes, 0, 0);
  if (s == "records") return set(net->records(), 2, (c.num_classes - 1) * c.max_per_image, 6 + c.mask_size * c.mask_size, 0, 0);
  set_error("mnc_net_blob: unknown blob %s", name);
  return MNC_ERR_INVALID;
}

int mnc_net_destroy(mnc_net* net) {
  if (!net) return MNC_OK;
  if (net->sharers > 0) {
    set_error("mnc_net_destroy: %d net(s) created with mnc_net_create_shared still use this net's weights; destroy them first",
              net->sharers.load());
    return MNC_ERR_STATE;
  }
  mnc_ctx* ctx = net->ctx;
  (void)hipSetDevice(ctx->device);
  (void)hipStreamSynchronize(ctx->stream);
  if (net->gexec) (void)hipGraphExecDestroy(net->gexec);
  DevBuf* bufs[] = {&net->img, &net->taps, &net->data, &net->rpn_out, &net->rpn_score, &net->rpn_prob, &net->rois,
                    &net->rois_ext, &net->feat14, &net->h_mask, &net->m14, &net->box7, &net->mask7, &net->f6, &net->f6m, &net->join,
                    &net->feat14_sm, &net->box7_sm, &net->mask7_sm, &net->f6_sm, &net->f6m_sm,
                    &net->heads, &net->boxes, &net->masks, &net->scores, &net->outblk, &net->hwc5, &net->act12_pk};
  for (DevBuf* b : bufs) if (b->p) (void)hipFree(b->p);
  for (auto& b : net->act) if (b.p) (void)hipFree(b.p);
  for (auto& b : net->pooled) if (b.p) (void)hipFree(b.p);
  if (net->owner) {
    --net->owner->sharers;
  } else {
    void* singles[] = {net->w_c3, net->w_rpn, net->b_rpn};
    for (void* p : singles) if (p) (void)hipFree(p);
    for (int i = 0; i < 14; ++i) {
      if (net->w_conv[i]) (void)hipFree(net->w_conv[i]);
      if (net->b_conv[i]) (void)hipFree(net->b_conv[i]);
    }
    mnc_net::Fc* fcs[] = {&net->fc_maskest, &net->fc_maskpred, &net->fc6, &net->fc7, &net->fc6m, &net->fc7m, &net->fc_heads};
    for (mnc_net::Fc* f : fcs) {
      if (f->w) (void)hipFree(f->w);
      if (f->b) (void)hipFree(f->b);
    }
  }
  if (net->pin_img) (void)hipHostFree(net->pin_img);
  if (net->pin_out) (void)hipHostFree(net->pin_out);
  if (net->render_dev) (void)hipFree(net->render_dev);
  if (net->render_pin) (void)hipHostFree(net->render_pin);
  for (int i = 0; i < 2; ++i) {
    if (net->ev_fork[i]) (void)hipEventDestroy(net->ev_fork[i]);
    if (net->ev_join[i]) (void)hipEventDestroy(net->ev_join[i]);
  }
  if (net->ctx_b) (void)mnc_ctx_destroy(net->ctx_b);
  delete net;
  clear_error();
  return MNC_OK;
}

}
```

mnc_amd/csrc/tune.h:

```cpp
#pragma once
#include <climits>

namespace mnc {
#define MNC_TUNE_KEYS(X)                                                                                                          \
  X(CONV_COT) X(CONV_ROWS) X(CONV_KSPLIT) X(CONV_ABL) X(CONV1X1_TILE) X(CONV2D_WIDE) X(WINO_ROWS) X(WINO_TAIL) X(WINO_V) X(WINO_VAR)  \
  X(WINO_DMA) X(WINO_XCD) X(CONVX3_TILE) X(FC_NOTAIL) X(FC_TILE) X(FC_ABL) X(FC_DMA) X(PLAN) X(FC_RANGE_K) X(FC_SLOTS) X(FC_EVEN) X(FC_SPLIT_DIV) X(WINO_FILL) X(CONVX3_P0MIN) X(CONVX3_P1MIN) X(FC_DMA_ABL) X(FC_DMA_WAVES)    \
  X(FC_NO256) X(FCX3_TILE) X(FC_ORDER) X(FCX3_ABL) X(FC_SM) X(PACKED_ACT) X(FUSE_POOLS) X(BRANCH_STREAMS) X(TOPK_SINGLE_WG)           \
  X(ROI_SM_VARIANT) X(ROI_WARP_VARIANT) X(FC_REDUCE) X(WINO_F4) X(FUSE_SMALL) X(FCX3_WIDE) X(FC_HALF) X(WINO_STREAM) X(FC_MFMA16) X(WINO_MFMA16) X(ROI_ROW_SEGS)
enum TuneKey {
#define MNC_TUNE_ENUM(n) T_##n,
  MNC_TUNE_KEYS(MNC_TUNE_ENUM)
#undef MNC_TUNE_ENUM
  T_COUNT
};
constexpr int kTuneUnset = INT_MIN;

inline bool tune_set(const int* t, TuneKey k) { return t[k] != kTuneUnset; }
inline int tune(const int* t, TuneKey k, int dflt) { return t[k] != kTuneUnset ? t[k] : dflt; }
inline bool plan_latency(const int* t) { return tune(t, T_PLAN, 0) == 1; }

static inline int cdiv(long a, long b) { return (int)((a + b - 1) / b); }
}
```

mnc_amd/engine.py:

```python
import ctypes
import importlib
import os
from collections import OrderedDict
from collections.abc import Mapping

import numpy as np

from . import _lib, install_paths, prototxt
from .devarray import DeviceArray

WINOGRAD_DEFAULT = "4"


def winograd_mode(value):
    import os
    if value is None:
        value = os.environ.get("MNC_CONV_WINOGRAD", WINOGRAD_DEFAULT)
    if value is True:
        return 4
    if value is False:
        return 0
    v = int(value)
    if v not in (0, 1, 2, 4):
        raise ValueError("winograd must be 0 (direct), 2 (F(2x2,3x3)) or 4 (F(4x4,3x3)), got %r" % (value,))
# ... 617 lines not shown
    @staticmethod
    def _conv_geometry(L):
        cp = L.msg.get1("convolution_param")
        for key in ("kernel_h", "kernel_w", "pad_h", "pad_w", "stride_h", "stride_w"):
            if cp.get1(key) is not None:
                raise NotImplementedError("Convolution %s: %s is not supported (square kernel_size / pad / stride only)"
                                          % (L.name, key))
        if cp.get1("dilation", 1) != 1:
            raise NotImplementedError("Convolution %s: dilation %r is not supported" % (L.name, cp.get1("dilation")))
        if cp.get1("group", 1) != 1:
            raise NotImplementedError("Convolution %s: group %r is not supported" % (L.name, cp.get1("group")))
        if cp.get1("kernel_size") is None:
            raise NotImplementedError("Convolution %s: kernel_size is required" % L.name)
        return cp.get1("kernel_size"), cp.get1("pad", 0), cp.get1("stride", 1), cp.get1("num_output"), cp.get1("bias_term", True)

    def _conv_kind(self, L):
        k, pad, stride, cout, _ = self._conv_geometry(L)
        first = L.bottoms[0] in self.inputs
        if first:
            return "c3" if (k == 3 and pad == 1 and stride == 1) else "stem"
        if k == 3 and pad == 1 and stride == 1 and cout % 32 == 0 and L.residual is None:
            return "fast3x3"
        if k == 1 and pad == 0 and stride == 1 and not L.relu and L.bn is None and L.scale is None and L.residual is None \
                and self._rpn_head_conv(L):
            return "nchw1x1"
        return "general"

    def _conv_is_general(self, L):
        return self._conv_kind(L) == "general"

    def _rpn_head_conv(self, L):
        cons = [self._layers[i].type for i in self._consumers.get(L.tops[0], [])]
        return bool(cons) and all(t in ("Reshape", "Python", "Softmax") for t in cons)

    @staticmethod
    def _is_pool2(L):
        p = L.msg.get1("pooling_param")
        return (p.get1("pool", "MAX") == "MAX" and p.get1("kernel_size") == 2 and p.get1("stride") == 2
                and p.get1("pad", 0) == 0)

    def _bind_layers(self):
        for i, L in enumerate(self._layers):
            if L.skip:
                continue
            binder = getattr(self, "_bind_" + L.type, None)
            if binder is None:
                raise NotImplementedError("layer type %r (%s) is not supported by the MI355X engine" % (L.type, L.name))
            L.run = binder(L, i)

    def _h(self):
        return self._ctx.h

    def _folded_conv_params(self, L):
        _, _, _, cout, _ = self._conv_geometry(L)
        blobs = self._layer_weights(L)
        W = np.asarray(blobs[0], dtype=F32)
        b = np.asarray(blobs[1], dtype=F32) if len(blobs) > 1 and blobs[1] is not None else np.zeros(cout, F32)
        self.params[L.name] = [_Param(W), _Param(b)] if len(blobs) > 1 and blobs[1] is not None else [_Param(W)]
        if L.bn is None and L.scale is None:
            return W, b
        a, c = np.ones(cout, np.float64), np.zeros(cout, np.float64)
        if L.bn is not None:
            mean, var, factor = [np.asarray(x, dtype=np.float64) for x in self._layer_weights(L.bn)[:3]]
            bp = L.bn.msg.get1("batch_norm_param")
            eps = float(bp.get1("eps", 1e-5)) if bp is not None else 1e-5
            f = float(factor.reshape(-1)[0])
            inv = 0.0 if f == 0.0 else 1.0 / f
            a = 1.0 / np.sqrt(var.reshape(-1) * inv + eps)
            c = -mean.reshape(-1) * inv * a
            self.params[L.bn.name] = [_Param(np.asarray(x, dtype=F32)) for x in self._layer_weights(L.bn)[:3]]
        if L.scale is not None:
            sw = self._layer_weights(L.scale)
            gamma = np.asarray(sw[0], dtype=np.float64).reshape(-1)
            beta = np.asarray(sw[1], dtype=np.float64).reshape(-1) if len(sw) > 1 and sw[1] is not None else np.zeros(cout)
            a, c = a * gamma, c * gamma + beta
            self.params[L.scale.name] = [_Param(np.asarray(x, dtype=F32)) for x in sw if x is not None]
        Wf = (W.astype(np.float64) * a[:, None, None, None]).astype(F32)
        bf = (b.astype(np.float64) * a + c).astype(F32)
        return Wf, bf

    def _bind_Convolution(self, L, i):
        k, pad, stride, cout, _ = self._conv_geometry(L)
        kind = self._conv_kind(L)
        W, b = self._folded_conv_params(L)
        cin = W.shape[1]
        key = tuple(L.param_names) if all(L.param_names) and L.param_names else (L.name,)
        d_b = self._dev_param(key + ("b",), lambda: self._upload(b))
        bot, top = self.blobs[L.bottoms[0]], self.blobs[L.out_name or L.tops[0]]
        relu = 1 if L.relu else 0
        if kind == "c3":
            d_w = self._dev_param(key + ("w",), lambda: self._upload(W))

            def run():
                N, _, H, Wd = bot.shape
                src = bot.dev_in("plain")
                top.reshape(N, cout, H, Wd)
                pk = _PACKED_OF.get(self.conv_math, "c8h")
                dst = top.dev_out(pk if L.out_h else "c8")
                ob = _PACKED[pk][0] if L.out_h else 4
                for n in range(N):
                    if L.out_h:
                        _lib.call("mnc_conv3x3_c3_fmt", self._h(), src + n * 3 * H * Wd * 4, d_w, d_b,
                                  dst + n * cout * H * Wd * ob, H, Wd, cout, relu, _PACKED[pk][1] + 1)
                    else:
                        _lib.call("mnc_conv3x3_c3", self._h(), src + n * 3 * H * Wd * 4, d_w, d_b, dst + n * cout * H * Wd * 4,
                                  H, Wd, cout, relu)
            return run
        if kind == "stem":
            if cin != 3 or W.shape[2] != W.shape[3]:
                raise NotImplementedError("Convolution %s on the input blob: 3 channels, square kernel" % L.name)
            mfma = (self.conv_math == "f16" and k in (3, 5, 7) and cout % 32 == 0 and os.environ.get("MNC_STEM_F16", "1") != "0")
            if mfma:
                def build_stem():
                    raw = self._upload(W)
                    packed = self._ctx.alloc(((3 * k + 1) // 2) * (cout // 32) * 1024)
                    _lib.call("mnc_pack_conv_stem_f16", self._h(), raw, packed, cout, k)
                    self._ctx.free(raw)
                    return packed
                d_w = self._dev_param(key + ("w", "stem_f16"), build_stem)
            else:
                d_w = self._dev_param(key + ("w",), lambda: self._upload(W))

            def run():
                N, _, H, Wd = bot.shape
                OH, OW = (H + 2 * pad - k) // stride + 1, (Wd + 2 * pad - k) // stride + 1
                src = bot.dev_in("plain")
                top.reshape(N, cout, OH, OW)
                dst = top.dev_out("c8h" if L.out_h else "c8")
                ob = 2 if L.out_h else 4
                for n in range(N):
                    _lib.call("mnc_conv_stem_f16" if mfma else "mnc_conv_stem_c3_fmt", self._h(), src + n * 3 * H * Wd * 4, d_w, d_b,
                              dst + n * cout * OH * OW * ob, H, Wd, cout, k, stride, pad, relu, 1 if L.out_h else 0)
            return run
        if kind == "fast3x3":
            x3 = self.conv_math in ("bf16x3", "f16", "bf16")
            pitch, pack, conv = (84, "mnc_pack_conv3x3_f16", "mnc_conv3x3_f16") if self.conv_math == "f16" else \
                                (84, "mnc_pack_conv3x3_bf16", "mnc_conv3x3_bf16") if self.conv_math == "bf16" else \
                                (84, "mnc_pack_conv3x3_bf16x3", "mnc_conv3x3_bf16x3") if x3 else \
                                (288, "mnc_pack_conv3x3_wino4", "mnc_conv3x3_wino4") if self._wino == 4 else \
                                (136, "mnc_pack_conv3x3_wino", "mnc_conv3x3_wino") if self._wino == 2 else \
                                (76, "mnc_pack_conv3x3_weights", "mnc_conv3x3")

            def build():
                raw = self._upload(W)
                nbytes = (cin // 8) * cout * pitch * 4
                if x3:
                    nbytes = max(nbytes, ((cin + 15) // 16) * (cout // 32) * (4 if self.conv_math == "bf16x3" else 2) * 4608)
                packed = self._ctx.alloc(nbytes)
                _lib.call(pack, self._h(), raw, packed, cout, cin)
                self._ctx.free(raw)
                return packed
            d_w = self._dev_param(key + ("w", self.conv_math, ("wino%d" % self._wino) if (self._winograd and not x3) else "direct"), build)

            def run():
                N, _, H, Wd = bot.shape
                pk = _PACKED_OF.get(self.conv_math)
                in_h = pk is not None and bot._dev_valid and bot.layout == pk
                src = bot.dev_in(pk if in_h else "c8")
                if L.fused_pool and pk is not None:
                    if not in_h:
                        src = bot.dev_in(pk)
                    OH, OW = _pool_out(H), _pool_out(Wd)
                    top.reshape(N, cout, OH, OW)
                    dst = top.dev_out(pk)
                    eb, mode = _PACKED[pk]
                    for n in range(N):
                        _lib.call("mnc_conv3x3_lowp_pool", self._h(), mode, src + n * cin * H * Wd * eb, d_w, d_b,
                                  dst + n * cout * OH * OW * eb, H, Wd, cin, cout, relu)
                    return
                if L.fused_pool:
                    OH, OW = _pool_out(H), _pool_out(Wd)
                    top.reshape(N, cout, OH, OW)
                    dst = top.dev_out("c8")
                    for n in range(N):
                        _lib.call("mnc_conv3x3_wino4_pool" if self._wino == 4 else "mnc_conv3x3_wino_pool", self._h(), src + n * cin * H * Wd * 4, d_w, d_b,
                                  dst + n * cout * OH * OW * 4, H, Wd, cin, cout, relu)
                    return
                top.reshape(N, cout, H, Wd)
                if in_h or L.out_h:
                    dst = top.dev_out(pk if L.out_h else "c8")
                    eb = _PACKED[pk][0]
                    ib, ob = (eb if in_h else 4), (eb if L.out_h else 4)
                    for n in range(N):
                        _lib.call(conv + "_pk", self._h(), src + n * cin * H * Wd * ib, d_w, d_b,
                                  dst + n * cout * H * Wd * ob, H, Wd, cin, cout, relu, 1 if in_h else 0, 1 if L.out_h else 0)
                    return
                dst = top.dev_out("c8")
                for n in range(N):
                    _lib.call(conv, self._h(), src + n * cin * H * Wd * 4, d_w, d_b, dst + n * cout * H * Wd * 4, H, Wd, cin,
                              cout, relu)
            return run
        if kind == "nchw1x1":
            d_w = self._dev_param(key + ("w",), lambda: self._upload(W.reshape(cout, cin)))

            def run():
                N, _, H, Wd = bot.shape
                src = bot.dev_in("c8")
                top.reshape(N, cout, H, Wd)
                dst = top.dev_out("plain")
                for n in range(N):
                    _lib.call("mnc_conv1x1_to_nchw", self._h(), src + n * cin * H * Wd * 4, d_w, d_b,
                              dst + n * cout * H * Wd * 4, H, Wd, cin, cout)
            return run
        if cin % 8 or cout % 8:
            raise NotImplementedError("Convolution %s: channel counts must be multiples of 8 (got %d -> %d)" % (L.name, cin, cout))
        kh, kw = W.shape[2], W.shape[3]

        f16 = self.conv_math == "f16"
        conv2d = "mnc_conv2d_f16" if f16 else "mnc_conv2d"
        if self._conv_fast1x1(L):
            return self._bind_conv1x1(L, W, d_b, key, bot, top, stride, relu)

        def build_general():
            raw = self._upload(W)
            packed = self._ctx.alloc(kh * kw * ((cin + 31) // 32) * 32 * cout * 2 if f16 else W.nbytes)
            _lib.call("mnc_pack_conv_weights_f16" if f16 else "mnc_pack_conv_weights", self._h(), raw, packed, cout, cin, kh, kw)
            self._ctx.free(raw)
            return packed
        d_w = self._dev_param(key + ("w", "general", "f16" if f16 else "fp32"), build_general)
        res = self.blobs[L.residual] if L.residual else None

        def run():
            N, _, H, Wd = bot.shape
            OH, OW = (H + 2 * pad - kh) // stride + 1, (Wd + 2 * pad - kw) // stride + 1
            src = bot.dev_in("c8")
            rsrc = res.dev_in("c8") if res is not None else None
            if res is not None and tuple(res.shape) != (N, cout, OH, OW):
                raise ValueError("Convolution %s: residual %r has shape %r, expected %r" % (L.name, res.name, res.shape,
                                                                                            (N, cout, OH, OW)))
            top.reshape(N, cout, OH, OW)
            dst = top.dev_out("c8")
            for n in range(N):
                _lib.call(conv2d, self._h(), src + n * cin * H * Wd * 4, d_w, d_b,
                          (rsrc + n * cout * OH * OW * 4) if rsrc is not None else None, dst + n * cout * OH * OW * 4, H, Wd, cin,
                          cout, kh, kw, stride, pad, relu)
        return run

    def _bind_conv1x1(self, L, W, d_b, key, bot, top, stride, relu):
        cout, cin = int(W.shape[0]), int(W.shape[1])
        f16 = self.conv_math == "f16"

        def build():
            raw = self._upload(W.reshape(cout, cin))
            packed = self._ctx.alloc(cin * ((cout + 31) // 32) * 32 * (2 if f16 else 4))
            _lib.call("mnc_pack_conv1x1", self._h(), raw, packed, cout, cin, 1 if f16 else 0)
            self._ctx.free(raw)
            return packed
        d_w = self._dev_param(key + ("w", "1x1", "f16" if f16 else "fp32"), build)
        res = self.blobs[L.residual] if L.residual else None

        def run():
            N, _, H, Wd = bot.shape
            OH, OW = (H - 1) // stride + 1, (Wd - 1) // stride + 1
            if res is not None and tuple(res.shape) != (N, cout, OH, OW):
                raise ValueError("Convolution %s: residual %r has shape %r, expected %r" % (L.name, res.name, res.shape,
                                                                                            (N, cout, OH, OW)))
            if not f16:
                src = bot.dev_in("c8")
                rsrc = res.dev_in("c8") if res is not None else None
                top.reshape(N, cout, OH, OW)
                dst = top.dev_out("c8")
                for n in range(N):
                    _lib.call("mnc_conv1x1", self._h(), src + n * cin * H * Wd * 4, d_w, d_b,
                              (rsrc + n * cout * OH * OW * 4) if rsrc is not None else None, dst + n * cout * OH * OW * 4,
                              H, Wd, cin, cout, stride, relu)
                return
            src = bot.dev_in("c8h")
            res_h = res is not None and res._dev_valid and res.layout == "c8h"
            rsrc = res.dev_in("c8h" if res_h else "c8") if res is not None else None
            rb, ob = (2 if res_h else 4), (2 if L.out_h else 4)
            top.reshape(N, cout, OH, OW)
            dst = top.dev_out("c8h" if L.out_h else "c8")
            for n in range(N):
                _lib.call("mnc_conv1x1_f16_pk", self._h(), src + n * cin * H * Wd * 2, d_w, d_b,
                          (rsrc + n * cout * OH * OW * rb) if rsrc is not None else None, dst + n * cout * OH * OW * ob,
                          H, Wd, cin, cout, stride, relu, 1 if res_h else 0, 1 if L.out_h else 0)
        return run

    def _bind_ReLU(self, L, i):
        raise NotImplementedError("stand-alone ReLU %s (only in-place ReLU after Convolution/InnerProduct)" % L.name)

    def _bind_Dropout(self, L, i):
        if L.tops[0] == L.bottoms[0]:
            return None
        bot, top = self.blobs[L.bottoms[0]], self.blobs[L.tops[0]]

        def run():
            src = bot.dev_in("plain")
            top.reshape(*bot.shape)
            if bot.count:
                _lib.call("mnc_copy2d", self._h(), top.dev_out("plain"), bot.shape[-1], src, bot._ld() if len(bot.shape) == 2
                          else bot.shape[-1], bot.count // bot.shape[-1], bot.shape[-1])
            else:
                top.dev_out("plain")
        return run

    def _bind_Pooling(self, L, i):
        bot, top = self.blobs[L.bottoms[0]], self.blobs[L.tops[0]]
        if not self._is_pool2(L):
            p = L.msg.get1("pooling_param")
            if p.get1("pool", "MAX") != "MAX":
                raise NotImplementedError("Pooling %s: only MAX" % L.name)
            k, stride, pad = p.get1("kernel_size"), p.get1("stride", 1), p.get1("pad", 0)

            def out_size(n):
                o = -(-(n + 2 * pad - k) // stride) + 1
                return o - 1 if pad > 0 and (o - 1) * stride >= n + pad else o

            def run_general():
                N, C, H, W = bot.shape
                half = bot._dev_valid and bot.layout == "c8h"
                lay, eb = ("c8h", 2) if half else ("c8", 4)
                src = bot.dev_in(lay)
                OH, OW = out_size(H), out_size(W)
                top.reshape(N, C, OH, OW)
                dst = top.dev_out(lay)
                for n in range(N):
                    _lib.call("mnc_maxpool_c8_f16" if half else "mnc_maxpool_c8", self._h(), src + n * C * H * W * eb,
                              dst + n * C * OH * OW * eb, C, H, W, k, stride, pad)
            return run_general

        def run():
            if bot._dev_valid and (bot.layout == "c8" or bot.layout in _PACKED):
                N, C, H, W = bot.shape
                lay = bot.layout
                eb = _PACKED[lay][0] if lay in _PACKED else 4
                fn = {"c8": "mnc_maxpool2_c8", "c8h": "mnc_maxpool2_c8_f16", "c8x": "mnc_maxpool2_c8_bf16x3", "c8b": "mnc_maxpool2_c8_bf16"}[lay]
                src = bot.dev_in(lay)
                OH, OW = _pool_out(H), _pool_out(W)
                top.reshape(N, C, OH, OW)
                dst = top.dev_out(lay)
                for n in range(N):
                    _lib.call(fn, self._h(), src + n * C * H * W * eb, dst + n * C * OH * OW * eb, C, H, W)
            else:
                R, C, PH, PW = bot.shape
                if PH % 2 or PW % 2:
                    raise NotImplementedError("Pooling %s on per-RoI features: odd size %dx%d (MAX 2x2/2 needs even sizes)"
                                              % (L.name, PH, PW))
                top.reshape(R, C, PH // 2, PW // 2)
                K = C * (PH // 2) * (PW // 2)
                fmt = self._sm_format(top.name, R, K, C) if R else 0
# ... 830 lines not shown
```

Baseline: 267.5 images/s.

## Add split-phase Winograd F(4,3) conv using batched MFMA GEMM for wide layers

Adds a three-phase Winograd F(4x4,3x3) convolution: an input-transform kernel writes 36 transformed planes to a workspace, a new batched mode of the MFMA FC GEMM multiplies each plane by pre-transformed weights, and an output-transform kernel applies bias, ReLU and optional 2x2 max-pool. By default it is selected for layers with at least 512 input and output channels and enough tiles, meaning conv4/conv5 and the RPN conv. The goal is to run the channel reduction on the tuned GEMM path instead of the fused Winograd kernel. In exchange, the transformed tensors make an extra round trip through global memory and need a workspace buffer plus separately packed weights.

Result: faster. 271.5 images/s (median of 6 runs) (+1.5%).

```diff
diff --git a/include/mnc_hip.h b/include/mnc_hip.h
--- a/include/mnc_hip.h
+++ b/include/mnc_hip.h
@@ -237,6 +237,13 @@
                               int H, int W, int Cin, int Cout, int relu);
 MNC_API int mnc_conv3x3_wino4_pool(mnc_ctx* ctx, const float* d_in_c8, const float* d_w_packed, const float* d_bias,
                                    float* d_out_pooled_c8, int H, int W, int Cin, int Cout, int relu);
+MNC_API int mnc_pack_conv3x3_wino4_split(mnc_ctx* ctx, const float* d_oihw, float* d_packed, int Cout, int Cin);
+MNC_API size_t mnc_conv3x3_wino4_split_ws_bytes(int H, int W, int Cin, int Cout);
+MNC_API int mnc_conv3x3_wino4_split_selected(mnc_ctx* ctx, int H, int W, int Cin, int Cout);
+MNC_API int mnc_conv3x3_wino4_split(mnc_ctx* ctx, const float* d_in_c8, const float* d_w_split, const float* d_bias, float* d_out_c8,
+                                    void* d_ws, int H, int W, int Cin, int Cout, int relu);
+MNC_API int mnc_conv3x3_wino4_split_pool(mnc_ctx* ctx, const float* d_in_c8, const float* d_w_split, const float* d_bias,
+                                         float* d_out_pooled_c8, void* d_ws, int H, int W, int Cin, int Cout, int relu);
 MNC_API int mnc_maxpool2_c8(mnc_ctx* ctx, const float* d_in, float* d_out, int C, int H, int W);
 MNC_API int mnc_conv1x1_to_nchw(mnc_ctx* ctx, const float* d_in_c8, const float* d_w, const float* d_bias,
                                 float* d_out_nchw, int H, int W, int Cin, int Cout);
@@ -282,6 +289,8 @@
                    int N, int K, int ldc, int act);
 MNC_API int mnc_fc_pair(mnc_ctx* ctx, const float* d_a0, const float* d_w0, const float* d_bias0, float* d_out0, const float* d_a1,
                         const float* d_w1, const float* d_bias1, float* d_out1, int M, int N, int K, int ldc, int act);
+MNC_API int mnc_fc_batch(mnc_ctx* ctx, const float* d_a, long stride_a, const float* d_w, long stride_w, float* d_out,
+                         long stride_out, int B, int M, int N, int K, int ldc);
 MNC_API int mnc_pack_fc_bf16x3(mnc_ctx* ctx, const float* d_w, void* d_packed, int N, int K);
 MNC_API int mnc_fc_bf16x3(mnc_ctx* ctx, const float* d_a, const void* d_w_packed, const float* d_bias, float* d_out, int M,
                           int N, int K, int ldc, int act);
diff --git a/mnc_amd/_lib.py b/mnc_amd/_lib.py
--- a/mnc_amd/_lib.py
+++ b/mnc_amd/_lib.py
@@ -19,6 +19,7 @@
 
 _CTYPES = {
     "int": ctypes.c_int, "float": ctypes.c_float, "size_t": ctypes.c_size_t, "double": ctypes.c_double,
+    "long": ctypes.c_long,
     "void": None,
 }
 
diff --git a/mnc_amd/csrc/conv_wino4_split.hip b/mnc_amd/csrc/conv_wino4_split.hip
--- /dev/null
+++ b/mnc_amd/csrc/conv_wino4_split.hip
@@ -0,0 +1,228 @@
+#include "mnc_internal.h"
+
+namespace mnc {
+
+typedef float s4f __attribute__((ext_vector_type(4)));
+
+__device__ __forceinline__ s4f fma4(float s, s4f a, s4f b) {
+  return s4f{fmaf(s, a.x, b.x), fmaf(s, a.y, b.y), fmaf(s, a.z, b.z), fmaf(s, a.w, b.w)};
+}
+
+__device__ __forceinline__ void bt6(const s4f (&d)[6], s4f (&x)[6]) {
+  const s4f a = fma4(-4.f, d[2], d[4]), b = fma4(-4.f, d[1], d[3]), c = d[4] - d[2], e = d[3] - d[1];
+  x[0] = fma4(4.f, d[0], fma4(-5.f, d[2], d[4]));
+  x[1] = a + b;
+  x[2] = a - b;
+  x[3] = fma4(2.f, e, c);
+  x[4] = fma4(-2.f, e, c);
+  x[5] = fma4(4.f, d[1], fma4(-5.f, d[3], d[5]));
+}
+
+__device__ __forceinline__ void at6(const s4f (&m)[6], s4f (&y)[4]) {
+  const s4f s12 = m[1] + m[2], d12 = m[1] - m[2], s34 = m[3] + m[4], d34 = m[3] - m[4];
+  y[0] = (m[0] + s12) + s34;
+  y[1] = fma4(2.f, d34, d12);
+  y[2] = fma4(4.f, s34, s12);
+  y[3] = fma4(8.f, d34, d12) + m[5];
+}
+
+__global__ __launch_bounds__(256) void wino4_split_input_kernel(const float* __restrict__ in, float* __restrict__ V, int H, int W, int Cin,
+                                                                int tiles_x, int ntiles) {
+  const int c4n = Cin >> 2;
+  const long total = (long)ntiles * c4n;
+  const long idx = (long)blockIdx.x * blockDim.x + threadIdx.x;
+  if (idx >= total) return;
+  const int c4 = (int)(idx % c4n), tile = (int)(idx / c4n);
+  const int ty = tile / tiles_x, tx = tile - ty * tiles_x;
+  const int y0 = 4 * ty - 1, x0 = 4 * tx - 1;
+  const float* src = in + (long)(c4 >> 1) * H * W * 8 + (c4 & 1) * 4;
+  s4f t[6][6];
+#pragma unroll
+  for (int j = 0; j < 6; ++j) {
+    s4f d[6], x[6];
+    const int xx = x0 + j;
+#pragma unroll
+    for (int i = 0; i < 6; ++i) {
+      const int yy = y0 + i;
+      d[i] = s4f{0.f, 0.f, 0.f, 0.f};
+      if (yy >= 0 && yy < H && xx >= 0 && xx < W) d[i] = *reinterpret_cast<const s4f*>(src + ((long)yy * W + xx) * 8);
+    }
+    bt6(d, x);
+#pragma unroll
+    for (int i = 0; i < 6; ++i) t[i][j] = x[i];
+  }
+  float* dst = V + (long)tile * Cin + c4 * 4;
+  const long pstride = (long)ntiles * Cin;
+#pragma unroll
+  for (int i = 0; i < 6; ++i) {
+    s4f x[6];
+    bt6(t[i], x);
+#pragma unroll
+    for (int j = 0; j < 6; ++j) *reinterpret_cast<s4f*>(dst + (long)(6 * i + j) * pstride) = x[j];
+  }
+}
+
+template <int POOL>
+__global__ __launch_bounds__(256) void wino4_split_output_kernel(const float* __restrict__ Mt, const float* __restrict__ bias,
+                                                                 float* __restrict__ out, int H, int W, int Cout, int relu, int tiles_x,
+                                                                 int ntiles) {
+  const int c4n = Cout >> 2;
+  const long total = (long)ntiles * c4n;
+  const long idx = (long)blockIdx.x * blockDim.x + threadIdx.x;
+  if (idx >= total) return;
+  const int c4 = (int)(idx % c4n), tile = (int)(idx / c4n);
+  const int ty = tile / tiles_x, tx = tile - ty * tiles_x;
+  const int oy = 4 * ty, ox = 4 * tx;
+  const float* src = Mt + (long)tile * Cout + c4 * 4;
+  const long pstride = (long)ntiles * Cout;
+  s4f z[4][6];
+#pragma unroll
+  for (int j = 0; j < 6; ++j) {
+    s4f m[6], y[4];
+#pragma unroll
+    for (int i = 0; i < 6; ++i) m[i] = *reinterpret_cast<const s4f*>(src + (long)(6 * i + j) * pstride);
+    at6(m, y);
+#pragma unroll
+    for (int i = 0; i < 4; ++i) z[i][j] = y[i];
+  }
+  const s4f bv = *reinterpret_cast<const s4f*>(bias + c4 * 4);
+  s4f y[4][4];
+#pragma unroll
+  for (int i = 0; i < 4; ++i) {
+    at6(z[i], y[i]);
+#pragma unroll
+    for (int j = 0; j < 4; ++j) {
+      y[i][j] += bv;
+      if (relu) y[i][j] = s4f{fmaxf(y[i][j].x, 0.f), fmaxf(y[i][j].y, 0.f), fmaxf(y[i][j].z, 0.f), fmaxf(y[i][j].w, 0.f)};
+    }
+  }
+  const int cb = c4 >> 1, half = (c4 & 1) * 4;
+  if (!POOL) {
+#pragma unroll
+    for (int i = 0; i < 4; ++i)
+#pragma unroll
+      for (int j = 0; j < 4; ++j)
+        if (oy + i < H && ox + j < W) *reinterpret_cast<s4f*>(out + (((long)cb * H + oy + i) * W + ox + j) * 8 + half) = y[i][j];
+  } else {
+    const int OH = (H + 1) >> 1, OW = (W + 1) >> 1;
+#pragma unroll
+    for (int pi = 0; pi < 2; ++pi)
+#pragma unroll
+      for (int pj = 0; pj < 2; ++pj) {
+        const int py = oy + 2 * pi, px = ox + 2 * pj;
+        if (py >= H || px >= W) continue;
+        s4f best = y[2 * pi][2 * pj];
+#pragma unroll
+        for (int di = 0; di < 2; ++di)
+#pragma unroll
+          for (int dj = 0; dj < 2; ++dj)
+            if (py + di < H && px + dj < W) {
+              const s4f o = y[2 * pi + di][2 * pj + dj];
+              best = s4f{fmaxf(best.x, o.x), fmaxf(best.y, o.y), fmaxf(best.z, o.z), fmaxf(best.w, o.w)};
+            }
+        *reinterpret_cast<s4f*>(out + (((long)cb * OH + (py >> 1)) * OW + (px >> 1)) * 8 + half) = best;
+      }
+  }
+}
+
+__global__ __launch_bounds__(256) void pack_conv3x3_wino4_split_kernel(const float* __restrict__ w, float* __restrict__ U, int Cout,
+                                                                       int Cin) {
+  const double G[6][3] = {{6.0, 0.0, 0.0}, {-4.0, -4.0, -4.0}, {-4.0, 4.0, -4.0}, {1.0, 2.0, 4.0}, {1.0, -2.0, 4.0}, {0.0, 0.0, 24.0}};
+  const long total = (long)Cout * Cin;
+  for (long r = (long)blockIdx.x * blockDim.x + threadIdx.x; r < total; r += (long)gridDim.x * blockDim.x) {
+    const float* f = w + r * 9;
+    for (int a = 0; a < 6; ++a) {
+      double tmp[3];
+#pragma unroll
+      for (int b = 0; b < 3; ++b) tmp[b] = G[a][0] * (double)f[b] + G[a][1] * (double)f[3 + b] + G[a][2] * (double)f[6 + b];
+#pragma unroll
+      for (int b = 0; b < 6; ++b)
+        U[(long)(6 * a + b) * total + r] = (float)((tmp[0] * G[b][0] + tmp[1] * G[b][1] + tmp[2] * G[b][2]) / 576.0);
+    }
+  }
+}
+
+bool wino4_split_supported(int H, int W, int Cin, int Cout) {
+  return H > 0 && W > 0 && Cin > 0 && Cin % 32 == 0 && Cout > 0 && Cout % 32 == 0 &&
+         36.0 * cdiv(H, 4) * (double)cdiv(W, 4) * (Cin > Cout ? Cin : Cout) * 4.0 < 2.0e9;
+}
+
+bool wino4_split_selected(const mnc_ctx* ctx, int H, int W, int Cin, int Cout) {
+  const int v = tune(ctx, T_WINO_SPLIT, kWinoSplitDefault);
+  if (v == 0 || !wino4_split_supported(H, W, Cin, Cout)) return false;
+  if (v == 2) return true;
+  if (plan_latency(ctx)) return false;
+  return wino4_split_plan_channels(Cin, Cout) && cdiv(H, 4) * cdiv(W, 4) >= 304;
+}
+
+static size_t wino4_split_v_bytes(int H, int W, int Cin) {
+  return ((size_t)36 * cdiv(W, 4) * cdiv(H, 4) * Cin * 4 + 255) & ~(size_t)255;
+}
+
+static int wino4_split_impl(mnc_ctx* ctx, const float* d_in, const float* d_u, const float* d_bias, float* d_out, void* d_ws, int H,
+                            int W, int Cin, int Cout, int relu, int pool) {
+  MNC_REQUIRE(ctx && d_in && d_u && d_bias && d_out && d_ws, "mnc_conv3x3_wino4_split: null pointer");
+  MNC_REQUIRE((reinterpret_cast<uintptr_t>(d_ws) & 15) == 0, "mnc_conv3x3_wino4_split: workspace not 16-byte aligned");
+  MNC_REQUIRE(wino4_split_supported(H, W, Cin, Cout),
+              "mnc_conv3x3_wino4_split: unsupported shape H=%d W=%d Cin=%d Cout=%d (need Cin%%32==0, Cout%%32==0)", H, W, Cin, Cout);
+  const int tiles_x = cdiv(W, 4), ntiles = tiles_x * cdiv(H, 4);
+  float* V = (float*)d_ws;
+  float* Mt = (float*)((char*)d_ws + wino4_split_v_bytes(H, W, Cin));
+  const double flops = 2.0 * H * W * 9.0 * Cin * Cout;
+  const double out_px = pool ? (double)((H + 1) / 2) * ((W + 1) / 2) : (double)H * W;
+  const double bytes = 4.0 * ((double)H * W * Cin + out_px * Cout + 9.0 * Cin * Cout);
+  LaunchScope ls(ctx, "conv3x3_wino4_mfma", flops, bytes);
+  const long in_items = (long)ntiles * (Cin >> 2), out_items = (long)ntiles * (Cout >> 2);
+  hipLaunchKernelGGL(wino4_split_input_kernel, dim3((unsigned)((in_items + 255) / 256)), dim3(256), 0, ctx->stream, d_in, V, H, W, Cin,
+                     tiles_x, ntiles);
+  int rc = fc_batch_launch(ctx, V, (long)ntiles * Cin, d_u, (long)Cout * Cin, Mt, (long)ntiles * Cout, 36, ntiles, Cout, Cin, Cout);
+  if (rc) {
+    (void)ls.finish("conv3x3_wino4_split");
+    return rc;
+  }
+  if (pool)
+    hipLaunchKernelGGL(wino4_split_output_kernel<1>, dim3((unsigned)((out_items + 255) / 256)), dim3(256), 0, ctx->stream, Mt, d_bias,
+                       d_out, H, W, Cout, relu, tiles_x, ntiles);
+  else
+    hipLaunchKernelGGL(wino4_split_output_kernel<0>, dim3((unsigned)((out_items + 255) / 256)), dim3(256), 0, ctx->stream, Mt, d_bias,
+                       d_out, H, W, Cout, relu, tiles_x, ntiles);
+  return ls.finish("conv3x3_wino4_split");
+}
+
+}
+
+using namespace mnc;
+
+extern "C" {
+
+int mnc_pack_conv3x3_wino4_split(mnc_ctx* ctx, const float* d_oihw, float* d_packed, int Cout, int Cin) {
+  MNC_REQUIRE(ctx && d_oihw && d_packed && Cin > 0 && Cin % 32 == 0 && Cout > 0 && Cout % 32 == 0,
+              "mnc_pack_conv3x3_wino4_split: bad argument (Cin%%32==0, Cout%%32==0)");
+  LaunchScope ls(ctx, "pack_conv3x3_wino4_split");
+  long g = ((long)Cout * Cin + 255) / 256;
+  if (g > 8192) g = 8192;
+  hipLaunchKernelGGL(pack_conv3x3_wino4_split_kernel, dim3((int)g), dim3(256), 0, ctx->stream, d_oihw, d_packed, Cout, Cin);
+  return ls.finish("pack_conv3x3_wino4_split_kernel");
+}
+
+size_t mnc_conv3x3_wino4_split_ws_bytes(int H, int W, int Cin, int Cout) {
+  if (!wino4_split_supported(H, W, Cin, Cout)) return 0;
+  return wino4_split_v_bytes(H, W, Cin) + (size_t)36 * cdiv(W, 4) * cdiv(H, 4) * Cout * 4;
+}
+
+int mnc_conv3x3_wino4_split_selected(mnc_ctx* ctx, int H, int W, int Cin, int Cout) {
+  return ctx && wino4_split_selected(ctx, H, W, Cin, Cout) ? 1 : 0;
+}
+
+int mnc_conv3x3_wino4_split(mnc_ctx* ctx, const float* d_in, const float* d_u, const float* d_bias, float* d_out, void* d_ws, int H,
+                            int W, int Cin, int Cout, int relu) {
+  return wino4_split_impl(ctx, d_in, d_u, d_bias, d_out, d_ws, H, W, Cin, Cout, relu, 0);
+}
+
+int mnc_conv3x3_wino4_split_pool(mnc_ctx* ctx, const float* d_in, const float* d_u, const float* d_bias, float* d_out_pooled,
+                                 void* d_ws, int H, int W, int Cin, int Cout, int relu) {
+  MNC_REQUIRE(H >= 2 && W >= 2, "mnc_conv3x3_wino4_split_pool: map %dx%d too small for MAX 2x2/2", H, W);
+  return wino4_split_impl(ctx, d_in, d_u, d_bias, d_out_pooled, d_ws, H, W, Cin, Cout, relu, 1);
+}
+
+}
diff --git a/mnc_amd/csrc/gemm.hip b/mnc_amd/csrc/gemm.hip
--- a/mnc_amd/csrc/gemm.hip
+++ b/mnc_amd/csrc/gemm.hip
@@ -407,14 +407,15 @@
   }
 }
 
-template <int kMT, int ABL = 0, int BUF = 0>
+template <int kMT, int ABL = 0, int BUF = 0, int BATCH = 0>
 __global__ __launch_bounds__(512) void fc_mfma_dma16_kernel(const float* __restrict__ A_0, const float* __restrict__ Wt_0,
                                                             const float* __restrict__ bias_0, float* __restrict__ out_0,
                                                             float* __restrict__ part_0, int M, int N, int K, int ldc, int kper,
                                                             int act, int fused, int tn_, int splits_, int tm_, int drop_last,
                                                             const float* __restrict__ A_1,
                                                             const float* __restrict__ Wt_1, const float* __restrict__ bias_1,
-                                                            float* __restrict__ out_1, int pair_tn) {
+                                                            float* __restrict__ out_1, int pair_tn, long batch_a,
+                                                            long batch_w, long batch_o) {
   constexpr int kBM = 32 * kMT;
   constexpr int kRows = kBM + kBN;
   constexpr int kNW = 8;
@@ -429,17 +430,19 @@
   const int r16 = lane & 15, g4 = lane >> 4;
   int bn, split, bmz;
   xcd_decode(blockIdx.x, tn_, splits_, tm_, bn, split, bmz);
-  const int which = (pair_tn && bn >= pair_tn) ? 1 : 0;
+  int which = (pair_tn && bn >= pair_tn) ? 1 : 0;
   bn -= which * pair_tn;
-  const float* __restrict__ A = which ? A_1 : A_0;
-  const float* __restrict__ Wt = which ? Wt_1 : Wt_0;
+  if (BATCH) { which = bmz; bmz = split; split = 0; }
+  const float* __restrict__ A = BATCH ? A_0 + which * batch_a : which ? A_1 : A_0;
+  const float* __restrict__ Wt = BATCH ? Wt_0 + which * batch_w : which ? Wt_1 : Wt_0;
   const float* __restrict__ bias = which ? bias_1 : bias_0;
-  float* __restrict__ out = which ? out_1 : out_0;
+  float* __restrict__ out = BATCH ? out_0 + which * batch_o : which ? out_1 : out_0;
   float* __restrict__ part = part_0;
-  const int n0 = bn * kBN, m0 = bmz * kBM;
+  constexpr int kLive = kBM - 16;
+  const int n0 = bn * kBN, m0 = bmz * (BATCH && drop_last ? kLive : kBM);
   const int kbeg = split * kper, kend = min(K, kbeg + kper);
   const int nstages = (kend - kbeg) / 32;
-  const int mrows = min(M - m0, kBM);
+  const int mrows = min(M - m0, BATCH && drop_last ? kLive : kBM);
 
   const float* src[kPer];
 #pragma unroll
@@ -566,6 +569,21 @@
   }
 
   const bool final_out = fused == 1;
+  if (BATCH) {
+#pragma unroll
+    for (int c = 0; c < 2; ++c) {
+      const int n = n0 + wn * 32 + c * 16 + r16;
+      if (n >= N) continue;
+#pragma unroll
+      for (int i = 0; i < TS; ++i)
+#pragma unroll
+        for (int e = 0; e < 4; ++e) {
+          const int r = wm * TS * 16 + i * 16 + 4 * g4 + e;
+          if (r < mrows) out[(long)(m0 + r) * ldc + n] = acc[i][c][e];
+        }
+    }
+    return;
+  }
   if (fused == 0) {
     constexpr int kSlabF4 = kNW * TS * 2 * 64;
     const int tile = bmz * tn_ + which * pair_tn + bn;
@@ -768,6 +786,25 @@
   }
 }
 
+int fc_batch_launch(mnc_ctx* ctx, const float* d_a, long stride_a, const float* d_w, long stride_w, float* d_out, long stride_o, int B,
+                    int M, int N, int K, int ldc) {
+  MNC_REQUIRE(ctx && d_a && d_w && d_out, "fc_batch: null pointer");
+  MNC_REQUIRE(B > 0 && M > 0 && N > 0 && K > 0 && K % kBK == 0 && ldc >= N && stride_a >= 0 && stride_w >= 0 && stride_o >= 0,
+              "fc_batch: unsupported shape B=%d M=%d N=%d K=%d ldc=%d (need K%%32==0)", B, M, N, K, ldc);
+  MNC_REQUIRE(320.0 * (double)K * 4.0 < 1.8e9 && stride_a % 4 == 0 && stride_w % 4 == 0 &&
+                  ((reinterpret_cast<uintptr_t>(d_a) | reinterpret_cast<uintptr_t>(d_w)) & 15) == 0,
+              "fc_batch: operands must be 16-byte aligned, K=%d below the descriptor range", K);
+  const int drop = cdiv(M, 304) == cdiv(M, 320) ? 1 : 0;
+  const int tn = cdiv(N, kBN), tm = cdiv(M, drop ? 304 : 320);
+  MNC_REQUIRE((double)B * tn * tm < 2.0e9, "fc_batch: too many workgroups");
+  constexpr int lds = 65536 + (320 + kBN) * 32 * 4;
+  MNC_HIP_TRY((lds_limit_once<fc_mfma_dma16_kernel<10, 0, 1, 1>>(ctx->device, lds)));
+  hipLaunchKernelGGL((fc_mfma_dma16_kernel<10, 0, 1, 1>), dim3(B * tn * tm), dim3(512), lds, ctx->stream, d_a, d_w, (const float*)nullptr,
+                     d_out, (float*)nullptr, M, N, K, ldc, K, 0, 1, tn, tm, B, drop, (const float*)nullptr, (const float*)nullptr,
+                     (const float*)nullptr, (float*)nullptr, 0, stride_a, stride_w, stride_o);
+  return MNC_OK;
+}
+
 }
 
 using namespace mnc;
@@ -824,7 +861,7 @@
         MNC_HIP_TRY(hipFuncSetAttribute(reinterpret_cast<const void*>(kern), hipFuncAttributeMaxDynamicSharedMemorySize, lds));
         hipLaunchKernelGGL(kern, dim3(tn * splits * tm), dim3(512), lds, ctx->stream, d_a, d_w, d_bias, d_out, part, M, N, K, ldc, kper,
                            act, splits == 1 ? 1 : 0, tn, splits, tm, p.drop, (const float*)nullptr, (const float*)nullptr,
-                           (const float*)nullptr, (float*)nullptr, 0);
+                           (const float*)nullptr, (float*)nullptr, 0, 0L, 0L, 0L);
       } else if (tune(ctx, T_FC_MFMA16, 1) == 0 || waves == 4 || dabl) {
         launched = true;
         if (dabl == 1) MNC_FC_DMA_LAUNCH(1, 1);
@@ -839,7 +876,8 @@
         else MNC_HIP_TRY((lds_limit_once<fc_mfma_dma16_kernel<10, 0, 0>>(ctx->device, lds)));
         hipLaunchKernelGGL((p.buf ? fc_mfma_dma16_kernel<10, 0, 1> : fc_mfma_dma16_kernel<10, 0, 0>), dim3(tn * splits * tm), dim3(512), lds,
                            ctx->stream, d_a, d_w, d_bias, d_out, part, M, N, K, ldc, kper, act, splits == 1 ? 1 : 0, tn, splits,
-                           tm, p.drop, (const float*)nullptr, (const float*)nullptr, (const float*)nullptr, (float*)nullptr, 0);
+                           tm, p.drop, (const float*)nullptr, (const float*)nullptr, (const float*)nullptr, (float*)nullptr, 0, 0L, 0L,
+                           0L);
       }
     }
     else if (mt == 2) MNC_FC_LAUNCH(2, 32, 0);
@@ -921,7 +959,7 @@
     MNC_HIP_TRY((lds_limit_once<fc_mfma_dma16_kernel<10, 0, 1>>(ctx->device, lds)));
     hipLaunchKernelGGL((fc_mfma_dma16_kernel<10, 0, 1>), dim3(2 * tn * splits * tm), dim3(512), lds, ctx->stream, d_a0, d_w0, d_bias0,
                        d_out0, part, M, N, K, ldc, kper, act, splits == 1 ? 1 : 0, 2 * tn, splits, tm, p.drop, d_a1, d_w1,
-                       d_bias1, d_out1, tn);
+                       d_bias1, d_out1, tn, 0L, 0L, 0L);
     int rc = ls.finish("fc_mfma_dma16_kernel");
     if (rc) return rc;
   }
@@ -934,6 +972,15 @@
     return ls.finish("fc_reduce_slab_kernel");
   }
   return MNC_OK;
+}
+
+int mnc_fc_batch(mnc_ctx* ctx, const float* d_a, long stride_a, const float* d_w, long stride_w, float* d_out, long stride_out,
+                 int B, int M, int N, int K, int ldc) {
+  MNC_REQUIRE(ctx, "mnc_fc_batch: null context");
+  LaunchScope ls(ctx, "fc_batch", 2.0 * B * M * (double)N * K, 4.0 * B * ((double)N * K + (double)M * K + (double)M * N));
+  const int rc = fc_batch_launch(ctx, d_a, stride_a, d_w, stride_w, d_out, stride_out, B, M, N, K, ldc);
+  const int rf = ls.finish("fc_mfma_dma16_kernel");
+  return rc ? rc : rf;
 }
 
 int mnc_softmax_rows_ld(mnc_ctx* ctx, const float* d_in, int ld_in, float* d_out, int M, int N) {
diff --git a/mnc_amd/csrc/mnc_internal.h b/mnc_amd/csrc/mnc_internal.h
--- a/mnc_amd/csrc/mnc_internal.h
+++ b/mnc_amd/csrc/mnc_internal.h
@@ -250,6 +250,10 @@
                       int act);
 bool fc_reduce_launch_sm(hipStream_t stream, const float* part, const float* bias, float* out, int M, int N, int ldc, int splits,
                          int act, void* sm, int sm_fmt, long sm_rows, long sm_row0);
+int fc_batch_launch(mnc_ctx* ctx, const float* d_a, long stride_a, const float* d_w, long stride_w, float* d_out, long stride_o, int B,
+                    int M, int N, int K, int ldc);
+bool wino4_split_supported(int H, int W, int Cin, int Cout);
+bool wino4_split_selected(const mnc_ctx* ctx, int H, int W, int Cin, int Cout);
 bool fc_reduce_pair_launch_sm(hipStream_t stream, const float* part0, const float* part1, const float* bias0, const float* bias1,
                               float* out0, float* out1, int M, int N, int ldc, int splits, int act, void* sm0, void* sm1, int sm_fmt,
                               long sm_rows, bool* sm_done);
diff --git a/mnc_amd/csrc/pipeline.hip b/mnc_amd/csrc/pipeline.hip
--- a/mnc_amd/csrc/pipeline.hip
+++ b/mnc_amd/csrc/pipeline.hip
@@ -55,6 +55,7 @@
   std::atomic<int> sharers{0};
   float* w_c3 = nullptr;
   void* w_conv[14] = {nullptr};
+  float* w_split[14] = {nullptr};
   bool packed_trunk = false;
   bool conv_fast[14] = {false};
   float* b_conv[14] = {nullptr};
@@ -66,6 +67,7 @@
   float* rpn_bbox_p = nullptr;
   DevBuf rois, rois_ext, feat14, h_mask, m14, box7, mask7, f6, f6m, join, heads, boxes, masks, scores;
   DevBuf outblk;
+  DevBuf wino_ws;
   DevBuf hwc5;
   float* records() const { return (float*)((char*)outblk.p + 512); }
   int* counts() const { return (int*)outblk.p; }
@@ -241,6 +243,14 @@
         NET_TRY(mnc_dev_alloc(n->ctx, (size_t)cout * cin * 9 * 4, &n->w_conv[i]));
         NET_TRY(mnc_pack_conv_weights(n->ctx, raw, (float*)n->w_conv[i], cout, cin, 3, 3));
       }
+      const int ws = tune(n->ctx, T_WINO_SPLIT, kWinoSplitDefault);
+      if (n->conv_fast[i] && conv_math(c) == 0 && c.winograd == 4 && wino4_split_supported(4, 4, cin, cout) &&
+          (ws == 2 || (ws == 1 && wino4_split_plan_channels(cin, cout)))) {
+        void* u = nullptr;
+        NET_TRY(mnc_dev_alloc(n->ctx, (size_t)36 * cout * cin * 4, &u));
+        n->w_split[i] = (float*)u;
+        NET_TRY(mnc_pack_conv3x3_wino4_split(n->ctx, raw, n->w_split[i], cout, cin));
+      }
       NET_TRY(mnc_dev_free(n->ctx, raw));
     }
     cin = cout;
@@ -295,14 +305,24 @@
   NET_TRY(dev_ensure(n, &n->taps, (size_t)(2 * OW + 2 * OH) * 4));
   NET_TRY(dev_ensure(n, &n->data, (size_t)3 * OH * OW * 4));
   int h = OH, w = OW, pi = 0;
+  size_t split_ws = 0;
+  auto split_need = [&](int i, int hh, int ww, int cin, int cout) {
+    if (n->w_split[i] && wino4_split_selected(n->ctx, hh, ww, cin, cout)) {
+      const size_t b = mnc_conv3x3_wino4_split_ws_bytes(hh, ww, cin, cout);
+      if (b > split_ws) split_ws = b;
+    }
+  };
   for (int i = 0; i < 13; ++i) {
     const int ch = c.trunk_channels[kTrunkStage[i]];
+    if (i > 0) split_need(i, h, w, c.trunk_channels[kTrunkStage[i - 1]], ch);
     NET_TRY(dev_ensure(n, &n->act[i], (size_t)ch * h * w * 4));
     if (kPoolAfter[i]) {
       h = pool_out(h); w = pool_out(w);
       NET_TRY(dev_ensure(n, &n->pooled[pi++], (size_t)ch * h * w * 4));
     }
   }
+  split_need(13, h, w, c.trunk_channels[4], c.rpn_channels);
+  if (split_ws) NET_TRY(dev_ensure(n, &n->wino_ws, split_ws));
   const int A = c.num_anchors;
   if (n->packed_trunk) NET_TRY(dev_ensure(n, &n->act12_pk, (size_t)c.trunk_channels[4] * h * w * 4));
   NET_TRY(dev_ensure(n, &n->hwc5, (size_t)c.trunk_channels[4] * h * w * 4));
@@ -382,6 +402,8 @@
     if (cm == 2) return mnc_conv2d_f16(n->ctx, in, n->w_conv[i], n->b_conv[i], nullptr, out, h, w, cin, cout, 3, 3, 1, 1, 1);
     return mnc_conv2d(n->ctx, in, (const float*)n->w_conv[i], n->b_conv[i], nullptr, out, h, w, cin, cout, 3, 3, 1, 1, 1);
   }
+  if (cm == 0 && c.winograd == 4 && n->w_split[i] && wino4_split_selected(n->ctx, h, w, cin, cout))
+    return mnc_conv3x3_wino4_split(n->ctx, in, n->w_split[i], n->b_conv[i], out, n->wino_ws.p, h, w, cin, cout, 1);
   if (cm == 0 && c.winograd == 4)
     return mnc_conv3x3_wino4(n->ctx, in, (const float*)n->w_conv[i], n->b_conv[i], out, h, w, cin, cout, 1);
   if (cm == 0 && c.winograd)
@@ -432,6 +454,9 @@
     float* out = (float*)n->act[i].p;
     if (kPoolAfter[i] && i > 0 && conv_math(c) == 0 && c.winograd && n->conv_fast[i]) {
       float* p = (float*)n->pooled[pi++].p;
+      if (c.winograd == 4 && n->w_split[i] && wino4_split_selected(ctx, h, w, cin, cout))
+        NET_TRY(mnc_conv3x3_wino4_split_pool(ctx, cur, n->w_split[i], n->b_conv[i], p, n->wino_ws.p, h, w, cin, cout, 1));
+      else
       NET_TRY(c.winograd == 4 ? mnc_conv3x3_wino4_pool(ctx, cur, (const float*)n->w_conv[i], n->b_conv[i], p, h, w, cin, cout, 1)
                               : mnc_conv3x3_wino_pool(ctx, cur, (const float*)n->w_conv[i], n->b_conv[i], p, h, w, cin, cout, 1));
       h = pool_out(h); w = pool_out(w);
@@ -746,6 +771,7 @@
   n->w_c3 = parent->w_c3;
   for (int i = 0; i < 14; ++i) {
     n->w_conv[i] = parent->w_conv[i];
+    n->w_split[i] = parent->w_split[i];
     n->b_conv[i] = parent->b_conv[i];
     n->conv_fast[i] = parent->conv_fast[i];
   }
@@ -1014,7 +1040,8 @@
   DevBuf* bufs[] = {&net->img, &net->taps, &net->data, &net->rpn_out, &net->rpn_score, &net->rpn_prob, &net->rois,
                     &net->rois_ext, &net->feat14, &net->h_mask, &net->m14, &net->box7, &net->mask7, &net->f6, &net->f6m, &net->join,
                     &net->feat14_sm, &net->box7_sm, &net->mask7_sm, &net->f6_sm, &net->f6m_sm,
-                    &net->heads, &net->boxes, &net->masks, &net->scores, &net->outblk, &net->hwc5, &net->act12_pk};
+                    &net->heads, &net->boxes, &net->masks, &net->scores, &net->outblk, &net->hwc5, &net->act12_pk,
+                    &net->wino_ws};
   for (DevBuf* b : bufs) if (b->p) (void)hipFree(b->p);
   for (auto& b : net->act) if (b.p) (void)hipFree(b.p);
   for (auto& b : net->pooled) if (b.p) (void)hipFree(b.p);
@@ -1025,6 +1052,7 @@
     for (void* p : singles) if (p) (void)hipFree(p);
     for (int i = 0; i < 14; ++i) {
       if (net->w_conv[i]) (void)hipFree(net->w_conv[i]);
+      if (net->w_split[i]) (void)hipFree(net->w_split[i]);
       if (net->b_conv[i]) (void)hipFree(net->b_conv[i]);
     }
     mnc_net::Fc* fcs[] = {&net->fc_maskest, &net->fc_maskpred, &net->fc6, &net->fc7, &net->fc6m, &net->fc7m, &net->fc_heads};
diff --git a/mnc_amd/csrc/tune.h b/mnc_amd/csrc/tune.h
--- a/mnc_amd/csrc/tune.h
+++ b/mnc_amd/csrc/tune.h
@@ -6,7 +6,7 @@
   X(CONV_COT) X(CONV_ROWS) X(CONV_KSPLIT) X(CONV_ABL) X(CONV1X1_TILE) X(CONV2D_WIDE) X(WINO_ROWS) X(WINO_TAIL) X(WINO_V) X(WINO_VAR)  \
   X(WINO_DMA) X(WINO_XCD) X(CONVX3_TILE) X(FC_NOTAIL) X(FC_TILE) X(FC_ABL) X(FC_DMA) X(PLAN) X(FC_RANGE_K) X(FC_SLOTS) X(FC_EVEN) X(FC_SPLIT_DIV) X(WINO_FILL) X(CONVX3_P0MIN) X(CONVX3_P1MIN) X(FC_DMA_ABL) X(FC_DMA_WAVES)    \
   X(FC_NO256) X(FCX3_TILE) X(FC_ORDER) X(FCX3_ABL) X(FC_SM) X(PACKED_ACT) X(FUSE_POOLS) X(BRANCH_STREAMS) X(TOPK_SINGLE_WG)           \
-  X(ROI_SM_VARIANT) X(ROI_WARP_VARIANT) X(FC_REDUCE) X(WINO_F4) X(FUSE_SMALL) X(FCX3_WIDE) X(FC_HALF) X(WINO_STREAM) X(FC_MFMA16) X(WINO_MFMA16) X(ROI_ROW_SEGS)
+  X(ROI_SM_VARIANT) X(ROI_WARP_VARIANT) X(FC_REDUCE) X(WINO_F4) X(FUSE_SMALL) X(FCX3_WIDE) X(FC_HALF) X(WINO_STREAM) X(FC_MFMA16) X(WINO_MFMA16) X(ROI_ROW_SEGS) X(WINO_SPLIT)
 enum TuneKey {
 #define MNC_TUNE_ENUM(n) T_##n,
   MNC_TUNE_KEYS(MNC_TUNE_ENUM)
@@ -19,5 +19,8 @@
 inline int tune(const int* t, TuneKey k, int dflt) { return t[k] != kTuneUnset ? t[k] : dflt; }
 inline bool plan_latency(const int* t) { return tune(t, T_PLAN, 0) == 1; }
 
+constexpr int kWinoSplitDefault = 1;
+inline bool wino4_split_plan_channels(int Cin, int Cout) { return Cin >= 512 && Cout >= 512; }
+
 static inline int cdiv(long a, long b) { return (int)((a + b - 1) / b); }
 }
diff --git a/mnc_amd/engine.py b/mnc_amd/engine.py
--- a/mnc_amd/engine.py
+++ b/mnc_amd/engine.py
@@ -793,6 +793,24 @@
                 return packed
             d_w = self._dev_param(key + ("w", self.conv_math, ("wino%d" % self._wino) if (self._winograd and not x3) else "direct"), build)
 
+            def split_form(H, Wd):
+                selected = getattr(_lib.load(), "mnc_conv3x3_wino4_split_selected", None)
+                if x3 or self._wino != 4 or selected is None or not selected(self._h(), H, Wd, cin, cout):
+                    return None
+
+                def build_split():
+                    raw = self._upload(W)
+                    packed = self._ctx.alloc(36 * cout * cin * 4)
+                    _lib.call("mnc_pack_conv3x3_wino4_split", self._h(), raw, packed, cout, cin)
+                    self._ctx.free(raw)
+                    return packed
+                need = int(_lib.load().mnc_conv3x3_wino4_split_ws_bytes(H, Wd, cin, cout))
+                have = max([k[1] for k in self._dev_params if k[0] == "wino4_split_ws"] or [0])
+                if have < need:
+                    have = need
+                    self._dev_params[("wino4_split_ws", have)] = self._ctx.alloc(have)
+                return self._dev_param(key + ("w", "wino4split"), build_split), self._dev_params[("wino4_split_ws", have)]
+
             def run():
                 N, _, H, Wd = bot.shape
                 pk = _PACKED_OF.get(self.conv_math)
@@ -813,7 +831,12 @@
                     OH, OW = _pool_out(H), _pool_out(Wd)
                     top.reshape(N, cout, OH, OW)
                     dst = top.dev_out("c8")
+                    sp = split_form(H, Wd)
                     for n in range(N):
+                        if sp:
+                            _lib.call("mnc_conv3x3_wino4_split_pool", self._h(), src + n * cin * H * Wd * 4, sp[0], d_b,
+                                      dst + n * cout * OH * OW * 4, sp[1], H, Wd, cin, cout, relu)
+                            continue
                         _lib.call("mnc_conv3x3_wino4_pool" if self._wino == 4 else "mnc_conv3x3_wino_pool", self._h(), src + n * cin * H * Wd * 4, d_w, d_b,
                                   dst + n * cout * OH * OW * 4, H, Wd, cin, cout, relu)
                     return
@@ -827,7 +850,12 @@
                                   dst + n * cout * H * Wd * ob, H, Wd, cin, cout, relu, 1 if in_h else 0, 1 if L.out_h else 0)
                     return
                 dst = top.dev_out("c8")
+                sp = split_form(H, Wd)
                 for n in range(N):
+                    if sp:
+                        _lib.call("mnc_conv3x3_wino4_split", self._h(), src + n * cin * H * Wd * 4, sp[0], d_b,
+                                  dst + n * cout * H * Wd * 4, sp[1], H, Wd, cin, cout, relu)
+                        continue
                     _lib.call(conv, self._h(), src + n * cin * H * Wd * 4, d_w, d_b, dst + n * cout * H * Wd * 4, H, Wd, cin,
                               cout, relu)
             return run
```
